# nianticlabs/implicit-depth

Measured on AMD Instinct MI355X. Metric: frames/sec (BDModel.forward hot path, 512x384, 64 planes, 8-frame tuple = 1 current + 7 source views; third-party backbones excluded), higher is better.
Workload: dtype f32

## Files before the change

implicit-depth_amd/_lib.py:

```python
from __future__ import annotations

import ctypes as C
import os

import torch

_HERE = os.path.dirname(os.path.abspath(__file__))
LIB_PATH = os.environ.get("IDH_LIB") or os.path.join(_HERE, "lib", "libidh.so")

_lib = None
MIN_ABI_VERSION = 111

f32p = C.c_void_p


class IdhError(RuntimeError):
    pass


class VolumeOpts(C.Structure):

    _fields_ = [("cur_batch_stride", C.c_int64), ("src_batch_stride", C.c_int64), ("planes", C.c_void_p),
                ("planes_batch_stride", C.c_int64), ("planes_plane_stride", C.c_int64), ("planes_pixel_stride", C.c_int32),
                ("kernel", C.c_int32), ("scratch", C.c_void_p), ("scratch_floats", C.c_int64), ("struct_size", C.c_int64)]

    def __init__(self, *a, **k):
        super().__init__(*a, **k)
        self.struct_size = C.sizeof(VolumeOpts)


CV_KERNEL_LANE, CV_KERNEL_QUAD, CV_KERNEL_WINDOW = 1, 2, 3


class EvalArgs(C.Structure):

    _fields_ = [("struct_size", C.c_int64), ("prediction", C.c_void_p), ("pred_kind", C.c_int32), ("sampling", C.c_int32),
                ("sigmoid_multiplier", C.c_float), ("surface_threshold", C.c_float), ("rendered_bphw", C.c_void_p), ("depth_b1hw", C.c_void_p),
                ("gt_b1HW", C.c_void_p), ("thresholds", C.c_void_p), ("bins", C.c_void_p), ("T", C.c_int32), ("n_bins", C.c_int32),
                ("tag_mask", C.c_int32), ("B", C.c_int32), ("P", C.c_int32), ("h", C.c_int32), ("w", C.c_int32), ("H", C.c_int32), ("W", C.c_int32)]

    def __init__(self, *a, **k):
        super().__init__(*a, **k)
        self.struct_size = C.sizeof(EvalArgs)


EVAL_PRED_LOGITS, EVAL_PRED_DEPTH = 0, 1
EVAL_BILINEAR, EVAL_NEAREST = 0, 1
EVAL_TAG_ALL, EVAL_TAG_SURFACE, EVAL_TAG_BOUNDARY = 1, 2, 4


class CompositeArgs(C.Structure):

    _fields_ = [("struct_size", C.c_int64), ("image_bHW3", C.c_void_p), ("virtual_rgba_bHW4", C.c_void_p), ("map_b1hw", C.c_void_p),
                ("virtual_depth_bHW", C.c_void_p), ("fade_b", C.c_void_p), ("out_bHW3", C.c_void_p), ("matte_out_bHW", C.c_void_p),
                ("plane_distance", C.c_double), ("colour", C.c_double * 3), ("sigmoid_multiplier", C.c_float), ("mode", C.c_int32),
                ("has_colour", C.c_int32), ("has_plane", C.c_int32), ("bgr", C.c_int32), ("B", C.c_int32), ("h", C.c_int32), ("w", C.c_int32),
                ("H", C.c_int32), ("W", C.c_int32)]

    def __init__(self, *a, **k):
        super().__init__(*a, **k)
        self.struct_size = C.sizeof(CompositeArgs)


COMPOSITE_MASK_LOGITS, COMPOSITE_MASK_PROB, COMPOSITE_DEPTH_SOFT, COMPOSITE_DEPTH_HARD = 0, 1, 2, 3


class IngestColorArgs(C.Structure):

    _fields_ = [("struct_size", C.c_int64), ("frames_bHW3", C.c_void_p), ("x_bounds", C.c_void_p), ("x_taps", C.c_void_p), ("y_bounds", C.c_void_p),
                ("y_taps", C.c_void_p), ("image_b3hw", C.c_void_p), ("resized_bhw3", C.c_void_p), ("filter", C.c_int32), ("normalize", C.c_int32),
                ("B", C.c_int32), ("Hs", C.c_int32), ("Ws", C.c_int32), ("h", C.c_int32), ("w", C.c_int32)]

    def __init__(self, *a, **k):
        super().__init__(*a, **k)
        self.struct_size = C.sizeof(IngestColorArgs)


class IngestDepthArgs(C.Structure):

    _fields_ = [("struct_size", C.c_int64), ("depth_bHW", C.c_void_p), ("depth_b1hw", C.c_void_p), ("mask_b1hw", C.c_void_p),
                ("mask_b_b1hw", C.c_void_p), ("full_depth_b1HW", C.c_void_p), ("full_mask_b1HW", C.c_void_p), ("full_mask_b_b1HW", C.c_void_p),
                ("value_scale", C.c_float), ("min_valid", C.c_float), ("max_valid", C.c_float), ("B", C.c_int32), ("Hs", C.c_int32),
                ("Ws", C.c_int32), ("h", C.c_int32), ("w", C.c_int32)]

    def __init__(self, *a, **k):
        super().__init__(*a, **k)
        self.struct_size = C.sizeof(IngestDepthArgs)


class Bank(C.Structure):

    _fields_ = [("struct_size", C.c_int64), ("feats", C.c_void_p), ("mats", C.c_void_p), ("N", C.c_int32), ("H", C.c_int32), ("W", C.c_int32),
                ("C", C.c_int32)]

    def __init__(self, *a, **k):
        super().__init__(*a, **k)
        self.struct_size = C.sizeof(Bank)


BANK_MAX_SLOTS, BANK_MAX_VIEWS = 64, 1024

RESIZE_BILINEAR, RESIZE_BICUBIC = 0, 1
INGEST_MAX_RATIO = 8


class ConvDescSrc(C.Structure):
    _fields_ = [(n, C.c_int32) for n in ("H", "W", "cs", "Cin", "ks", "stride", "is_cat", "_r")]


class ConvDesc(C.Structure):

    _fields_ = ([(n, C.c_int32) for n in ("N", "Ho", "Wo", "Cout", "pad_mode", "act")] + [("slope", C.c_float)] +
                [(n, C.c_int32) for n in ("out_cs", "res_cs", "has_res", "has_norm", "any_size", "math", "n_src")] + [("src", ConvDescSrc * 2)])


class ConvTuning(C.Structure):

    _fields_ = ([(n, C.c_int32) for n in ("winograd", "winograd4", "winograd4_proj", "s2_first", "wino_min_tiles", "wino4_min_tiles", "split_min_blocks",
                                          "narrow_tile_below", "narrowest_tile_below", "split_min_chunks", "split_max", "s2_first_min_blocks",
                                          "fused_up_rows", "target_waves", "min_waves", "_r")] +
                [(n, C.c_double) for n in ("wino_min_fill", "wino4_min_fill", "proj_chunk_weight")])


class ConvChoice(C.Structure):

    _fields_ = [(n, C.c_int32) for n in ("tile_m", "tile_n", "split_k", "w_layout", "families", "lds_tile_m", "lds_split_k", "lds_subtiles", "split_rows",
                                         "direct_tile_m", "direct_tile_n", "direct_split_k")]


_SIGS = {
    "idh_version": (C.c_int, []),
    "idh_sizeof_volume_opts": (C.c_size_t, []),
    "idh_cost_volume_dot_scratch_floats": (C.c_longlong, [C.c_int, C.c_int, C.c_int, C.c_int, C.c_int, C.c_int]),
    "idh_error_string": (C.c_char_p, [C.c_int]),
    "idh_nchw_to_nhwc_f32": (C.c_int, [f32p, f32p, C.c_int, C.c_int, C.c_int, C.c_void_p]),
    "idh_nhwc_to_nchw_f32": (C.c_int, [f32p, f32p, C.c_int, C.c_int, C.c_int, C.c_void_p]),
    "idh_packed_weight_floats": (C.c_size_t, [C.c_int, C.c_int, C.c_int]),
    "idh_pack_conv_weight": (C.c_int, [f32p, f32p, C.c_int, C.c_int, C.c_int, C.c_void_p]),
    "idh_packed_split_weight_bytes": (C.c_size_t, [C.c_int, C.c_int, C.c_int, C.c_int]),
    "idh_pack_conv_weight_split": (C.c_int, [f32p, f32p, C.c_void_p, C.c_int, C.c_int, C.c_int, C.c_int, C.c_void_p]),
    "idh_packed_wino_weight_floats": (C.c_size_t, [C.c_int, C.c_int]),
    "idh_pack_conv_weight_wino": (C.c_int, [f32p, f32p, C.c_int, C.c_int, C.c_void_p]),
    "idh_packed_wino4_weight_floats": (C.c_size_t, [C.c_int, C.c_int]),
    "idh_pack_conv_weight_wino4": (C.c_int, [f32p, f32p, C.c_int, C.c_int, C.c_void_p]),
    "idh_stem_weight_floats": (C.c_size_t, []),
    "idh_pack_stem_weight": (C.c_int, [f32p] * 5 + [C.c_float, f32p, C.c_void_p]),
    "idh_fold_conv_bn": (C.c_int, [f32p, C.c_int, C.c_int] + [f32p] * 4 + [C.c_float, f32p, f32p, C.c_void_p]),
    "idh_sizeof_op": (C.c_size_t, []),
    "idh_run_ops": (C.c_int, [C.c_void_p, C.c_int, C.c_void_p]),
    "idh_count_launches": (C.c_int, [C.c_void_p, C.c_int]),
    "idh_conv_variant": (C.c_int, [C.c_void_p, C.POINTER(C.c_int32)]),
    "idh_conv_tuning_defaults": (None, [C.POINTER(ConvTuning)]),
    "idh_conv_select": (C.c_int, [C.POINTER(ConvDesc), C.POINTER(ConvTuning), C.POINTER(ConvChoice)]),
    "idh_sizeof_conv_select": (None, [C.POINTER(C.c_size_t)]),
    "idh_schedule_ops": (C.c_int, [C.c_void_p, C.c_int, C.c_int, C.c_void_p, C.c_void_p, C.c_int, C.c_void_p, C.c_void_p]),
    "idh_packed_mlp_weight_floats": (C.c_size_t, [C.c_int]),
    "idh_pack_mlp_weight": (C.c_int, [f32p, f32p, C.c_int, C.c_int, C.c_int, C.c_void_p]),
    "idh_binary_mlp_fwd": (C.c_int, [f32p, C.c_int, C.c_int, f32p, f32p, C.c_int, C.c_float, f32p, f32p, f32p, C.c_int, C.c_int, C.c_int, f32p, C.c_void_p]),
    "idh_binary_mlp_strided_fwd": (C.c_int, [f32p, C.c_longlong, C.c_int, C.c_int, C.c_int, f32p, f32p, C.c_int, C.c_float, f32p, f32p, f32p, C.c_int, C.c_int, C.c_int, f32p, C.c_void_p]),
    "idh_binary_mlp_f16x3_fwd": (C.c_int, [f32p, C.c_int, C.c_int, f32p, f32p, C.c_int, C.c_float, f32p, f32p, f32p, C.c_int, C.c_int, C.c_int, f32p, C.c_void_p]),
    "idh_feature_volume_workspace_bytes": (C.c_size_t, [C.c_int]),
    "idh_feature_volume_plane_groups": (C.c_int, [C.c_int] * 4 + [C.POINTER(C.c_int)] * 2),
    "idh_feature_volume_fwd": (
        C.c_int,
        [f32p] * 6 + [C.c_float, C.c_float] + [C.c_int] * 6 + [f32p] * 6 + [f32p, C.c_int, f32p, C.c_void_p, f32p, C.c_void_p, C.c_size_t, C.c_void_p],
    ),
    "idh_feature_volume_f16x3_fwd": (
        C.c_int,
        [f32p] * 6 + [C.c_float, C.c_float] + [C.c_int] * 6 + [f32p] * 6 + [f32p, C.c_int, f32p, C.c_void_p, f32p, C.c_void_p, C.c_size_t, C.c_void_p],
    ),
    "idh_feature_volume_ex_fwd": (
        C.c_int,
        [f32p] * 6 + [C.c_float, C.c_float] + [C.c_int] * 6 + [f32p] * 6 + [f32p, C.c_int, f32p, C.c_void_p, f32p, C.c_void_p, C.c_size_t,
                                                                  C.c_int, C.POINTER(VolumeOpts), C.c_void_p],
    ),
    "idh_cost_volume_dot_ex_fwd": (
        C.c_int,
        [f32p, f32p, f32p, f32p, f32p, C.c_float, C.c_float] + [C.c_int] * 6 + [f32p, C.c_int, f32p, f32p, C.POINTER(VolumeOpts), C.c_void_p],
    ),
    "idh_cost_volume_dot_kernel_name": (C.c_char_p, [C.c_int] * 5),
    "idh_packed_mlp_weight_f16_bytes": (C.c_size_t, [C.c_int]),
    "idh_pack_mlp_weight_f16": (C.c_int, [f32p, C.c_void_p, C.c_int, C.c_int, C.c_int, C.c_void_p]),
    "idh_binary_mlp_search_fwd": (C.c_int, [f32p, C.c_int, C.c_int, f32p, C.c_int, C.c_float, f32p, f32p, f32p, C.c_int, C.c_int, C.c_int,
                                            C.c_float, C.c_float, C.c_float, f32p, f32p, C.c_void_p]),
    "idh_binary_mlp_search_thr_fwd": (C.c_int, [f32p, C.c_int, C.c_int, f32p, C.c_int, C.c_float, f32p, f32p, f32p, C.c_int, C.c_int, C.c_int,
                                                C.c_float, C.c_float, f32p, f32p, C.c_int, f32p, f32p, C.c_void_p]),
    "idh_binary_mlp_search_f16x3_fwd": (C.c_int, [f32p, C.c_int, C.c_int, f32p, C.c_int, C.c_float, f32p, C.c_void_p, f32p, C.c_int, C.c_int, C.c_int,
                                                  C.c_float, C.c_float, C.c_float, f32p, f32p, C.c_int, f32p, f32p, C.c_void_p]),
    "idh_metrics_workspace_bytes": (C.c_size_t, [C.c_int, C.c_int, C.c_int, C.c_int]),
    "idh_plane_iou_fwd": (C.c_int, [f32p, f32p, f32p, f32p, C.c_int, f32p, C.c_int, C.c_int, C.c_int, C.c_int, f32p, C.c_void_p, C.c_size_t, C.c_void_p]),
    "idh_depth_metrics_fwd": (C.c_int, [f32p, f32p, C.c_void_p, C.c_int, C.c_int, C.c_int, f32p, C.c_void_p, C.c_size_t, C.c_void_p]),
    "idh_sizeof_eval_args": (C.c_size_t, []),
    "idh_eval_frame_workspace_bytes": (C.c_size_t, [C.c_int] * 7),
    "idh_eval_masks_fwd": (C.c_int, [f32p, f32p, C.c_int, C.c_int, C.c_int, C.c_int, C.c_float, f32p, f32p, C.c_void_p, C.c_void_p]),
    "idh_eval_plane_scores_fwd": (C.c_int, [C.POINTER(EvalArgs), f32p, C.c_void_p, C.c_void_p, C.c_size_t, C.c_void_p]),
    "idh_eval_depth_metrics_fwd": (C.c_int, [f32p, f32p] + [C.c_int] * 6 + [C.c_float, C.c_int, f32p, C.c_void_p, C.c_size_t, C.c_void_p]),
    "idh_raster_workspace_bytes": (C.c_size_t, [C.c_int] * 3),
    "idh_raster_depth_fwd": (C.c_int, [f32p, C.c_int, C.c_void_p, C.c_int, f32p, f32p, C.c_int, C.c_int, C.c_int, f32p, C.c_void_p, C.c_size_t, C.c_void_p]),
    "idh_vertex_predictions_fwd": (C.c_int, [f32p, C.c_int, f32p, f32p, f32p, f32p, C.c_int, C.c_int, C.c_float, f32p, C.c_void_p]),
    "idh_vertex_occlusion_changes_fwd": (C.c_int, [f32p, C.c_int, C.c_int, C.c_void_p, C.c_void_p]),
    "idh_sizeof_composite_args": (C.c_size_t, []),
    "idh_prep_rendered_depth_fwd": (C.c_int, [f32p, C.c_int, C.c_int, C.c_int, C.c_int, C.c_int, f32p, C.c_void_p]),
    "idh_composite_fwd": (C.c_int, [C.POINTER(CompositeArgs), C.c_void_p]),
    "idh_resize_coeffs_sizes": (C.c_int, [C.c_int, C.c_int, C.c_int, C.POINTER(C.c_int64), C.POINTER(C.c_int64)]),
    "idh_resize_coeffs_pack": (C.c_int, [C.c_int, C.c_int, C.c_int, C.c_void_p, C.c_void_p]),
    "idh_sizeof_ingest_color_args": (C.c_size_t, []),
    "idh_sizeof_ingest_depth_args": (C.c_size_t, []),
    "idh_ingest_color_fwd": (C.c_int, [C.POINTER(IngestColorArgs), C.c_void_p]),
    "idh_ingest_depth_fwd": (C.c_int, [C.POINTER(IngestDepthArgs), C.c_void_p]),
    "idh_sizeof_bank": (C.c_size_t, []),
    "idh_bank_commit_fwd": (C.c_int, [C.POINTER(Bank), C.c_int, f32p, f32p, f32p, f32p, C.c_void_p]),
    "idh_bank_gather_fwd": (C.c_int, [C.POINTER(Bank), C.POINTER(C.c_int32), f32p, f32p, f32p, f32p, f32p, f32p, C.c_int, C.c_int, C.c_void_p]),
    "idh_sample_prior_fwd": (C.c_int, [f32p, f32p, C.c_int, f32p, f32p, f32p, f32p, C.c_int, C.c_int, C.c_int, C.c_int, f32p, C.c_void_p]),
    "idh_binary_mlp_rays_fwd": (C.c_int, [f32p, C.c_int, C.c_int, C.c_int, C.c_int, C.c_int, f32p, f32p, f32p, C.c_int, C.c_float, C.c_int, C.c_int,
                                          C.c_int, C.c_int, C.c_int, f32p, f32p, f32p, f32p, C.c_void_p]),
    "idh_project_points_fwd": (C.c_int, [f32p, f32p, f32p, C.c_int, C.c_int, C.c_int, C.c_int, f32p, f32p, C.c_void_p, f32p, f32p, f32p, f32p, C.c_void_p]),
    "idh_cost_volume_dot_fwd": (
        C.c_int,
        [f32p, f32p, f32p, f32p, f32p, C.c_float, C.c_float] + [C.c_int] * 6 + [f32p, C.c_int, f32p, f32p, C.c_void_p],
    ),
}


def _all_sigs():
    from . import model_abi, net_abi

    return {**_SIGS, **net_abi.SIGS, **model_abi.SIGS}


def declared_symbols():
    return sorted(_all_sigs())


def lib():
    global _lib
    if _lib is None:
        if not os.path.exists(LIB_PATH):
            raise IdhError(
                f"{LIB_PATH} not found — the gfx950 HIP extension is not built. Run "
                "`python -c 'import __graft_entry__ as g; g.build()'` (there is no CPU fallback)."
            )
        h = C.CDLL(LIB_PATH)
        for name, (res, args) in _all_sigs().items():
            try:
                fn = getattr(h, name)
            except AttributeError:
                raise IdhError(f"{LIB_PATH} does not export {name}: it was built from an older tree; rebuild with `python implicit-depth_amd/build.py --force`") from None
            fn.restype = res
            fn.argtypes = args
        ver = h.idh_version()
        if ver < MIN_ABI_VERSION and not os.environ.get("IDH_LIB_ANY_ABI"):
            raise IdhError(f"{LIB_PATH} reports ABI version {ver}, this binding needs >= {MIN_ABI_VERSION}: rebuild with `python implicit-depth_amd/build.py --force`")
        if h.idh_sizeof_eval_args() != C.sizeof(EvalArgs):
            raise IdhError(f"{LIB_PATH}: sizeof(idh_eval_args) = {h.idh_sizeof_eval_args()} in the library, {C.sizeof(EvalArgs)} in this binding")
        if h.idh_sizeof_composite_args() != C.sizeof(CompositeArgs):
            raise IdhError(f"{LIB_PATH}: sizeof(idh_composite_args) = {h.idh_sizeof_composite_args()} in the library, {C.sizeof(CompositeArgs)} in this binding")
        for what, got, mirror in (("idh_ingest_color_args", h.idh_sizeof_ingest_color_args(), IngestColorArgs),
                                  ("idh_ingest_depth_args", h.idh_sizeof_ingest_depth_args(), IngestDepthArgs),
                                  ("idh_bank", h.idh_sizeof_bank(), Bank)):
            if got != C.sizeof(mirror):
                raise IdhError(f"{LIB_PATH}: sizeof({what}) = {got} in the library, {C.sizeof(mirror)} in this binding")
        sizes = (C.c_size_t * 3)()
        h.idh_sizeof_conv_select(sizes)
        if list(sizes) != [C.sizeof(ConvDesc), C.sizeof(ConvTuning), C.sizeof(ConvChoice)]:
            raise IdhError(f"{LIB_PATH}: sizeof(idh_conv_desc / _tuning / _choice) = {list(sizes)} in the library, another in this binding")
        if h.idh_sizeof_volume_opts() != C.sizeof(VolumeOpts):
            raise IdhError(f"{LIB_PATH}: sizeof(idh_volume_opts) = {h.idh_sizeof_volume_opts()} in the library, {C.sizeof(VolumeOpts)} in this binding")
        _lib = h
    return _lib


def check(code: int, what: str) -> None:
    if code != 0:
        msg = lib().idh_error_string(code).decode()
        raise IdhError(f"{what} failed: {msg} ({code})")


def ptr(t: "torch.Tensor | None"):
    if t is None:
        return None
    return t.data_ptr()


def stream_ptr():
    return torch.cuda.current_stream().cuda_stream


_weights_epoch = 0


def invalidate_weight_caches() -> None:
    global _weights_epoch
    _weights_epoch += 1


def _sd_post_hook(module, incompatible_keys) -> None:
    invalidate_weight_caches()


def watch_state_dict_loads(module) -> None:
    for m in module.modules():
        if not m.__dict__.get("_idh_sd_hook"):
            m.register_load_state_dict_post_hook(_sd_post_hook)
            m.__dict__["_idh_sd_hook"] = True


def param_version(t):
    try:
        return t._version
    except RuntimeError:
        return ("inference", _weights_epoch)


def require_cuda_f32(*tensors):
    for t in tensors:
        if t is None:
            continue
        if not t.is_cuda:
            raise IdhError("implicit_depth_amd kernels need tensors on the MI355X (got a CPU tensor); there is no CPU fallback")
        if t.dtype != torch.float32:
            raise IdhError(f"implicit_depth_amd kernels are fp32 (got {t.dtype})")
```

implicit-depth_amd/csrc/conv.hip:

```cpp
#include <algorithm>
#include "conv_args.h"
#include "../../include/idh_ops.h"

using namespace idh_conv;

int idh_stem_op(const idh_op &op, hipStream_t st, bool launch);

namespace {

__device__ float g_zero_page[kZeroFloats];

thread_local bool t_dry_run = false;
thread_local int t_launches = 0;
#undef IDH_CHECK_LAUNCH
#define IDH_CHECK_LAUNCH()                                              \
    do {                                                                \
        if (!t_dry_run && hipGetLastError() != hipSuccess) return IDH_ELAUNCH; \
    } while (0)
#define IDH_LAUNCH(...)                         \
    do {                                        \
        if (t_dry_run) ++t_launches;            \
        else hipLaunchKernelGGL(__VA_ARGS__);   \
    } while (0)

// ... 896 lines not shown
            float *o = a.out + ((size_t)n * a.HW + p) * a.out_cs + 4 * h;
#pragma unroll
            for (int j = 0; j < NT; ++j) {
                f32x4 v = acc[j];
                if (a.bias) v += *reinterpret_cast<const f32x4 *>(a.bias + 16 * j + 4 * h);
                *reinterpret_cast<f32x4 *>(o + 16 * j) = v;
            }
        }
    };
    f32x4 xa[C16], xb[C16];
    long long t = blockIdx.x;
    if (t >= a.tiles) return;
    load(t, xa);
    for (;;) {
        const long long t1 = t + gridDim.x;
        if (t1 < a.tiles) load(t1, xb);
        compute(t, xa);
        if (t1 >= a.tiles) break;
        const long long t2 = t1 + gridDim.x;
        if (t2 < a.tiles) load(t2, xa);
        compute(t1, xb);
        if (t2 >= a.tiles) break;
        t = t2;
    }
}

struct PwUpArgs {
    const float *in, *w, *bias, *low;
    float *out;
    int H, W, in_cs, low_cs, out_cs, tiles_per_img;
    long long tiles;
};

template <int C16, int NT>
__global__ __launch_bounds__(256) void pointwise_up_k(const PwUpArgs a) {
    constexpr int kCout = 16 * NT;
    extern __shared__ f32x4 sWu[];
    {
        const f32x4 *g = reinterpret_cast<const f32x4 *>(a.w);
        for (int i = threadIdx.x; i < 4 * C16 * kCout; i += 256) sWu[i] = g[i];
    }
    __syncthreads();
    const int lane = threadIdx.x & 63;
    const int wave = __builtin_amdgcn_readfirstlane(threadIdx.x >> 6);
    const int ln = lane & 15, h = lane >> 4;
    const int HW = a.H * a.W, Hl = a.H >> 1, Wl = a.W >> 1;
    for (long long tile = blockIdx.x; tile < a.tiles; tile += gridDim.x) {
        const int n = (int)(tile / a.tiles_per_img);
        const int p = (int)(tile - (long long)n * a.tiles_per_img) * kPwTile + 16 * wave + ln;
        const bool ok = p < HW;
        const int pc = ok ? p : 0;
        const float *ip = a.in + ((size_t)n * HW + pc) * a.in_cs + 4 * h;
        f32x4 x[C16];
#pragma unroll
        for (int c = 0; c < C16; ++c) x[c] = *reinterpret_cast<const f32x4 *>(ip + 16 * c);
        const int y = pc / a.W, xq = pc - y * a.W;
        const int iy = y >> 1, ix = xq >> 1;
        int y0, y1, x0, x1;
        float hy0, hy1, wx0, wx1;
        if (y & 1) { y0 = iy; y1 = min(iy + 1, Hl - 1); hy0 = 0.75f; hy1 = 0.25f; }
        else { y0 = max(iy - 1, 0); y1 = iy; hy0 = 0.25f; hy1 = 0.75f; }
        if (xq & 1) { x0 = ix; x1 = min(ix + 1, Wl - 1); wx0 = 0.75f; wx1 = 0.25f; }
        else { x0 = max(ix - 1, 0); x1 = ix; wx0 = 0.25f; wx1 = 0.75f; }
        const float *lb = a.low + (size_t)n * Hl * Wl * a.low_cs + 4 * h;
        const float *t00 = lb + ((size_t)y0 * Wl + x0) * a.low_cs, *t01 = lb + ((size_t)y0 * Wl + x1) * a.low_cs;
        const float *t10 = lb + ((size_t)y1 * Wl + x0) * a.low_cs, *t11 = lb + ((size_t)y1 * Wl + x1) * a.low_cs;
        f32x4 acc[NT];
#pragma unroll
        for (int j = 0; j < NT; ++j) acc[j] = a.bias ? *reinterpret_cast<const f32x4 *>(a.bias + 16 * j + 4 * h) : (f32x4){0.f, 0.f, 0.f, 0.f};
        int opaque = 0;
        asm volatile("" : "+s"(opaque));
        const f32x4 *sWt = sWu + opaque;
#pragma unroll
        for (int c = 0; c < C16; ++c)
#pragma unroll
            for (int j = 0; j < NT; ++j) {
                const f32x4 A = sWt[(4 * c + h) * kCout + 16 * j + ln];
#pragma unroll
                for (int kk = 0; kk < 4; ++kk) acc[j] = __builtin_amdgcn_mfma_f32_16x16x4f32(A[kk], x[c][kk], acc[j], 0, 0, 0);
            }
        if (ok) {
            float *o = a.out + ((size_t)n * HW + p) * a.out_cs + 4 * h;
#pragma unroll
            for (int j = 0; j < NT; ++j) {
                const f32x4 p00 = *reinterpret_cast<const f32x4 *>(t00 + 16 * j), p01 = *reinterpret_cast<const f32x4 *>(t01 + 16 * j);
                const f32x4 p10 = *reinterpret_cast<const f32x4 *>(t10 + 16 * j), p11 = *reinterpret_cast<const f32x4 *>(t11 + 16 * j);
                f32x4 v;
#pragma unroll
                for (int e = 0; e < 4; ++e) v[e] = acc[j][e] + (hy0 * (wx0 * p00[e] + wx1 * p01[e]) + hy1 * (wx0 * p10[e] + wx1 * p11[e]));
                *reinterpret_cast<f32x4 *>(o + 16 * j) = v;
            }
        }
    }
}

__global__ __launch_bounds__(256) void pointwise_head_k(const float *__restrict__ in, const float *__restrict__ w,
                                                        const float *__restrict__ bias, float *__restrict__ out,
                                                        float *__restrict__ out_exp, long long M, int C, int in_cs) {
    for (long long m = blockIdx.x * 256ll + threadIdx.x; m < M; m += gridDim.x * 256ll) {
        const float4 *p = reinterpret_cast<const float4 *>(in + m * in_cs);
        const float4 *wv = reinterpret_cast<const float4 *>(w);
        float s = 0.f;
        for (int q = 0; q < (C >> 2); ++q) {
            const float4 a = p[q], b = wv[q];
            s = fmaf(a.x, b.x, s); s = fmaf(a.y, b.y, s); s = fmaf(a.z, b.z, s); s = fmaf(a.w, b.w, s);
        }
        const float v = s + (bias ? bias[0] : 0.f);
        out[m] = v;
        if (out_exp) out_exp[m] = expf(v);
    }
}

constexpr int kInChunk = 1024;

template <int SUB>
__global__ __launch_bounds__(1024) void instnorm_stats_k(const float *__restrict__ in, int cs, int C, int HW, int nchunks,
                                                         float *__restrict__ part) {
    extern __shared__ float red[];
    const int n = blockIdx.y, chunk = blockIdx.x;
    const int cq = C >> 2;
    const int q = threadIdx.x % cq;
    const int prow = threadIdx.x / cq, pstep = (int)blockDim.x / cq;
    const int rows = SUB * pstep;
    const int p0 = chunk * kInChunk, p1 = min(HW, p0 + kInChunk);
    const float4 pv = *reinterpret_cast<const float4 *>(in + (size_t)n * HW * cs + 4 * q);
    float s[SUB][4], ss[SUB][4];
#pragma unroll
    for (int u = 0; u < SUB; ++u)
#pragma unroll
        for (int e = 0; e < 4; ++e) s[u][e] = ss[u][e] = 0.f;
    for (int p = p0 + prow; p < p1; p += rows) {
#pragma unroll
        for (int u = 0; u < SUB; ++u) {
            const int pp = p + u * pstep;
            if (pp < p1) {
                const float4 v = *reinterpret_cast<const float4 *>(in + ((size_t)n * HW + pp) * cs + 4 * q);
                const float d0 = v.x - pv.x, d1 = v.y - pv.y, d2 = v.z - pv.z, d3 = v.w - pv.w;
                s[u][0] += d0; s[u][1] += d1; s[u][2] += d2; s[u][3] += d3;
                ss[u][0] = fmaf(d0, d0, ss[u][0]); ss[u][1] = fmaf(d1, d1, ss[u][1]); ss[u][2] = fmaf(d2, d2, ss[u][2]); ss[u][3] = fmaf(d3, d3, ss[u][3]);
            }
        }
    }
#pragma unroll
    for (int u = 0; u < SUB; ++u) {
        float *mine = red + ((size_t)(prow + u * pstep) * cq + q) * 8;
#pragma unroll
        for (int e = 0; e < 4; ++e) { mine[e] = s[u][e]; mine[4 + e] = ss[u][e]; }
    }
    __syncthreads();
    for (int t = threadIdx.x; t < 8 * cq; t += blockDim.x) {
        const int qq = t >> 3, e = t & 7;
        float a = 0.f;
        for (int r = 0; r < rows; ++r) a += red[(r * cq + qq) * 8 + e];
        part[((size_t)(n * nchunks + chunk) * 2 + (e >> 2)) * C + 4 * qq + (e & 3)] = a;
    }
}

__global__ __launch_bounds__(256) void instnorm_finalize_k(const float *__restrict__ part, const float *__restrict__ in, int cs, int C, int HW,
                                                           int nchunks, float *__restrict__ stats) {
    const int n = blockIdx.x;
    for (int c = threadIdx.x; c < C; c += 256) {
        float s = 0.f, ss = 0.f;
        for (int k = 0; k < nchunks; ++k) {
            const float *o = part + ((size_t)(n * nchunks + k) * 2) * C + c;
            s += o[0];
            ss += o[C];
        }
        const float ms = s / (float)HW;
        const float var = fmaxf(ss / (float)HW - ms * ms, 0.f);
        stats[(size_t)n * 2 * C + c] = in[(size_t)n * HW * cs + c] + ms;
        stats[(size_t)n * 2 * C + C + c] = 1.0f / sqrtf(var + 1e-5f);
    }
}

__global__ __launch_bounds__(256) void instnorm_apply_k(const float *__restrict__ in, int cs, float *__restrict__ out, int out_cs,
                                                        int C, int HW, long long total, const float *__restrict__ stats, int act,
                                                        float slope) {
    const int cq = C >> 2;
    for (long long t = blockIdx.x * 256ll + threadIdx.x; t < total; t += gridDim.x * 256ll) {
        const int q = (int)(t % cq);
        const long long np = t / cq;
        const int n = (int)(np / HW);
        const float4 mean = *reinterpret_cast<const float4 *>(stats + (size_t)n * 2 * C + 4 * q);
        const float4 rstd = *reinterpret_cast<const float4 *>(stats + (size_t)n * 2 * C + C + 4 * q);
        const float4 v = *reinterpret_cast<const float4 *>(in + (size_t)np * cs + 4 * q);
        float r[4] = {(v.x - mean.x) * rstd.x, (v.y - mean.y) * rstd.y, (v.z - mean.z) * rstd.z, (v.w - mean.w) * rstd.w};
        for (int e = 0; e < 4; ++e) r[e] = act_apply(r[e], act, slope);
        *reinterpret_cast<float4 *>(out + (size_t)np * out_cs + 4 * q) = make_float4(r[0], r[1], r[2], r[3]);
    }
}

enum { LV_LDS4 = 0, LV_LDS2 = 1, LV_MFMA14 = 2, LV_UP2 = 3 };
struct LevelArgs {
    int n;
    unsigned start[kMaxGroup + 1];
    int kind[kMaxGroup];
    LdsConvArgs op[kMaxGroup];
};

template <bool WIDE>
__global__ __launch_bounds__(256) void level_k(const LevelArgs g) {
    __shared__ f32x4 sA[lds_a_slots(1)];
    __shared__ f32x4 sB[lds_b_slots(WIDE ? 4 : 2)];
    int idx = 0;
    for (int i = 1; i < g.n; ++i)
        if (blockIdx.x >= g.start[i]) idx = i;
    const unsigned blk = blockIdx.x - g.start[idx], nblk = g.start[idx + 1] - g.start[idx];
    const LdsConvArgs &la = g.op[idx];
    switch (g.kind[idx]) {
        case LV_LDS4:
            if constexpr (WIDE) conv3x3_lds_body<1, false, 4>(la, blk, nblk, sA, sB);
            break;
        case LV_LDS2: conv3x3_lds_body<1, false, 2>(la, blk, nblk, sA, sB); break;
        case LV_MFMA14: conv_mfma_body<1, 4>(la.c, blk, nblk); break;
        default: upsample2_body(la.c.s[0].in, la.c.out, la.c.M, la.c.s[0].H, la.c.s[0].W, la.c.s[0].Cin, la.c.s[0].cs, la.c.out_cs, blk, nblk); break;
    }
}

inline int ceil16(int v) { return (v + 15) & ~15; }

struct PreparedConv {
    ConvArgs a;
    LdsConvArgs la;
    int lds_rows, tm, tn;
    int n_img;
    unsigned blocks;
    bool up;
    bool norm;
    bool s2;
    int nj;
    ReduceDesc red;
};

int prep_conv(const idh_op &op, PreparedConv &pc) {
    ConvArgs &a = pc.a;
    a = ConvArgs{};
    pc.up = false;
    pc.norm = op.src[0].norm != nullptr;
    pc.s2 = false;
    pc.nj = 4;
    int steps = 0;
    for (int i = 0; i < 2; ++i) {
        const idh_conv_src &s = op.src[i];
        ConvSrc &d = a.s[i];
        d.in = s.in;
        if (!s.in) continue;
        if (!s.w || s.Cin <= 0 || s.cs < (s.up_in[0] ? s.up_c0 : ceil16(s.Cin)) || (s.cs & 3) || (s.ks != 1 && s.ks != 3) ||
            (s.stride != 1 && s.stride != 2) || s.H <= 0 || s.W <= 0)
            return IDH_EINVAL;
        if (ceil16(s.Cin) > kZeroFloats) return IDH_EUNSUPPORTED;
        const int pad = s.ks / 2;
        if ((s.H + 2 * pad - s.ks) / s.stride + 1 != op.Ho || (s.W + 2 * pad - s.ks) / s.stride + 1 != op.Wo)
            return IDH_EINVAL;
        d.w = s.w; d.cs = s.cs; d.H = s.H; d.W = s.W; d.Cin = s.Cin; d.ks = s.ks; d.stride = s.stride;
        d.pad_mode = s.pad_mode; d.cblocks = ceil16(s.Cin) / 16;
        d.up_in[0] = s.up_in[0]; d.up_in[1] = s.up_in[1]; d.up_cs[0] = s.up_cs[0]; d.up_cs[1] = s.up_cs[1];
        d.up_c0 = s.up_c0; d.up_C = s.up_C;
        d.norm = s.norm; d.norm_slope = s.norm_slope; d.norm_act = s.norm_act;
        if (s.norm && (i != 0 || s.up_in[0] || ((uintptr_t)s.norm & 15) || (s.Cin & 15))) return IDH_EUNSUPPORTED;
        if (s.up_in[0]) {
            const int nseg = s.up_in[1] ? 2 : 1;
            if (s.up_c0 < 0 || (s.up_c0 & 15) || s.up_C <= 0 || (s.up_C & 15) || s.up_c0 + nseg * s.up_C != s.Cin || (s.H & 1) || (s.W & 1) ||
                s.stride != 1 || (s.up_c0 > 0 && s.cs < s.up_c0) || s.up_cs[0] < s.up_C || (s.up_cs[0] & 3) ||
                (nseg == 2 && (s.up_cs[1] < s.up_C || (s.up_cs[1] & 3))))
                return IDH_EINVAL;
            pc.up = true;
        }
        steps += s.ks * s.ks * d.cblocks;
    }
    if (!a.s[0].in || !op.out || op.Cout <= 0 || op.N <= 0) return IDH_EINVAL;
    if ((op.Cout & 3) || (op.out_cs & 3) || ((uintptr_t)op.out & 15) || (op.bias && ((uintptr_t)op.bias & 15)) ||
        (op.res && ((op.res_cs & 3) || ((uintptr_t)op.res & 15))))
        return IDH_EINVAL;
    a.bias = op.bias; a.res = op.res; a.out = op.out; a.ws = op.ws;
    a.res_cs = op.res_cs; a.out_cs = op.out_cs; a.Ho = op.Ho; a.Wo = op.Wo; a.Cout = op.Cout;
    a.Cout_pad = ceil16(op.Cout);
    const long long M = (long long)op.N * op.Ho * op.Wo;
    if (M >= (1ll << 31)) return IDH_EUNSUPPORTED;
    a.M = (int)M; a.steps_total = steps; a.act = op.act; a.slope = op.slope;
    a.S = op.split_k > 1 ? op.split_k : 1;
    if (a.S > steps) a.S = steps;
    if (a.s[0].ks == 3 && a.s[0].stride == 2 && !a.s[1].in && (op.tile_m == 8 || op.tile_m == 9) && a.s[0].pad_mode == IDH_PAD_ZEROS &&
        !a.s[0].up_in[0] && !a.s[0].norm && op.Wo >= kLT_W && (op.Cout % 32) == 0 && (op.tile_n == 0 ? (op.Cout % 64) == 0 : op.tile_n == 2)) {
        a.s[1] = a.s[0];
        ConvSrc e{};
        e.in = a.s[1].in; e.w = a.s[1].w; e.ks = 3; e.stride = 1; e.pad_mode = IDH_PAD_ZEROS;
        a.s[0] = e;
    }
    const int nj = (op.tile_m == 8 || op.tile_m == 9 || op.tile_m == 0) ? (op.tile_n == 0 ? 4 : op.tile_n) : 4;
    const bool lds_ok = a.s[0].ks == 3 && a.s[0].stride == 1 && (nj == 4 || nj == 2 || nj == 1) && (op.Cout % (16 * nj)) == 0 &&
                        (a.s[0].pad_mode == IDH_PAD_ZEROS || (a.s[0].pad_mode == IDH_PAD_REPLICATE && !a.s[1].in)) &&
                        (!a.s[1].in || (a.s[1].ks == 1 && a.s[1].stride == 1) ||
                         (a.s[1].ks == 3 && a.s[1].stride == 2 && a.s[1].pad_mode == IDH_PAD_ZEROS && !a.s[1].up_in[0] && !a.s[0].up_in[0] &&
                          !op.src[0].norm && (nj == 4 || nj == 2))) &&
                        op.Wo >= kLT_W;
    pc.lds_rows = 0;
    const bool lds_fits = (long long)a.s[0].H * a.s[0].W * a.s[0].cs * 4 < (1ll << 31) && 9ll * a.s[0].cblocks * 4 * a.Cout_pad * 16 < (1ll << 31) &&
                          (!a.s[1].in || ((long long)a.s[1].H * a.s[1].W * a.s[1].cs * 4 < (1ll << 31) && 9ll * a.s[1].cblocks * 4 * a.Cout_pad * 16 < (1ll << 31))) &&
                          (long long)op.Ho * op.Wo * op.out_cs * 4 < (1ll << 31) && (!op.res || (long long)op.Ho * op.Wo * op.res_cs * 4 < (1ll << 31));
    if (op.tile_m == IDH_TILE_WINO) {
        if (!wino_supported(a)) return IDH_EUNSUPPORTED;
        pc.lds_rows = 32;
        pc.tm = op.tile_m;
        pc.tn = 0;
        pc.n_img = op.N;
        pc.blocks = 0;
    } else if (op.tile_m == IDH_TILE_WINO4) {
        if (!wino4_supported(a)) return IDH_EUNSUPPORTED;
        pc.lds_rows = 36;
        pc.tm = op.tile_m;
        pc.tn = 0;
        pc.n_img = op.N;
        pc.blocks = 0;
    } else if (op.tile_m == IDH_SPLIT_F16X3) {
        if (!lds_ok || a.s[0].pad_mode != IDH_PAD_ZEROS || (op.Cout % 64) || a.S != 1 || op.Wo < kSplitTile || op.Ho < 1 || (op.tile_n != 0 && op.tile_n != 8 && op.tile_n != 16))
            return IDH_EUNSUPPORTED;
        if (a.s[1].in && (a.s[1].ks != 1 || a.s[1].stride != 1 || a.s[1].H != op.Ho || a.s[1].W != op.Wo || a.s[1].up_in[0] || a.s[1].norm))
            return IDH_EUNSUPPORTED;
        a.NT = op.Cout / 64;
        pc.lds_rows = 16;
        pc.tm = op.tile_m;
        pc.tn = op.tile_n == 8 ? 8 : 16;
        pc.n_img = op.N;
        pc.blocks = 0;
    } else if (lds_ok && lds_fits && (op.tile_m == 8 || op.tile_m == 0 || op.tile_m == 9)) {
        const int rows = op.tile_m == 9 ? 4 : 8;
        const int chunks = a.s[0].cblocks + (a.s[1].in ? a.s[1].cblocks : 0);
        if (a.S > chunks) a.S = chunks;
        {
            const int w1 = (a.s[1].in && a.s[1].ks == 3) ? 9 : 1;
            const int T = 9 * a.s[0].cblocks + (a.s[1].in ? w1 * a.s[1].cblocks : 0);
            const int smax = T / 9 > 1 ? T / 9 : 1;
            if (a.S > smax) a.S = smax;
        }
        a.NT = op.Cout / (16 * nj);
        pc.nj = nj;
        pc.la = LdsConvArgs{a, (op.Wo + kLT_W - 1) / kLT_W, (op.Ho + rows - 1) / rows};
        const long long blocks = (long long)a.S * op.N * pc.la.tiles_x * pc.la.tiles_y * a.NT;
        if (blocks >= (1ll << 31)) return IDH_EUNSUPPORTED;
        pc.blocks = (unsigned)blocks;
        pc.lds_rows = rows;
        pc.s2 = a.s[1].in && a.s[1].ks == 3;
    } else {
        int tm = op.tile_m, tn = op.tile_n;
        if (tm == 8 || tm == 9) tm = 0;
        const int nsub = a.Cout_pad / 16;
        if (tn == 0) tn = (nsub % 4 == 0) ? 4 : (nsub % 2 == 0 ? 2 : 1);
        if (tm == 0) tm = 4;
        if ((tm != 1 && tm != 2 && tm != 4) || (tn != 1 && tn != 2 && tn != 4) || nsub % tn) return IDH_EINVAL;
        a.MT = (int)((M + 16 * tm - 1) / (16 * tm));
        a.NT = nsub / tn;
        pc.tm = tm; pc.tn = tn;
        const long long waves = (long long)a.MT * a.NT * a.S;
        if ((waves + 3) / 4 >= (1ll << 31)) return IDH_EUNSUPPORTED;
        pc.blocks = (unsigned)((waves + 3) / 4);
    }
    if (pc.up && ((pc.lds_rows != 8 && pc.lds_rows != 4) || pc.nj != 4)) return IDH_EUNSUPPORTED;
    if (pc.norm && ((pc.lds_rows != 8 && pc.lds_rows != 4) || pc.nj != 1)) return IDH_EUNSUPPORTED;
    if (a.S > 1) {
        if (!op.ws) return IDH_EWORKSPACE;
        pc.red = ReduceDesc{op.ws, op.bias, op.res, op.out, a.M, op.Cout, a.Cout_pad, a.S, op.res_cs, op.out_cs, op.act, op.slope};
    }
    return IDH_OK;
}

int launch_conv(const PreparedConv &pc, hipStream_t st) {
    if (pc.lds_rows == 16) {
        if (t_dry_run) { ++t_launches; return IDH_OK; }
        return launch_conv_split(pc.a, pc.n_img, pc.tm, pc.tn, st);
    }
    if (pc.lds_rows == 32) {
        if (t_dry_run) { ++t_launches; return IDH_OK; }
        return launch_conv_wino(pc.a, pc.n_img, pc.tn, st);
    }
    if (pc.lds_rows == 36) {
        if (t_dry_run) { ++t_launches; return IDH_OK; }
        return launch_conv_wino4(pc.a, pc.n_img, st);
    }
    if (pc.lds_rows == 8 && pc.up) IDH_LAUNCH(conv3x3_lds_up_k<2>, dim3(pc.blocks), dim3(256), 0, st, pc.la);
    else if (pc.lds_rows == 8 && pc.s2 && pc.nj == 4) IDH_LAUNCH((conv3x3_lds_k<2, false, 4, false, true>), dim3(pc.blocks), dim3(256), 0, st, pc.la);
    else if (pc.lds_rows == 8 && pc.s2) IDH_LAUNCH((conv3x3_lds_k<2, false, 2, false, true>), dim3(pc.blocks), dim3(256), 0, st, pc.la);
    else if (pc.lds_rows == 4 && pc.s2 && pc.nj == 4) IDH_LAUNCH((conv3x3_lds_k<1, false, 4, false, true>), dim3(pc.blocks), dim3(256), 0, st, pc.la);
    else if (pc.lds_rows == 4 && pc.s2) IDH_LAUNCH((conv3x3_lds_k<1, false, 2, false, true>), dim3(pc.blocks), dim3(256), 0, st, pc.la);
    else if (pc.lds_rows == 8 && pc.norm) IDH_LAUNCH((conv3x3_lds_k<2, false, 1, true>), dim3(pc.blocks), dim3(256), 0, st, pc.la);
    else if (pc.lds_rows == 4 && pc.norm) IDH_LAUNCH((conv3x3_lds_k<1, false, 1, true>), dim3(pc.blocks), dim3(256), 0, st, pc.la);
    else if (pc.lds_rows == 8 && pc.nj == 2) IDH_LAUNCH((conv3x3_lds_k<2, false, 2>), dim3(pc.blocks), dim3(256), 0, st, pc.la);
    else if (pc.lds_rows == 8 && pc.nj == 1) IDH_LAUNCH((conv3x3_lds_k<2, false, 1>), dim3(pc.blocks), dim3(256), 0, st, pc.la);
    else if (pc.lds_rows == 4 && pc.nj == 2) IDH_LAUNCH((conv3x3_lds_k<1, false, 2>), dim3(pc.blocks), dim3(256), 0, st, pc.la);
    else if (pc.lds_rows == 4 && pc.nj == 1) IDH_LAUNCH((conv3x3_lds_k<1, false, 1>), dim3(pc.blocks), dim3(256), 0, st, pc.la);
    else if (pc.lds_rows == 8) IDH_LAUNCH((conv3x3_lds_k<2, false>), dim3(pc.blocks), dim3(256), 0, st, pc.la);
    else if (pc.lds_rows == 4 && pc.up) IDH_LAUNCH(conv3x3_lds_up_k<1>, dim3(pc.blocks), dim3(256), 0, st, pc.la);
    else if (pc.lds_rows == 4) IDH_LAUNCH((conv3x3_lds_k<1, false>), dim3(pc.blocks), dim3(256), 0, st, pc.la);
    else {
#define IDH_CASE(TM_, TN_) \
    if (pc.tm == TM_ && pc.tn == TN_) IDH_LAUNCH((conv_mfma_k<TM_, TN_>), dim3(pc.blocks), dim3(256), 0, st, pc.a);
        IDH_CASE(4, 4) IDH_CASE(2, 4) IDH_CASE(1, 4) IDH_CASE(4, 2) IDH_CASE(2, 2) IDH_CASE(1, 2) IDH_CASE(4, 1)
        IDH_CASE(2, 1) IDH_CASE(1, 1)
#undef IDH_CASE
    }
    IDH_CHECK_LAUNCH();
    return IDH_OK;
}

int launch_reduces(const PreparedConv *pcs, int n, hipStream_t st) {
    ReduceGroupArgs g{};
    unsigned cursor = 0;
    for (int i = 0; i < n; ++i) {
        if (pcs[i].a.S <= 1) continue;
        g.start[g.n] = cursor;
        g.d[g.n] = pcs[i].red;
        cursor += (unsigned)idh_cdiv((long long)pcs[i].red.M * pcs[i].red.Cout, 256);
        ++g.n;
    }
    if (g.n == 0) return IDH_OK;
    g.start[g.n] = cursor;
    IDH_LAUNCH(splitk_reduce_group_k, dim3(cursor), dim3(256), 0, st, g);
    IDH_CHECK_LAUNCH();
    return IDH_OK;
}

int launch_group(const PreparedConv *pcs, int n, hipStream_t st) {
    LdsGroupArgs g{};
    unsigned cursor = 0;
    g.n = n;
    for (int i = 0; i < n; ++i) {
        g.start[i] = cursor;
        g.op[i] = pcs[i].la;
        cursor += pcs[i].blocks;
    }
    g.start[n] = cursor;
    bool any_up = false;
    for (int i = 0; i < n; ++i) any_up = any_up || pcs[i].up;
    if (any_up) IDH_LAUNCH((conv3x3_lds_group_k<1, true>), dim3(cursor), dim3(256), 0, st, g);
    else if (pcs[0].nj == 2) IDH_LAUNCH((conv3x3_lds_group_k<1, false, 2>), dim3(cursor), dim3(256), 0, st, g);
    else if (pcs[0].nj == 1) IDH_LAUNCH((conv3x3_lds_group_k<1, false, 1>), dim3(cursor), dim3(256), 0, st, g);
    else IDH_LAUNCH((conv3x3_lds_group_k<1, false>), dim3(cursor), dim3(256), 0, st, g);
    IDH_CHECK_LAUNCH();
    return launch_reduces(pcs, n, st);
}

int launch_level(const PreparedConv *pcs, const int *kinds, int n, hipStream_t st) {
    LevelArgs g{};
    unsigned cursor = 0;
    g.n = n;
    for (int i = 0; i < n; ++i) {
        g.start[i] = cursor;
        g.kind[i] = kinds[i];
        g.op[i] = pcs[i].la;
        if (kinds[i] == LV_MFMA14) g.op[i].c = pcs[i].a;
        cursor += pcs[i].blocks;
    }
    g.start[n] = cursor;
    bool wide = false;
    for (int i = 0; i < n; ++i) wide = wide || kinds[i] == LV_LDS4;
    if (wide) IDH_LAUNCH(level_k<true>, dim3(cursor), dim3(256), 0, st, g);
    else IDH_LAUNCH(level_k<false>, dim3(cursor), dim3(256), 0, st, g);
    IDH_CHECK_LAUNCH();
    return launch_reduces(pcs, n, st);
}

int level_kind(const PreparedConv &pc) {
    if (pc.up || pc.norm || pc.s2) return -1;
    if (pc.lds_rows == 4 && pc.nj == 4) return LV_LDS4;
    if (pc.lds_rows == 4 && pc.nj == 2) return LV_LDS2;
    if (pc.lds_rows == 0 && pc.tm == 1 && pc.tn == 4) return LV_MFMA14;
    return -1;
}

int check_upsample(const idh_op &op) {
    const idh_conv_src &s = op.src[0];
    if (!s.in || !op.out || (s.Cin & 3) || (s.cs & 3) || (op.out_cs & 3) || op.N <= 0 || s.H <= 0 || s.W <= 0 || s.Cin <= 0) return IDH_EINVAL;
    if ((long long)op.N * s.H * s.W * (s.Cin >> 2) >= (1ll << 31)) return IDH_EUNSUPPORTED;
    return IDH_OK;
}

constexpr unsigned kLevelMaxBlocks = 512;
constexpr unsigned kLevelUpsampleBlocks = 512;
constexpr long long kLevelUpsampleNatural = 4096;

}

extern "C" size_t idh_sizeof_op(void) { return sizeof(idh_op); }

extern "C" size_t idh_packed_weight_floats(int Cout, int Cin, int ks) {
    if (Cout <= 0 || Cin <= 0 || ks <= 0) return 0;
    return (size_t)ks * ks * ceil16(Cin) * ceil16(Cout);
}

extern "C" int idh_pack_conv_weight(const float *w, float *dst, int Cout, int Cin, int ks, void *stream) {
    if (!w || !dst || Cout <= 0 || Cin <= 0 || (ks != 1 && ks != 3)) return IDH_EINVAL;
    const long long total = (long long)idh_packed_weight_floats(Cout, Cin, ks);
    int grid = idh_cdiv(total, 256);
    if (grid > 4096) grid = 4096;
    hipLaunchKernelGGL(pack_weight_k, dim3(grid), dim3(256), 0, idh_stream(stream), w, dst, Cout, Cin, ks, ceil16(Cin),
                       ceil16(Cout));
    IDH_CHECK_LAUNCH();
    return IDH_OK;
}

extern "C" int idh_run_ops(const idh_op *ops, int n, void *stream) {
    if (n < 0 || (n > 0 && !ops)) return IDH_EINVAL;
    hipStream_t st = idh_stream(stream);
    for (int i = 0; i < n; ++i) {
        const idh_op &op = ops[i];
        const idh_conv_src &s = op.src[0];
        switch (op.kind) {
            case IDH_OP_CONV:
            case IDH_OP_UPSAMPLE2: {
                PreparedConv pcs[kMaxGroup];
                int kinds[kMaxGroup];
                int run = 0;
                for (int j = i; j < n && run < kMaxGroup; ++j) {
                    const idh_op &o = ops[j];
                    if (j > i && (op.group == 0 || o.group != op.group)) break;
                    PreparedConv &pc = pcs[run];
                    if (o.kind == IDH_OP_CONV) {
                        const int rc = prep_conv(o, pc);
                        if (rc != IDH_OK) return rc;
                        kinds[run] = level_kind(pc);
                    } else if (o.kind == IDH_OP_UPSAMPLE2) {
                        const int rc = check_upsample(o);
                        if (rc != IDH_OK) return rc;
                        const idh_conv_src &us = o.src[0];
                        pc = PreparedConv{};
                        ConvArgs &c = pc.la.c;
                        c.s[0].in = us.in; c.s[0].H = us.H; c.s[0].W = us.W; c.s[0].Cin = us.Cin; c.s[0].cs = us.cs;
                        c.out = o.out; c.out_cs = o.out_cs; c.M = o.N; c.S = 1;
                        pc.a = c;
                        const long long tot = (long long)o.N * 4 * us.H * us.W * (us.Cin >> 2);
                        const long long natural = idh_cdiv(tot, 256);
                        pc.blocks = (unsigned)std::min<long long>(idh_cdiv(tot / 4, 256), kLevelUpsampleBlocks);
                        kinds[run] = natural <= kLevelUpsampleNatural ? LV_UP2 : -1;
                    } else {
                        break;
                    }
                    ++run;
                }
                int cnt = 0;
                if (op.kind == IDH_OP_CONV && pcs[0].lds_rows == 4 && !pcs[0].norm && !pcs[0].s2) {
                    cnt = 1;
                    while (cnt < run && ops[i + cnt].kind == IDH_OP_CONV && pcs[cnt].lds_rows == 4 && pcs[cnt].nj == pcs[0].nj &&
                           (!pcs[cnt].up || pcs[0].nj == 4) && !pcs[cnt].norm && !pcs[cnt].s2)
                        ++cnt;
                }
                int mix = 0;
                while (mix < run && kinds[mix] >= 0 && pcs[mix].blocks <= kLevelMaxBlocks) ++mix;
                int wg = 0;
                if (op.kind == IDH_OP_CONV && pcs[0].lds_rows == 32) {
                    wg = 1;
                    while (wg < run && wg < wino_max_group() && ops[i + wg].kind == IDH_OP_CONV && pcs[wg].lds_rows == 32 &&
                           (pcs[wg].a.s[1].in != nullptr) == (pcs[0].a.s[1].in != nullptr))
                        ++wg;
                }
                int rc, used;
                if (wg > 1) {
                    if (t_dry_run) {
                        ++t_launches;
                        rc = IDH_OK;
                    } else {
                        const ConvArgs *as[kMaxGroup];
                        int ns[kMaxGroup];
                        for (int j = 0; j < wg; ++j) { as[j] = &pcs[j].a; ns[j] = pcs[j].n_img; }
                        rc = launch_conv_wino_group(as, ns, wg, st);
                        if (rc == IDH_EUNSUPPORTED) {
                            rc = IDH_OK;
                            for (int j = 0; j < wg && rc == IDH_OK; ++j) rc = launch_conv(pcs[j], st);
                        }
                    }
                    used = wg;
                } else if (mix > cnt && mix > 1) {
                    rc = launch_level(pcs, kinds, mix, st);
                    used = mix;
                } else if (cnt > 1) {
                    rc = launch_group(pcs, cnt, st);
                    used = cnt;
                } else if (op.kind == IDH_OP_CONV) {
                    rc = launch_conv(pcs[0], st);
                    if (rc == IDH_OK) rc = launch_reduces(pcs, 1, st);
                    used = 1;
                } else {
                    const long long quads = (long long)op.N * s.H * s.W * (s.Cin >> 2);
                    int grid = idh_cdiv(quads, 256);
                    if (grid > 32768) grid = 32768;
                    IDH_LAUNCH(upsample2_k, dim3(grid), dim3(256), 0, st, s.in, op.out, op.N, s.H, s.W, s.Cin, s.cs, op.out_cs);
                    IDH_CHECK_LAUNCH();
                    rc = IDH_OK;
                    used = 1;
                }
                if (rc != IDH_OK) return rc;
                i += used - 1;
                break;
            }
            case IDH_OP_UPSAMPLE2_NEAREST: {
                if (!s.in || !op.out || (s.Cin & 3) || (s.cs & 3) || (op.out_cs & 3) || op.N <= 0) return IDH_EINVAL;
                const long long tot = (long long)op.N * 4 * s.H * s.W * (s.Cin >> 2);
                int grid = idh_cdiv(tot, 256);
                if (grid > 8192) grid = 8192;
                IDH_LAUNCH(upsample2_nearest_k, dim3(grid), dim3(256), 0, st, s.in, op.out, op.N, s.H, s.W, s.Cin, s.cs, op.out_cs);
                IDH_CHECK_LAUNCH();
                break;
            }
            case IDH_OP_NCHW_TO_NHWC: {
                ImportGroupArgs g{};
                unsigned cursor = 0;
                int run = 0;
                for (int j = i; j < n && run < kMaxImport; ++j) {
                    const idh_op &o = ops[j];
                    if (o.kind != IDH_OP_NCHW_TO_NHWC || (j > i && (op.group == 0 || o.group != op.group))) break;
                    const idh_conv_src &os = o.src[0];
                    if (!os.in || !o.out || o.N <= 0 || o.N > 65535 || os.H <= 0 || os.W <= 0 || os.Cin <= 0) return IDH_EINVAL;
                    const int HWj = os.H * os.W;
                    const long long blocks = (long long)idh_cdiv(HWj, 64) * idh_cdiv(os.Cin, 32) * o.N;
                    if (blocks > kLevelMaxBlocks * 8ll || cursor + blocks >= (1ll << 31)) break;
                    g.d[run].src = os.in; g.d[run].dst = o.out; g.d[run].C = os.Cin; g.d[run].HW = HWj; g.d[run].out_cs = o.out_cs;
                    g.d[run].nbx = idh_cdiv(HWj, 64); g.d[run].nby = idh_cdiv(os.Cin, 32);
                    g.start[run] = cursor;
                    cursor += (unsigned)blocks;
                    ++run;
                }
                if (run > 1) {
                    g.n = run;
                    g.start[run] = cursor;
                    IDH_LAUNCH(import_nchw_group_k, dim3(cursor), dim3(256), 0, st, g);
                    IDH_CHECK_LAUNCH();
                    i += run - 1;
                    break;
                }
                if (!s.in || !op.out || op.N <= 0 || op.N > 65535) return IDH_EINVAL;
                const int HW = s.H * s.W;
                IDH_LAUNCH(import_nchw_k, dim3(idh_cdiv(HW, 64), idh_cdiv(s.Cin, 32), op.N), dim3(256), 0, st, s.in,
                                   op.out, s.Cin, HW, op.out_cs);
                IDH_CHECK_LAUNCH();
                break;
            }
            case IDH_OP_NHWC_TO_NCHW: {
                if (!s.in || !op.out || op.N <= 0 || op.N > 65535) return IDH_EINVAL;
                const int HW = s.H * s.W;
                IDH_LAUNCH(export_nchw_k, dim3(idh_cdiv(HW, 64), idh_cdiv(s.Cin, 32), op.N), dim3(256), 0, st, s.in,
                                   op.out, s.Cin, HW, s.cs);
                IDH_CHECK_LAUNCH();
                break;
            }
            case IDH_OP_POINTWISE_HEAD: {
                if (!s.in || !s.w || !op.out || (s.Cin & 3) || (s.cs & 3)) return IDH_EINVAL;
                const long long M = (long long)op.N * s.H * s.W;
                int grid = idh_cdiv(M, 256);
                if (grid > 8192) grid = 8192;
                IDH_LAUNCH(pointwise_head_k, dim3(grid), dim3(256), 0, st, s.in, s.w, op.bias, op.out, op.ws, M, s.Cin,
                                   s.cs);
                IDH_CHECK_LAUNCH();
                break;
            }
            case IDH_OP_POINTWISE_NCHW: {
                if (!s.in || !s.w || !op.out || op.N <= 0 || s.H <= 0 || s.W <= 0 || (op.out_cs & 3) || ((uintptr_t)op.out & 15) ||
                    (op.bias && ((uintptr_t)op.bias & 15)))
                    return IDH_EINVAL;
                if (s.Cin != kPwCin || op.Cout != kPwCout || op.out_cs < kPwCout || (long long)s.H * s.W * kPwCin * 4 >= (1ll << 31))
                    return IDH_EUNSUPPORTED;
                PwNchwArgs pa{};
                pa.in = s.in; pa.w = s.w; pa.bias = op.bias; pa.out = op.out;
                pa.HW = s.H * s.W; pa.out_cs = op.out_cs;
                pa.tiles_per_img = idh_cdiv(pa.HW, kPwTile);
                pa.tiles = (long long)op.N * pa.tiles_per_img;
                const int grid = (int)std::min<long long>(pa.tiles, 256 * 4 * 4);
                IDH_LAUNCH(pointwise_nchw_k, dim3(grid), dim3(256), 0, st, pa);
                IDH_CHECK_LAUNCH();
                break;
            }
            case IDH_OP_POINTWISE_UP: {
                const idh_conv_src &lo = op.src[1];
                if (!s.in || !s.w || !lo.in || !op.out || op.N <= 0 || s.H <= 0 || s.W <= 0 || (s.H & 1) || (s.W & 1) || (s.cs & 3) || (lo.cs & 3) || (op.out_cs & 3) ||
                    s.cs < s.Cin || lo.cs < op.Cout || op.out_cs < op.Cout || ((uintptr_t)s.in & 15) || ((uintptr_t)lo.in & 15) || ((uintptr_t)op.out & 15) ||
                    ((uintptr_t)s.w & 15) || (op.bias && ((uintptr_t)op.bias & 15)) || lo.H != s.H / 2 || lo.W != s.W / 2)
                    return IDH_EINVAL;
                if (s.Cin != op.Cout || (s.Cin != 64 && s.Cin != 128) || (long long)s.H * s.W >= (1ll << 31)) return IDH_EUNSUPPORTED;
                PwUpArgs pa{};
                pa.in = s.in; pa.w = s.w; pa.bias = op.bias; pa.low = lo.in; pa.out = op.out;
                pa.H = s.H; pa.W = s.W; pa.in_cs = s.cs; pa.low_cs = lo.cs; pa.out_cs = op.out_cs;
                pa.tiles_per_img = idh_cdiv(s.H * s.W, kPwTile);
                pa.tiles = (long long)op.N * pa.tiles_per_img;
                const int grid = (int)std::min<long long>(pa.tiles, 256 * 8);
                if (s.Cin == 64) IDH_LAUNCH((pointwise_up_k<4, 4>), dim3(grid), dim3(256), 16 * 64 * sizeof(f32x4), st, pa);
                else IDH_LAUNCH((pointwise_up_k<8, 8>), dim3(grid), dim3(256), 32 * 128 * sizeof(f32x4), st, pa);
                IDH_CHECK_LAUNCH();
                break;
            }
            case IDH_OP_STEM: {
                const int rc = idh_stem_op(op, st, !t_dry_run);
                if (rc != IDH_OK) return rc;
                if (t_dry_run) ++t_launches;
                break;
            }
            case IDH_OP_COPY: {
                if (!s.in || !op.out || (s.Cin & 3) || (s.cs & 3) || (op.out_cs & 3) || op.N <= 0) return IDH_EINVAL;
                const long long npix = (long long)op.N * s.H * s.W;
                int grid = idh_cdiv(npix * (s.Cin >> 2), 256);
                if (grid > 8192) grid = 8192;
                IDH_LAUNCH(copy_nhwc_k, dim3(grid), dim3(256), 0, st, s.in, op.out, npix, s.Cin, s.cs, op.out_cs);
                IDH_CHECK_LAUNCH();
                break;
            }
            case IDH_OP_INSTNORM: {
                const int C = s.Cin, HW = s.H * s.W;
                if (!s.in || !op.ws || C <= 0 || (C & 3) || 256 % (C >> 2) || (s.cs & 3) || (op.out && (op.out_cs & 3)) ||
                    op.N <= 0 || op.N > 65535)
                    return IDH_EINVAL;
                const int nchunks = idh_cdiv(HW, kInChunk);
                const int sthreads = ((long long)nchunks * op.N < 512 && C >= 64) ? 1024 : 256;
                if (C >= 64 && sthreads == 256)
                    IDH_LAUNCH(instnorm_stats_k<4>, dim3(nchunks, op.N), dim3(256), 1024 * 8 * sizeof(float), st, s.in, s.cs, C, HW, nchunks, op.ws);
                else
                    IDH_LAUNCH(instnorm_stats_k<1>, dim3(nchunks, op.N), dim3(sthreads), sthreads * 8 * sizeof(float), st, s.in, s.cs, C, HW,
                                       nchunks, op.ws);
                IDH_CHECK_LAUNCH();
                float *stats = op.ws + (size_t)op.N * nchunks * 2 * C;
                IDH_LAUNCH(instnorm_finalize_k, dim3(op.N), dim3(256), 0, st, op.ws, s.in, s.cs, C, HW, nchunks, stats);
                IDH_CHECK_LAUNCH();
                if (!op.out) break;
                const long long total = (long long)op.N * HW * (C >> 2);
                int gx = idh_cdiv(total, 256 * 4);
                if (gx > 16384) gx = 16384;
                IDH_LAUNCH(instnorm_apply_k, dim3(gx), dim3(256), 0, st, s.in, s.cs, op.out, op.out_cs, C, HW, total, stats, op.act,
                                   op.slope);
                IDH_CHECK_LAUNCH();
                break;
            }
            default:
                return IDH_EINVAL;
        }
    }
    return IDH_OK;
}

extern "C" int idh_conv_variant(const idh_op *op, int32_t out[8]) {
    if (!op || !out || op->kind != IDH_OP_CONV) return IDH_EINVAL;
    PreparedConv pc{};
    const int rc = prep_conv(*op, pc);
    if (rc != IDH_OK) return rc;
    const bool lds = pc.lds_rows == 8 || pc.lds_rows == 4;
    out[0] = pc.lds_rows;
    out[1] = lds ? pc.nj : 0;
    out[2] = lds ? 0 : pc.tm;
    out[3] = lds ? 0 : pc.tn;
    out[4] = pc.a.S;
    out[5] = pc.up;
    out[6] = pc.norm;
    out[7] = pc.s2;
    return IDH_OK;
}

extern "C" int idh_count_launches(const idh_op *ops, int n) {
    t_dry_run = true;
    t_launches = 0;
    const int rc = idh_run_ops(ops, n, nullptr);
    t_dry_run = false;
    return rc == IDH_OK ? t_launches : rc;
}
```

implicit-depth_amd/csrc/conv_args.h:

```cpp
#pragma once
#include "idh_common.h"

namespace idh_conv {

typedef float f32x4 __attribute__((ext_vector_type(4)));

struct ConvSrc {
    const float *in;
    const float *w;
    int cs, H, W, Cin;
    int ks, stride, pad_mode, cblocks;
    const float *up_in[2];
    int up_cs[2];
    int up_c0, up_C;
    const float *norm;
    float norm_slope;
    int norm_act;
};

struct ConvArgs {
    ConvSrc s[2];
    const float *bias;
    const float *res;
    float *out;
    float *ws;
    int res_cs, out_cs;
    int Ho, Wo, Cout, Cout_pad;
    int M;
    int MT, NT, S;
    int steps_total;
    int act;
    float slope;
};

__device__ __forceinline__ float act_apply(float v, int act, float slope) {
    if (act == IDH_ACT_LRELU) return (slope >= 0.f && slope <= 1.f) ? fmaxf(v, v * slope) : (v < 0.f ? v * slope : v);
    if (act == IDH_ACT_ELU) return v > 0.f ? v : expm1f(v);
    return v;
}

template <typename Body>
__device__ __forceinline__ void act_dispatch(int act, float slope, Body &&body) {
    if (act == IDH_ACT_LRELU) {
        if (slope >= 0.f && slope <= 1.f) body([slope](float v) { return fmaxf(v, v * slope); });
        else body([slope](float v) { return v < 0.f ? v * slope : v; });
    } else if (act == IDH_ACT_ELU) {
        body([](float v) { return v > 0.f ? v : expm1f(v); });
    } else {
        body([](float v) { return v; });
    }
}

constexpr int kZeroFloats = 4096;

constexpr int kSplitTile = 16;
int launch_conv_split(const ConvArgs &a, int N, int mode, int rows, hipStream_t st);

bool wino_supported(const ConvArgs &a);
int launch_conv_wino(const ConvArgs &a, int N, int rows, hipStream_t st);
int wino_max_group();
int launch_conv_wino_group(const ConvArgs *const *as, const int *Ns, int n, hipStream_t st);

bool wino4_supported(const ConvArgs &a);
int launch_conv_wino4(const ConvArgs &a, int N, hipStream_t st);
bool wino4_split_enabled();

}
```

implicit-depth_amd/csrc/conv_wino.hip:

```cpp
#include <type_traits>

#include "conv_args.h"
#include "../../include/idh_ops.h"

using namespace idh_conv;

namespace {

typedef unsigned u32x4_t __attribute__((ext_vector_type(4)));
typedef __attribute__((address_space(3))) void lds_void;

constexpr int kWinoCH = 8;
constexpr int kWinoTileW = 32;
constexpr int kWinoHalf = 17;
constexpr int kOob = 0x7fffffff;

constexpr int wino_plane(int WAVES) { return (2 * WAVES + 2) * 2 * kWinoHalf; }
constexpr int wino_qs(int WAVES) { return (wino_plane(WAVES) + 63) / 64 * 64; }
constexpr int wino_stage(int WAVES, int NCO) { return 4 * wino_qs(WAVES) + NCO * 1024; }

__global__ __launch_bounds__(256) void pack_wino_weight_k(const float *__restrict__ w, float *__restrict__ dst, int Cout, int Cin, int nS, int nCB, int KS) {
    const long long total = (long long)nS * nCB * 16 * 64 * KS;
    for (long long t = blockIdx.x * 256ll + threadIdx.x; t < total; t += gridDim.x * 256ll) {
        const int e = (int)(t % KS);
        long long r = t / KS;
        const int m = (int)(r & 15), h = (int)((r >> 4) & 3), pos = (int)((r >> 6) & 15);
        r >>= 10;
        const int cb = (int)(r % nCB), c = (int)(r / nCB);
        const int co = 16 * cb + m, ci = 4 * KS * c + KS * h + e;
        double u = 0.0;
        if (co < Cout && ci < Cin) {
            const float *g = w + ((size_t)co * Cin + ci) * 9;
            const int xi = pos >> 2, nu = pos & 3;
            const double G[4][3] = {{1.0, 0.0, 0.0}, {0.5, 0.5, 0.5}, {0.5, -0.5, 0.5}, {0.0, 0.0, 1.0}};
            for (int a = 0; a < 3; ++a)
                for (int b = 0; b < 3; ++b) u += G[xi][a] * (double)g[a * 3 + b] * G[nu][b];
        }
        dst[t] = (float)u;
    }
}

__device__ __forceinline__ void dma16(__amdgpu_buffer_rsrc_t rs, f32x4 *dst, int voff, int soff) {
    __builtin_amdgcn_raw_ptr_buffer_load_lds(rs, (lds_void *)dst, 16, voff, soff, 0, 0);
}
struct BufRef {
    const float *p;
    int bytes;
};
__device__ __forceinline__ void dma16(BufRef b, f32x4 *dst, int voff, int soff) {
    dma16(__builtin_amdgcn_make_buffer_rsrc(const_cast<float *>(b.p), 0, b.bytes, 0x00020000), dst, voff, soff);
}

#ifdef IDH_ABL_WINO_TRACE
#define WINO_TRACE(idx) do { if (lane == 0) trace[(idx)] = __builtin_readcyclecounter(); } while (0)
#else
#define WINO_TRACE(idx) do { } while (0)
#endif

struct WinoArgs {
    ConvArgs c;
    int tiles_x, tiles_y;
    int tiles;
};

template <int WAVES, int NCO, int CH, bool SRC2>
constexpr int wino_stage_slots() {
    constexpr int halo = ((CH / 4) * wino_plane(WAVES) + 63) / 64 * 64;
    constexpr int s3 = halo + 64 * NCO * 4 * (CH / 4), sp = 8 * 32 * 2 * WAVES + 64 * 2 * NCO;
    return SRC2 && sp > s3 ? sp : s3;
}

template <int WAVES, int NCO, int CH, bool SRC2>
__device__ __forceinline__ void wino_tiles(const WinoArgs &wa, f32x4 *lds, const unsigned vblock, const unsigned vgrid) {
    constexpr int KS = CH / 4;
    constexpr int NP = CH / 4;
    typedef float vec __attribute__((ext_vector_type(KS)));
    constexpr int kRows = 2 * WAVES;
    constexpr int kPlane = wino_plane(WAVES);
    static_assert(NP == 2, "halo swizzle written for 8-channel K steps");
    constexpr int kHaloPieces = (NP * kPlane + 63) / 64;
    constexpr int kHP = (kHaloPieces + WAVES - 1) / WAVES;
    constexpr int kPanelPieces = NCO * 4 * KS;
    static_assert(kPanelPieces % WAVES == 0, "panel pieces must split evenly over the waves");
    constexpr int kPanel = kPanelPieces / WAVES;
    constexpr int kTPW = kHP + kPanel;
    static_assert(CH == 8, "K steps of 8 channels: every tile has >= 2 steps (the first stores the previous tile's outputs, the last loads the residual)");
    static_assert(kTPW <= 8 && 4 * NCO <= 8, "one DMA piece per even position group, one output store per odd group");
    constexpr int kHalo = 64 * kHaloPieces;
    constexpr int kTight = 32 * kRows;
    constexpr int kStage3 = kHalo + 64 * kPanelPieces;
    constexpr int kStageP = 8 * kTight + 64 * 2 * NCO;
    constexpr int kStage = SRC2 && kStageP > kStage3 ? kStageP : kStage3;
    static_assert(kStage == wino_stage_slots<WAVES, NCO, CH, SRC2>(), "stage size used by the kernels' LDS declaration");

    const ConvArgs &a = wa.c;
    const ConvSrc &s = a.s[0];
    const int lane = threadIdx.x & 63;
    const int wave = __builtin_amdgcn_readfirstlane(threadIdx.x >> 6);
    const int n = lane & 15, h = lane >> 4;
#ifdef IDH_ABL_WINO_TRACE
    unsigned long long *trace = reinterpret_cast<unsigned long long *>(a.ws) + ((size_t)blockIdx.x * WAVES + wave) * 64;
    int tr_i = 1;
    WINO_TRACE(0);
    if (lane == 0) trace[63] = __builtin_amdgcn_s_getreg((4 << 0) | (0 << 6) | (31 << 11));
#endif
    const int nS = s.cblocks * (16 / CH);
    const int nCB = a.Cout_pad / 16;
    const BufRef rsW{s.w, s.cblocks * nCB * 16384};

    const int T = wa.tiles;
    int t_cur, t_end, t_stride;
    if ((vgrid & 7) == 0) {
        const int xcd = vblock & 7;
        t_stride = vgrid >> 3;
        t_cur = (int)((long long)T * xcd / 8) + (int)(vblock >> 3);
        t_end = (int)((long long)T * (xcd + 1) / 8);
    } else {
        t_cur = vblock; t_end = T; t_stride = vgrid;
    }
    if (t_cur >= t_end) return;

    int y0, x0, cb0, img;
    auto decode = [&](int t) {
        unsigned blk = (unsigned)t;
        const int nt = blk % a.NT; blk /= a.NT;
        const int tx = blk % wa.tiles_x; blk /= wa.tiles_x;
        const int ty = blk % wa.tiles_y;
        img = blk / wa.tiles_y;
        y0 = ty * kRows; x0 = tx * kWinoTileW; cb0 = nt * NCO;
    };
    BufRef rsA;
    int voffH[kHP], panel_so;
    const int voffP = 16 * lane;
    auto halo_piece = [&](int k) { return wave + WAVES * k < kHaloPieces ? wave + WAVES * k : wave; };
    auto halo_voff = [&](int j, int lane) {
        const int pt = 32 * j + (lane >> 1);
        const int row = pt / kWinoHalf, hxh = pt - row * kWinoHalf;
        const int q = (lane & 1) ^ ((hxh >> 3) & 1);
        const int iy = y0 - 1 + (row >> 1), ix = x0 - 1 + 2 * hxh + (row & 1);
        const bool ok = (pt < kPlane) & ((unsigned)iy < (unsigned)s.H) & ((unsigned)ix < (unsigned)s.W);
        return ok ? (iy * s.W + ix) * s.cs * 4 + 16 * q : kOob;
    };
    auto set_fetch_tile = [&]() {
        rsA = BufRef{s.in + (size_t)img * s.H * s.W * s.cs, s.H * s.W * s.cs * 4};
        int lane_o = lane;
        asm volatile("" : "+v"(lane_o));
#pragma unroll
        for (int k = 0; k < kHP; ++k) voffH[k] = halo_voff(halo_piece(k), lane_o);
        panel_so = (cb0 * (4 * KS) + wave * kPanel) * 1024;
    };
    static_assert(!SRC2 || (kTight == 64 * WAVES && 2 * NCO == WAVES), "P-step pieces: eight of the pixels and one of the panel per wave");
    constexpr int kTPW2 = SRC2 ? 9 : 0;
    const ConvSrc &s1 = a.s[1];
    const int nS2 = SRC2 ? (s1.cblocks + 1) / 2 : 0;
    BufRef rsA2 = rsW, rsW2 = rsW;
    int voffT = 0, voffP2 = 0;
    if constexpr (SRC2) {
        rsW2 = BufRef{s1.w, s1.cblocks * 4 * a.Cout_pad * 16};
        voffP2 = ((lane >> 4) * a.Cout_pad + (lane & 15)) * 16;
    }
    int tile2_so = 0;
    auto set_fetch_tile2 = [&]() {
        if constexpr (SRC2) {
            rsA2 = BufRef{s1.in + (size_t)img * s1.H * s1.W * s1.cs, s1.H * s1.W * s1.cs * 4};
            tile2_so = (y0 * s1.W + x0) * s1.cs * 4;
        }
    };
    if constexpr (SRC2) voffT = 2 * (lane >> 3) * s1.cs * 4;
    auto issue_next = [&](int k, bool p, int c, int stage, int cbf) {
        int so, lo, vo;
        bool halo = true;
        const int k0 = k < kTPW ? k : kTPW - 1;
        if (k0 < kHP) {
            vo = voffH[k0]; so = 4 * CH * c; lo = 64 * halo_piece(k0);
        } else {
            const int i = k0 - kHP;
            halo = false;
            vo = voffP; so = panel_so + (c * nCB * (4 * KS) + i) * 1024; lo = kHalo + 64 * (wave * kPanel + i);
        }
#ifdef IDH_ABL_WINO_NOHALO
        if (halo && c + stage > 0) return;
#endif
#ifdef IDH_ABL_WINO_NOPANEL
        if (!halo && c + stage > 0) return;
#endif
        BufRef rs = halo ? rsA : rsW;
        if constexpr (SRC2) {
            int so1, lo1, vo1;
            bool halo1 = true;
            if (k < 8) {
                const int t = 8 * wave + k;
                const int plane = (lane & 7) ^ ((4 * (t & 1) + (lane >> 4)) & 7);
                vo1 = (plane >= 4 && 2 * c + 1 >= s1.cblocks) ? kOob : voffT + 16 * plane;
                so1 = tile2_so + (((t >> 2) * s1.W + 16 * (t & 1) + ((t >> 1) & 1)) * s1.cs + 32 * c) * 4;
                lo1 = 64 * t;
            } else {
                const int hh = wave / NCO, cbw = wave % NCO;
                halo1 = false;
                vo1 = voffP2; so1 = (4 * (2 * c + hh) * a.Cout_pad + 16 * (cbf + cbw)) * 16; lo1 = 8 * kTight + 64 * wave;
            }
            const int m = -(int)p;
            const unsigned long long m64 = (unsigned long long)(long long)m;
            vo ^= (vo ^ vo1) & m; so ^= (so ^ so1) & m; lo ^= (lo ^ lo1) & m;
            const BufRef rs1 = halo1 ? rsA2 : rsW2;
            const unsigned long long p0 = (unsigned long long)rs.p, p1 = (unsigned long long)rs1.p;
            rs.p = reinterpret_cast<const float *>(p0 ^ ((p0 ^ p1) & m64));
            rs.bytes ^= (rs.bytes ^ rs1.bytes) & m;
        }
        dma16(rs, lds + __builtin_amdgcn_readfirstlane(stage * kStage + lo), vo, __builtin_amdgcn_readfirstlane(so));
    };

    f32x4 acc[16][NCO];
    f32x4 ost[2][2][NCO];
    int voffS[2][2];
    __amdgpu_buffer_rsrc_t rsS;
    bool pending = false;

    const int pq = (KS * h) >> 2, pb8 = ((KS * h) & 3) * 4;
    const int patch0 = (NP * ((4 * wave) * kWinoHalf + n) + (pq ^ ((n >> 3) & 1))) * 16 + pb8;
    const int frag0 = kHalo * 16 + (h * 16 + n) * (4 * KS);

    constexpr int kAhead = CH == 16 ? 2 : 3;
    auto compute = [&](int stage, bool pnext, int cnext, int snext, int cbf, bool flush) {
        typedef const __attribute__((address_space(3))) volatile char lds_cchar;
        typedef const __attribute__((address_space(3))) volatile vec lds_cvec;
        int n_o = n;
        asm volatile("" : "+v"(n_o));
        const int patch1 = patch0 + (NP + ((pq ^ (((n_o + 1) >> 3) & 1)) - (pq ^ ((n_o >> 3) & 1)))) * 16;
        lds_cchar *sH0 = (lds_cchar *)(lds + stage * kStage) + patch0, *sH1 = (lds_cchar *)(lds + stage * kStage) + patch1;
        lds_cchar *sW = (lds_cchar *)(lds + stage * kStage) + frag0;
        vec d[4][4], A[kAhead + 1][NCO], r[4];
        auto rd_frag = [&](int g) {
            const int p = ((g >> 2) == 0 ? 4 : (g >> 2) == 1 ? 8 : (g >> 2) == 2 ? 0 : 12) + (g & 3);
#pragma unroll
            for (int j = 0; j < NCO; ++j) A[g % (kAhead + 1)][j] = *(lds_cvec *)(sW + (j * 16 + p) * 64 * (4 * KS));
        };
        auto rd_row = [&](int y) {
#pragma unroll
            for (int x = 0; x < 4; ++x) d[y][x] = *(lds_cvec *)(((x >> 1) ? sH1 : sH0) + NP * (2 * y + (x & 1)) * kWinoHalf * 16);
        };
        rd_frag(0);
        rd_row(1);
        rd_row(2);
#pragma unroll
        for (int g = 1; g < kAhead; ++g) rd_frag(g);
#pragma unroll
        for (int g = 0; g < 16; ++g) {
            const int xi = (g >> 2) == 0 ? 1 : (g >> 2) == 1 ? 2 : (g >> 2) == 2 ? 0 : 3, nu = g & 3;
            const int p = 4 * xi + nu;
            if (g + kAhead < 16) rd_frag(g + kAhead);
            if (g == 5) rd_row(0);
            if (g == 9) rd_row(3);
#ifndef IDH_ABL_WINO_NODMA
            if ((g & 1) == 0 && (g >> 1) < kTPW) issue_next(g >> 1, pnext, cnext, snext, cbf);
            if (SRC2 && (g == 1 || g == 3) && kTPW + (g >> 1) < kTPW2) {
                if (pnext) issue_next(kTPW + (g >> 1), true, cnext, snext, cbf);
            }
#endif
#ifndef IDH_ABL_WINO_NOSTORE
            if ((g & 1) == 1 && (g >> 1) < 4 * NCO && flush) {
                const int k = g >> 1;
                __builtin_amdgcn_raw_buffer_store_b128(__builtin_bit_cast(u32x4_t, ost[k >> 1 & 1][k & 1][k >> 2]), rsS, voffS[k >> 1 & 1][k & 1] + 64 * (k >> 2), 0, 0);
            }
#endif
            __builtin_amdgcn_sched_barrier(0);
#ifdef IDH_ABL_WINO_SCALARXF
            auto vadd = [](vec a, vec b) { vec o; for (int e = 0; e < KS; ++e) { float t = a[e] + b[e]; asm("" : "+v"(t)); o[e] = t; } return o; };
            auto vsub = [](vec a, vec b) { vec o; for (int e = 0; e < KS; ++e) { float t = a[e] - b[e]; asm("" : "+v"(t)); o[e] = t; } return o; };
#else
            auto vadd = [](vec a, vec b) { return a + b; };
            auto vsub = [](vec a, vec b) { return a - b; };
#endif
#ifndef IDH_ABL_WINO_NOXFORM
            if (nu == 0) {
#pragma unroll
                for (int x = 0; x < 4; ++x)
                    r[x] = xi == 0 ? vsub(d[0][x], d[2][x]) : xi == 1 ? vadd(d[1][x], d[2][x]) : xi == 2 ? vsub(d[2][x], d[1][x]) : vsub(d[1][x], d[3][x]);
            }
#endif
#ifdef IDH_ABL_WINO_NOXFORM
            const vec v = d[xi][nu];
#else
            const vec v = nu == 0 ? vsub(r[0], r[2]) : nu == 1 ? vadd(r[1], r[2]) : nu == 2 ? vsub(r[2], r[1]) : vsub(r[1], r[3]);
#endif
#pragma unroll
            for (int k = 0; k < KS; ++k)
#pragma unroll
                for (int j = 0; j < NCO; ++j)
                    acc[p][j] = __builtin_amdgcn_mfma_f32_16x16x4f32(A[g % (kAhead + 1)][j][k], v[k], acc[p][j], 0, 0, 0);
            __builtin_amdgcn_sched_barrier(0);
        }
    };

    auto compute_p = [&](int stage, bool pnext, int cnext, int snext, int cbf) {
        int ln_o = lane;
        asm volatile("" : "+v"(ln_o));
        const int n_o = ln_o & 15, h_o = ln_o >> 4;
        const f32x4 *sH = lds + stage * kStage + 8 * ((4 * wave) * 16 + n_o);
        const int x0s = h_o ^ ((n_o >> 1) & 7);
        const f32x4 *sW = lds + stage * kStage + 8 * kTight + ln_o;
        f32x4 d2[2][2][2], A1[2][NCO];
#pragma unroll
        for (int hh = 0; hh < 2; ++hh)
#pragma unroll
            for (int j = 0; j < NCO; ++j) A1[hh][j] = sW[64 * (hh * NCO + j)];
#pragma unroll
        for (int i = 0; i < 2; ++i)
#pragma unroll
            for (int j = 0; j < 2; ++j)
#pragma unroll
                for (int hh = 0; hh < 2; ++hh) d2[i][j][hh] = sH[8 * 16 * (2 * i + j) + (x0s ^ (4 * hh))];
#pragma unroll
        for (int g = 0; g < 8; ++g) {
            if (pnext) {
                if (g < 4) { issue_next(2 * g, true, cnext, snext, cbf); issue_next(2 * g + 1, true, cnext, snext, cbf); }
                if (g == 4) issue_next(8, true, cnext, snext, cbf);
            } else {
                if (g < 3) { issue_next(2 * g, false, cnext, snext, cbf); issue_next(2 * g + 1, false, cnext, snext, cbf); }
                if (g == 3 && kTPW > 6) issue_next(6, false, cnext, snext, cbf);
            }
            __builtin_amdgcn_sched_barrier(0);
            const int px = g >> 1, hh = g & 1;
            const int pos = 12 * (px >> 1) + 3 * (px & 1);
            f32x4 bop = d2[px >> 1][px & 1][hh];
            if ((px >> 1) != (px & 1)) bop = -bop;
#pragma unroll
            for (int k = 0; k < 4; ++k)
#pragma unroll
                for (int j = 0; j < NCO; ++j)
                    acc[pos][j] = __builtin_amdgcn_mfma_f32_16x16x4f32(A1[hh][j][k], bop[k], acc[pos][j], 0, 0, 0);
            __builtin_amdgcn_sched_barrier(0);
        }
    };

    decode(t_cur);
    set_fetch_tile();
#pragma unroll
    for (int k = 0; k < kTPW; ++k) issue_next(k, false, 0, 0, 0);
    WINO_TRACE(tr_i++);
    asm volatile("s_waitcnt vmcnt(0)" ::: "memory");
    __syncthreads();
    WINO_TRACE(tr_i++);

    int it = 0;
#pragma unroll 1
    for (;;) {
        const int t_next = t_cur + t_stride;
        const bool has_next = t_next < t_end;
#pragma unroll
        for (int p = 0; p < 16; ++p)
#pragma unroll
            for (int j = 0; j < NCO; ++j) acc[p][j] = (f32x4){0.f, 0.f, 0.f, 0.f};

        const int n0 = 16 * cb0;
        const __amdgpu_buffer_rsrc_t rsO = __builtin_amdgcn_make_buffer_rsrc(a.out + (size_t)img * a.Ho * a.Wo * a.out_cs, 0, a.Ho * a.Wo * a.out_cs * 4, 0x00020000);
        const __amdgpu_buffer_rsrc_t rsR = __builtin_amdgcn_make_buffer_rsrc(const_cast<float *>(a.res ? a.res + (size_t)img * a.Ho * a.Wo * a.res_cs : a.out), 0,
                                                                              a.res ? a.Ho * a.Wo * a.res_cs * 4 : 0, 0x00020000);
        const __amdgpu_buffer_rsrc_t rsB = __builtin_amdgcn_make_buffer_rsrc(const_cast<float *>(a.bias ? a.bias : a.out), 0, a.bias ? a.Cout * 4 : 0, 0x00020000);
        f32x4 b4[NCO];
        const int ey0 = y0, ex0 = x0;

        set_fetch_tile2();
        const int cb_cur = cb0;
        const int nT = nS + nS2;
#pragma unroll 1
        for (int c = 0; c < nT; ++c) {
            const bool last = c + 1 == nT;
            if (last) {
#pragma unroll
                for (int i = 0; i < 2; ++i)
#pragma unroll
                    for (int j = 0; j < 2; ++j) {
                        const int oy = y0 + 2 * wave + i, ox = x0 + 2 * n + j;
                        const bool ok = (oy < a.Ho) & (ox < a.Wo);
                        const int voffR = ok ? ((oy * a.Wo + ox) * a.res_cs + n0 + 4 * h) * 4 : kOob;
#pragma unroll
                        for (int cb = 0; cb < NCO; ++cb) ost[i][j][cb] = __builtin_bit_cast(f32x4, __builtin_amdgcn_raw_buffer_load_b128(rsR, voffR + 64 * cb, 0, 0));
                    }
#pragma unroll
                for (int cb = 0; cb < NCO; ++cb) b4[cb] = __builtin_bit_cast(f32x4, __builtin_amdgcn_raw_buffer_load_b128(rsB, (n0 + 16 * cb + 4 * h) * 4, 0, 0));
                if (has_next) {
                    decode(t_next);
                    set_fetch_tile();
                }
            }
            const bool pnext = SRC2 && !last && c + 1 >= nS;
            const int cnext = last ? 0 : pnext ? c + 1 - nS : c + 1, sn = (it + 1) & 1;
            if (!SRC2 || c < nS) {
                compute(it & 1, pnext, cnext, sn, cb_cur, pending);
                pending = false;
            } else {
                compute_p(it & 1, pnext, cnext, sn, cb_cur);
            }
            ++it;
            WINO_TRACE(tr_i < 61 ? tr_i++ : 61);
            asm volatile("s_waitcnt vmcnt(0)" ::: "memory");
            __syncthreads();
            WINO_TRACE(tr_i < 61 ? tr_i++ : 61);
        }

        act_dispatch(a.act, a.slope, [&](auto fn) {
#pragma unroll
            for (int cb = 0; cb < NCO; ++cb) {
                f32x4 t[2][4];
#pragma unroll
                for (int nu = 0; nu < 4; ++nu) {
                    t[0][nu] = acc[0 + nu][cb] + acc[4 + nu][cb] + acc[8 + nu][cb];
                    t[1][nu] = acc[4 + nu][cb] - acc[8 + nu][cb] - acc[12 + nu][cb];
                }
#pragma unroll
                for (int i = 0; i < 2; ++i) {
                    f32x4 y[2];
                    y[0] = t[i][0] + t[i][1] + t[i][2];
                    y[1] = t[i][1] - t[i][2] - t[i][3];
#pragma unroll
                    for (int j = 0; j < 2; ++j) {
                        f32x4 o = y[j] + b4[cb] + ost[i][j][cb];
#pragma unroll
                        for (int r = 0; r < 4; ++r) o[r] = fn(o[r]);
#ifdef IDH_ABL_WINO_NOSTORE
                        asm volatile("" ::"v"(o));
#endif
                        ost[i][j][cb] = o;
                    }
                }
            }
        });
#pragma unroll
        for (int i = 0; i < 2; ++i)
#pragma unroll
            for (int j = 0; j < 2; ++j) {
                const int oy = ey0 + 2 * wave + i, ox = ex0 + 2 * n + j;
                voffS[i][j] = ((oy < a.Ho) & (ox < a.Wo)) ? ((oy * a.Wo + ox) * a.out_cs + n0 + 4 * h) * 4 : kOob;
            }
        rsS = rsO;
        pending = true;
        WINO_TRACE(tr_i < 61 ? tr_i++ : 61);
        if (!has_next) break;
        t_cur = t_next;
    }
#ifndef IDH_ABL_WINO_NOSTORE
#pragma unroll
    for (int k = 0; k < 4 * NCO; ++k)
        __builtin_amdgcn_raw_buffer_store_b128(__builtin_bit_cast(u32x4_t, ost[k >> 1 & 1][k & 1][k >> 2]), rsS, voffS[k >> 1 & 1][k & 1] + 64 * (k >> 2), 0, 0);
#endif
    WINO_TRACE(62);
}

template <int WAVES, int NCO, int CH, bool SRC2>
__global__ __launch_bounds__(64 * WAVES, 2) void conv3x3_wino_k(const WinoArgs wa) {
    __shared__ f32x4 lds[2 * wino_stage_slots<WAVES, NCO, CH, SRC2>()];
    wino_tiles<WAVES, NCO, CH, SRC2>(wa, lds, blockIdx.x, gridDim.x);
}

constexpr int kWinoMaxGroup = 6;
struct WinoGroupArgs {
    WinoArgs op[kWinoMaxGroup];
    int rot[kWinoMaxGroup];
    int n;
};
template <int WAVES, int NCO, int CH, bool SRC2>
__global__ __launch_bounds__(64 * WAVES, 2) void conv3x3_wino_group_k(const WinoGroupArgs g) {
    __shared__ f32x4 lds[2 * wino_stage_slots<WAVES, NCO, CH, SRC2>()];
    const unsigned per = gridDim.x >> 3;
    for (int i = 0; i < g.n; ++i) {
        const unsigned vblock = (((blockIdx.x >> 3) + per - (unsigned)g.rot[i] % per) % per) << 3 | (blockIdx.x & 7);
        wino_tiles<WAVES, NCO, CH, SRC2>(g.op[i], lds, vblock, gridDim.x);
        asm volatile("s_waitcnt vmcnt(0)" ::: "memory");
        __syncthreads();
    }
}

template <int WAVES, int NCO>
int wino_args(const ConvArgs &a, int N, WinoArgs &wa) {
    wa = WinoArgs{a, (a.Wo + kWinoTileW - 1) / kWinoTileW, (a.Ho + 2 * WAVES - 1) / (2 * WAVES), 0};
    wa.c.NT = a.Cout / (16 * NCO);
    const long long tiles = (long long)N * wa.tiles_x * wa.tiles_y * wa.c.NT;
    if (tiles >= (1ll << 31)) return IDH_EUNSUPPORTED;
    wa.tiles = (int)tiles;
    return IDH_OK;
}

template <int WAVES, int NCO, int CH, bool SRC2>
long long wino_resident() {
    static int resident = 0;
    if (resident == 0) {
        int dev = 0, cus = 256;
        if (hipGetDevice(&dev) == hipSuccess) (void)hipDeviceGetAttribute(&cus, hipDeviceAttributeMultiprocessorCount, dev);
        resident = cus > 0 ? cus : 256;
    }
    constexpr int kLdsBytes = 2 * wino_stage_slots<WAVES, NCO, CH, SRC2>() * 16;
    return (long long)resident * (kLdsBytes * 2 <= 160 * 1024 ? 2 : 1);
}

template <int WAVES, int NCO, int CH, bool SRC2>
int launch_wino(const ConvArgs &a, int N, hipStream_t st) {
    WinoArgs wa;
    if (int rc = wino_args<WAVES, NCO>(a, N, wa)) return rc;
    long long grid = wino_resident<WAVES, NCO, CH, SRC2>();
    if (grid > wa.tiles) grid = wa.tiles >= 8 ? wa.tiles / 8 * 8 : wa.tiles;
    hipLaunchKernelGGL((conv3x3_wino_k<WAVES, NCO, CH, SRC2>), dim3((unsigned)grid), dim3(64 * WAVES), 0, st, wa);
    IDH_CHECK_LAUNCH();
    return IDH_OK;
}

template <int WAVES, int NCO, int CH, bool SRC2>
int launch_wino_group(const ConvArgs *const *as, const int *Ns, int n, hipStream_t st) {
    WinoGroupArgs g{};
    long long total = 0;
    int rot = 0;
    const long long res = wino_resident<WAVES, NCO, CH, SRC2>();
    for (int i = 0; i < n; ++i) {
        if (int rc = wino_args<WAVES, NCO>(*as[i], Ns[i], g.op[i])) return rc;
        g.rot[i] = rot;
        rot = (int)((rot + (g.op[i].tiles + 7) / 8) % (res / 8));
        total += g.op[i].tiles;
    }
    g.n = n;
    long long grid = res;
    if (grid > total) grid = total >= 8 ? total / 8 * 8 : 8;
    if ((grid & 7) || (res & 7)) return IDH_EUNSUPPORTED;
    hipLaunchKernelGGL((conv3x3_wino_group_k<WAVES, NCO, CH, SRC2>), dim3((unsigned)grid), dim3(64 * WAVES), 0, st, g);
    IDH_CHECK_LAUNCH();
    return IDH_OK;
}

}

namespace idh_conv {

bool wino_supported(const ConvArgs &a) {
    const ConvSrc &s = a.s[0];
    const ConvSrc &s1 = a.s[1];
    const bool src2_ok = !s1.in || (s1.ks == 1 && s1.stride == 1 && !s1.up_in[0] && !s1.norm && s1.H == s.H && s1.W == s.W &&
                                    (long long)s1.H * s1.W * s1.cs * 4 < (1ll << 31) && (long long)s1.cblocks * a.Cout_pad * 64 < (1ll << 31));
    return s.ks == 3 && s.stride == 1 && s.pad_mode == IDH_PAD_ZEROS && !s.up_in[0] && !s.norm && src2_ok && a.S == 1 && (a.Cout % 32) == 0 &&
           (long long)s.H * s.W * s.cs * 4 < (1ll << 31) && (long long)a.Ho * a.Wo * a.out_cs * 4 < (1ll << 31) &&
           (!a.res || (long long)a.Ho * a.Wo * a.res_cs * 4 < (1ll << 31)) && (long long)s.cblocks * a.Cout_pad * 1024 < (1ll << 31);
}

int wino_max_group() { return kWinoMaxGroup; }

int launch_conv_wino_group(const ConvArgs *const *as, const int *Ns, int n, hipStream_t st) {
    if (n < 1 || n > kWinoMaxGroup) return IDH_EINVAL;
    const bool src2 = as[0]->s[1].in != nullptr;
    for (int i = 0; i < n; ++i)
        if (!wino_supported(*as[i]) || (as[i]->s[1].in != nullptr) != src2) return IDH_EUNSUPPORTED;
    return src2 ? launch_wino_group<4, 2, kWinoCH, true>(as, Ns, n, st) : launch_wino_group<4, 2, kWinoCH, false>(as, Ns, n, st);
}

int launch_conv_wino(const ConvArgs &a, int N, int rows, hipStream_t st) {
    if (!wino_supported(a)) return IDH_EUNSUPPORTED;
    (void)rows;
    return a.s[1].in ? launch_wino<4, 2, kWinoCH, true>(a, N, st) : launch_wino<4, 2, kWinoCH, false>(a, N, st);
}

}

extern "C" size_t idh_packed_wino_weight_floats(int Cout, int Cin) {
    if (Cout <= 0 || Cin <= 0) return 0;
    return (size_t)((Cin + 15) & ~15) * ((Cout + 15) & ~15) * 16;
}

extern "C" int idh_pack_conv_weight_wino(const float *w, float *dst, int Cout, int Cin, void *stream) {
    constexpr int ch = kWinoCH;
    if (!w || !dst || Cout <= 0 || Cin <= 0) return IDH_EINVAL;
    const int nC = (Cin + 15) / 16, nCB = (Cout + 15) / 16;
    const long long total = (long long)nC * nCB * 4096;
    int grid = idh_cdiv(total, 256);
    if (grid > 4096) grid = 4096;
    hipLaunchKernelGGL(pack_wino_weight_k, dim3(grid), dim3(256), 0, idh_stream(stream), w, dst, Cout, Cin, nC * (16 / ch), nCB, ch / 4);
    IDH_CHECK_LAUNCH();
    return IDH_OK;
}
```

implicit-depth_amd/csrc/networks.hip:

```cpp
#include <algorithm>
#include <cstring>
#include <map>
#include <tuple>
#include <vector>

#include "idh_common.h"
#include "net_plan.h"
#include "../../include/idh_net.h"
#include "../../include/idh_ops.h"

namespace {

constexpr long long kReuseMinBytes = 64ll << 20;
constexpr bool kFuseHeadNorm = true;
constexpr bool kFuseHeadImport = true;

inline int ceil16(int v) { return (v + 15) & ~15; }
inline int cdiv(int a, int b) { return (a + b - 1) / b; }
inline size_t align64(size_t v) { return (v + 63) & ~(size_t)63; }

__global__ __launch_bounds__(256) void bias_sum_k(const float *__restrict__ a, const float *__restrict__ b, float *__restrict__ out, int n) {
    const int i = blockIdx.x * 256 + threadIdx.x;
    if (i < n) out[i] = (a ? a[i] : 0.f) + (b ? b[i] : 0.f);
}

enum Mode { MODE_SIZES, MODE_PACK, MODE_RUN };

struct Buf {
    float *base;
    int N, H, W, cs;
    bool internal;
    bool zero_fill;
    size_t floats;
};

struct View {
    int buf = -1, c0 = 0, C = 0;
};

struct Region {
    uint64_t buf, c0, c1;
};

struct Meta {
    std::vector<Region> reads, writes;
};

struct Src {
    View v;
    const idh_conv_params *cv;
};

struct Norm {
    const float *stats = nullptr;
    int buf = -1;
    int act = IDH_ACT_NONE;
    float slope = 0.2f;
};

class Plan {
  public:
    Plan(Mode mode, float *ws, size_t ws_cap, float *blob, hipStream_t st) : mode_(mode), ws_(ws), ws_cap_(ws_cap), blob_(blob), st_(st) {
        if (mode_ != MODE_RUN) ws_ = reinterpret_cast<float *>(uintptr_t(1) << 32);
        if (mode_ == MODE_SIZES) blob_ = reinterpret_cast<float *>(uintptr_t(1) << 40);
    }

    int err = IDH_OK;
    std::vector<idh_op> ops;
    std::vector<Meta> meta;
    std::vector<Buf> bufs;
    size_t ws_off = 0, blob_off = 0;
    int n_wino4 = 0, n_wino2 = 0, recycled = 0;

    int N(const View &v) const { return bufs[v.buf].N; }
    int H(const View &v) const { return bufs[v.buf].H; }
    int W(const View &v) const { return bufs[v.buf].W; }
    int cs(const View &v) const { return bufs[v.buf].cs; }
    float *ptr(const View &v) const { return bufs[v.buf].base + v.c0; }
    static View slice(const View &v, int c0, int C) { return View{v.buf, v.c0 + c0, C}; }

    float *ws_alloc(size_t floats) {
        float *p = ws_ + ws_off;
        ws_off = align64(ws_off + floats);
        if (mode_ == MODE_RUN && ws_off > ws_cap_) err = IDH_EWORKSPACE;
        return p;
    }
    float *blob_alloc(size_t floats) {
        float *p = blob_ + blob_off;
        blob_off = align64(blob_off + floats);
        return p;
    }

    View buffer(int n, int h, int w, int c) {
        const int cs_ = ceil16(c);
        if (dry_) return phantom(n, h, w, c, cs_);
        if (cs_ == c) {
            auto it = free_.find(std::make_tuple(n, h, w, cs_));
            if (it != free_.end() && !it->second.empty()) {
                const int b = it->second.back();
                it->second.pop_back();
                ++recycled;
                return View{b, 0, c};
            }
        }
        Buf b{};
        b.N = n; b.H = h; b.W = w; b.cs = cs_; b.internal = true; b.zero_fill = cs_ != c;
        b.floats = (size_t)n * h * w * cs_;
        b.base = ws_alloc(b.floats);
        bufs.push_back(b);
        return View{(int)bufs.size() - 1, 0, c};
    }
    View phantom(int n, int h, int w, int c, int cs_) {
        Buf b{};
        b.N = n; b.H = h; b.W = w; b.cs = cs_; b.internal = false; b.zero_fill = false;
        b.base = reinterpret_cast<float *>((uintptr_t(7) << 32) + ((uintptr_t)bufs.size() << 24));
        bufs.push_back(b);
        return View{(int)bufs.size() - 1, 0, c};
    }
    View external(const idh_tensor &t, int n) {
        Buf b{};
        b.N = n; b.H = t.H; b.W = t.W; b.cs = t.cs; b.internal = false; b.zero_fill = false;
        b.base = mode_ == MODE_RUN ? t.ptr : reinterpret_cast<float *>((uintptr_t(2) << 32) + ((uintptr_t)bufs.size() << 24));
        bufs.push_back(b);
        return View{(int)bufs.size() - 1, 0, t.C};
    }
    void release(const View &v) {
        const Buf &b = bufs[v.buf];
        if (!b.internal || v.c0 != 0 || v.C != b.cs || (long long)b.floats * 4 < kReuseMinBytes) return;
        auto &pool = free_[std::make_tuple(b.N, b.H, b.W, b.cs)];
        if (std::find(pool.begin(), pool.end(), v.buf) != pool.end()) { err = IDH_EINVAL; return; }
        pool.push_back(v.buf);
    }

    static Region region(const View &v, bool pad16 = false) { return Region{(uint64_t)v.buf, (uint64_t)v.c0, (uint64_t)(v.c0 + (pad16 ? ceil16(v.C) : v.C))}; }

    int select(const std::vector<Src> &srcs, const View &out, int act, float slope, const View *res, int pad_mode, bool norm, bool any_size,
               idh_conv_choice *c) const {
        idh_conv_desc d{};
        d.N = N(out); d.Ho = H(out); d.Wo = W(out); d.Cout = srcs[0].cv->cout; d.pad_mode = pad_mode; d.act = act; d.slope = slope;
        d.out_cs = cs(out); d.has_res = res != nullptr; d.res_cs = res ? cs(*res) : 0; d.has_norm = norm; d.any_size = any_size;
        d.n_src = (int)srcs.size();
        for (size_t i = 0; i < srcs.size(); ++i) {
            const View &v = srcs[i].v;
            d.src[i] = idh_conv_desc_src{H(v), W(v), cs(v), srcs[i].cv->cin, srcs[i].cv->ks, srcs[i].cv->stride, 0, 0};
        }
        return idh_conv_select(&d, nullptr, c);
    }

    const float *packed(const idh_conv_params &cv, int lay) {
        size_t n = 0;
        if (lay == IDH_W_WINO4) n = idh_packed_wino4_weight_floats(cv.cout, cv.cin);
        else if (lay == IDH_W_WINO) n = idh_packed_wino_weight_floats(cv.cout, cv.cin);
        else n = idh_packed_weight_floats(cv.cout, cv.cin, cv.ks);
        float *dst = blob_alloc(n);
        if (mode_ == MODE_PACK) {
            if (!cv.weight) { err = IDH_EINVAL; return dst; }
            int rc;
            if (lay == IDH_W_WINO4) rc = idh_pack_conv_weight_wino4(cv.weight, dst, cv.cout, cv.cin, st_);
            else if (lay == IDH_W_WINO) rc = idh_pack_conv_weight_wino(cv.weight, dst, cv.cout, cv.cin, st_);
            else rc = idh_pack_conv_weight(cv.weight, dst, cv.cout, cv.cin, cv.ks, st_);
            if (rc != IDH_OK) err = rc;
        }
        return dst;
    }
    const float *bias_of(const idh_conv_params &a, const idh_conv_params *b) {
        float *dst = blob_alloc(a.cout);
        if (mode_ == MODE_PACK) {
            hipLaunchKernelGGL(bias_sum_k, dim3(cdiv(a.cout, 256)), dim3(256), 0, st_, a.bias, b ? b->bias : nullptr, dst, a.cout);
            if (hipGetLastError() != hipSuccess) err = IDH_ELAUNCH;
        }
        return dst;
    }

    View conv(const View &x, const idh_conv_params &cv, const View &out, int act, float slope, const View *res, const View *x2, const idh_conv_params *cv2,
              int pad_mode = IDH_PAD_ZEROS, const Norm *norm = nullptr, bool wino4_any_size = false) {
        if (err) return out;
        idh_op op;
        std::memset(&op, 0, sizeof op);
        op.kind = IDH_OP_CONV;
        op.N = N(x);
        std::vector<Src> srcs{{x, &cv}};
        if (x2) srcs.push_back({*x2, cv2});
        const int n = N(out), Ho = H(out), Wo = W(out), cout = cv.cout;
        if (out.C != cout) { err = IDH_EINVAL; return out; }
        idh_conv_choice ch;
        if ((err = select(srcs, out, act, slope, res, pad_mode, norm != nullptr, wino4_any_size, &ch)) != IDH_OK) return out;
        for (size_t i = 0; i < srcs.size(); ++i) {
            const View &v = srcs[i].v;
            const idh_conv_params &c = *srcs[i].cv;
            if (v.C != c.cin || (c.ks != 1 && c.ks != 3) || c.cout != cout) { err = IDH_EINVAL; return out; }
            if (v.C % 16 && (v.c0 != 0 || cs(v) != ceil16(v.C))) { err = IDH_EINVAL; return out; }
            idh_conv_src &s = op.src[i];
            s.in = ptr(v); s.w = packed(c, i == 0 ? ch.w_layout : IDH_W_DIRECT); s.cs = cs(v); s.H = H(v); s.W = W(v); s.Cin = v.C;
            s.ks = c.ks; s.stride = c.stride; s.pad_mode = pad_mode;
        }
        op.bias = bias_of(cv, cv2);
        if (res) { op.res = ptr(*res); op.res_cs = cs(*res); }
        op.out = ptr(out); op.out_cs = cs(out);
        op.Ho = Ho; op.Wo = Wo; op.Cout = cout;
        op.act = act; op.slope = slope;
        const long long M = (long long)n * Ho * Wo;
        const int tm = ch.tile_m, tn = ch.tile_n, split = ch.split_k;
        n_wino4 += tm == IDH_TILE_WINO4 && !dry_;
        n_wino2 += tm == IDH_TILE_WINO && !dry_;
        op.tile_m = tm; op.tile_n = tn; op.split_k = split;
        if (norm) {
            if ((tm != 8 && tm != 9) || tn != 1 || x2) { err = IDH_EINVAL; return out; }
            op.src[0].norm = norm->stats; op.src[0].norm_act = norm->act; op.src[0].norm_slope = norm->slope;
        }
        if (dry_) return out;
        if (split > 1) op.ws = ws_alloc((size_t)split * M * ceil16(cout));
        ops.push_back(op);
        Meta m;
        if (res) m.reads.push_back(region(*res));
        if (norm) m.reads.push_back(Region{(uint64_t)norm->buf, 0, 1});
        for (const Src &s : srcs) m.reads.push_back(region(s.v, true));
        m.writes.push_back(region(out));
        meta.push_back(m);
        return out;
    }
    void upsample2(const View &x, const View &out) {
        if (err) return;
        idh_op op;
        std::memset(&op, 0, sizeof op);
        op.kind = IDH_OP_UPSAMPLE2; op.N = N(x);
        idh_conv_src &s = op.src[0];
        s.in = ptr(x); s.cs = cs(x); s.H = H(x); s.W = W(x); s.Cin = x.C;
        op.out = ptr(out); op.out_cs = cs(out);
        ops.push_back(op);
        meta.push_back(Meta{{region(x)}, {region(out)}});
    }
    void import_nchw(const float *src, int n, int C, int H_, int W_, const View &out) {
        if (err) return;
        if (n != N(out) || H_ != H(out) || W_ != W(out) || C != out.C) { err = IDH_EINVAL; return; }
        idh_op op;
        std::memset(&op, 0, sizeof op);
        op.kind = IDH_OP_NCHW_TO_NHWC; op.N = n;
        op.src[0].in = mode_ == MODE_RUN ? src : reinterpret_cast<const float *>(uintptr_t(3) << 32);
        op.src[0].H = H_; op.src[0].W = W_; op.src[0].Cin = C;
        op.out = ptr(out); op.out_cs = cs(out);
        ops.push_back(op);
        meta.push_back(Meta{{}, {region(out)}});
    }
    void export_nchw(const View &x, float *dst) {
        if (err) return;
        idh_op op;
        std::memset(&op, 0, sizeof op);
        op.kind = IDH_OP_NHWC_TO_NCHW; op.N = N(x);
        idh_conv_src &s = op.src[0];
        s.in = ptr(x); s.cs = cs(x); s.H = H(x); s.W = W(x); s.Cin = x.C;
        op.out = mode_ == MODE_RUN ? dst : reinterpret_cast<float *>(uintptr_t(4) << 32);
        ops.push_back(op);
        meta.push_back(Meta{{region(x)}, {}});
    }
    void head(const View &x, const idh_conv_params &cv, float *out, float *out_exp) {
        if (err) return;
        if (cv.cout != 1 || cv.ks != 1 || cv.cin != x.C) { err = IDH_EINVAL; return; }
        float *w = blob_alloc(cv.cin), *b = blob_alloc(1);
        if (mode_ == MODE_PACK) {
            if (!cv.weight || !cv.bias) { err = IDH_EINVAL; return; }
            if (hipMemcpyAsync(w, cv.weight, sizeof(float) * cv.cin, hipMemcpyDeviceToDevice, st_) != hipSuccess ||
                hipMemcpyAsync(b, cv.bias, sizeof(float), hipMemcpyDeviceToDevice, st_) != hipSuccess) err = IDH_ELAUNCH;
        }
        idh_op op;
        std::memset(&op, 0, sizeof op);
        op.kind = IDH_OP_POINTWISE_HEAD; op.N = N(x);
        idh_conv_src &s = op.src[0];
        s.in = ptr(x); s.w = w; s.cs = cs(x); s.H = H(x); s.W = W(x); s.Cin = x.C;
        op.bias = b;
        op.out = mode_ == MODE_RUN ? out : reinterpret_cast<float *>(uintptr_t(5) << 32);
        op.ws = mode_ == MODE_RUN ? out_exp : nullptr;
        ops.push_back(op);
        meta.push_back(Meta{{region(x)}, {}});
    }

    Norm instance_norm(const View &x, const View *out, int act, float slope) {
        Norm nm;
        if (err) return nm;
        if (x.C % 4 || 256 % (x.C / 4)) { err = IDH_EINVAL; return nm; }
        const int nchunks = cdiv(H(x) * W(x), 1024);
        float *w = ws_alloc((size_t)N(x) * (nchunks + 1) * 2 * x.C);
        idh_op op;
        std::memset(&op, 0, sizeof op);
        op.kind = IDH_OP_INSTNORM; op.N = N(x);
        idh_conv_src &s = op.src[0];
        s.in = ptr(x); s.cs = cs(x); s.H = H(x); s.W = W(x); s.Cin = x.C;
        op.act = act; op.slope = slope;
        if (out) { op.out = ptr(*out); op.out_cs = cs(*out); }
        op.ws = w;
        ops.push_back(op);
        Meta m{{region(x)}, {}};
        if (out) {
            m.writes.push_back(region(*out));
        } else {
            Buf b{};
            b.base = w + (size_t)N(x) * nchunks * 2 * x.C; b.N = N(x); b.H = 1; b.W = 1; b.cs = 1; b.internal = false;
            bufs.push_back(b);
            nm.stats = b.base; nm.buf = (int)bufs.size() - 1;
            m.writes.push_back(Region{(uint64_t)nm.buf, 0, 1});
        }
        meta.push_back(m);
        return nm;
    }
    static bool pointwise_nchw_eligible(const idh_conv_params &c) { return c.ks == 1 && c.stride == 1 && c.cin == 64 && c.cout == 128; }
    void pointwise_nchw(const float *src, int n, int C, int H_, int W_, const idh_conv_params &cv, const View &out) {
        if (err) return;
        if (n != N(out) || H_ != H(out) || W_ != W(out) || C != cv.cin || out.C != cv.cout || !pointwise_nchw_eligible(cv)) { err = IDH_EINVAL; return; }
        idh_op op;
        std::memset(&op, 0, sizeof op);
        op.kind = IDH_OP_POINTWISE_NCHW; op.N = n;
        idh_conv_src &s = op.src[0];
        s.in = mode_ == MODE_RUN ? src : reinterpret_cast<const float *>(uintptr_t(6) << 32);
        s.w = packed(cv, IDH_W_DIRECT); s.H = H_; s.W = W_; s.Cin = C; s.ks = 1; s.stride = 1;
        op.bias = bias_of(cv, nullptr);
        op.out = ptr(out); op.out_cs = cs(out); op.Ho = H_; op.Wo = W_; op.Cout = cv.cout;
        ops.push_back(op);
        meta.push_back(Meta{{}, {region(out)}});
    }

    void stem(const float *images, int n, int h, int w, const float *blob, const View &out) {
        if (err) return;
        idh_op op;
        std::memset(&op, 0, sizeof op);
        op.kind = IDH_OP_STEM; op.N = n;
        idh_conv_src &s = op.src[0];
        s.in = mode_ == MODE_RUN ? images : reinterpret_cast<const float *>(uintptr_t(3) << 32);
        s.w = blob; s.H = h; s.W = w; s.Cin = 3;
        s.up_C = n; s.up_cs[0] = 3 * h * w; s.up_cs[1] = n * 3 * h * w;
        op.out = ptr(out); op.out_cs = cs(out); op.Ho = H(out); op.Wo = W(out); op.Cout = 64;
        ops.push_back(op);
        meta.push_back(Meta{{}, {region(out)}});
    }

    View basic_block(const View &x, const idh_block_params &blk, const View *out_opt = nullptr) {
        const int st = blk.conv1.stride;
        if (st != 1 && st != 2) { err = IDH_EINVAL; return x; }
        const int Ho = (H(x) + 2 - 3) / st + 1, Wo = (W(x) + 2 - 3) / st + 1;
        const int planes = blk.conv1.cout;
        const View h = buffer(N(x), Ho, Wo, planes);
        conv(x, blk.conv1, h, IDH_ACT_LRELU, 0.2f, nullptr, nullptr, nullptr);
        const View out = out_opt ? *out_opt : buffer(N(x), Ho, Wo, planes);
        if (H(out) != Ho || W(out) != Wo) { err = IDH_EINVAL; return out; }
        if (blk.downsample.ks == 0) {
            if (x.C != planes || st != 1) { err = IDH_EINVAL; return out; }
            conv(h, blk.conv2, out, IDH_ACT_LRELU, 0.2f, &x, nullptr, nullptr);
        } else {
            conv(h, blk.conv2, out, IDH_ACT_LRELU, 0.2f, nullptr, &x, &blk.downsample);
        }
        release(h);
        return out;
    }

    void reserve_block(const View &x, const idh_block_params &blk, int out_cs) {
        dry_ = true;
        if (out_cs) {
            const int st = blk.conv1.stride == 2 ? 2 : 1;
            const View o = phantom(N(x), (H(x) + 2 - 3) / st + 1, (W(x) + 2 - 3) / st + 1, blk.conv1.cout, out_cs);
            basic_block(x, blk, &o);
        } else {
            basic_block(x, blk);
        }
        dry_ = false;
    }

    int schedule(int n_first = 0) {
        std::vector<Region> flat;
        std::vector<int32_t> offs{0};
        for (const Meta &m : meta)
            for (const std::vector<Region> *rs : {&m.reads, &m.writes}) {
                flat.insert(flat.end(), rs->begin(), rs->end());
                offs.push_back((int32_t)flat.size());
            }
        flat.push_back(Region{});
        return idh_schedule_ops(ops.data(), (int)ops.size(), n_first, &flat[0].buf, offs.data(), IDH_SCHED_MERGE_LEVELS | IDH_SCHED_WINO_GROUP, nullptr, nullptr);
    }

    int finish(idh_net_sizes *sizes, int n_first = 0) {
        if (err || (err = schedule(n_first)) != IDH_OK) return err;
        if (sizes) {
            sizes->workspace_floats = ws_off;
            sizes->weight_floats = blob_off;
            sizes->ops = (int)ops.size();
            sizes->launches = idh_count_launches(ops.data(), (int)ops.size());
            sizes->wino4 = n_wino4; sizes->wino2 = n_wino2; sizes->recycled = recycled;
            if (sizes->launches < 0) return sizes->launches;
        }
        if (mode_ == MODE_RUN) {
            if (ws_off > ws_cap_) return IDH_EWORKSPACE;
            for (const Buf &b : bufs)
                if (b.internal && b.zero_fill && hipMemsetAsync(b.base, 0, b.floats * sizeof(float), st_) != hipSuccess) return IDH_ELAUNCH;
            int rc = n_first ? idh_run_ops(ops.data(), n_first, st_) : IDH_OK;
            if (rc == IDH_OK && before_run) rc = before_run(before_ctx);
            return rc != IDH_OK ? rc : idh_run_ops(ops.data() + n_first, (int)ops.size() - n_first, st_);
        }
        return IDH_OK;
    }

    Mode mode() const { return mode_; }
    hipStream_t stream() const { return st_; }
    int (*before_run)(void *) = nullptr;
    void *before_ctx = nullptr;

  private:
    Mode mode_;
    float *ws_;
    size_t ws_cap_;
    float *blob_;
    hipStream_t st_;
    bool dry_ = false;
    std::map<std::tuple<int, int, int, int>, std::vector<int>> free_;
};

bool tensor_ok(const idh_tensor *t, bool need_ptr, bool read = true) {
    if (!t || t->C <= 0 || t->H <= 0 || t->W <= 0) return false;
    if (t->layout != IDH_LAYOUT_NHWC && t->layout != IDH_LAYOUT_NCHW) return false;
    if (t->layout == IDH_LAYOUT_NHWC && (t->cs < t->C || (t->cs & 3) || (read && (t->C & 15) && t->cs != ceil16(t->C)))) return false;
    if (need_ptr && (!t->ptr || ((uintptr_t)t->ptr & 15))) return false;
    return true;
}

View input_view(Plan &p, const idh_tensor &t, int N) {
    if (t.layout == IDH_LAYOUT_NHWC) return p.external(t, N);
    const View v = p.buffer(N, t.H, t.W, t.C);
    p.import_nchw(t.ptr, N, t.C, t.H, t.W, v);
    return v;
}
View output_view(Plan &p, const idh_tensor &t, int N) {
    if (t.layout == IDH_LAYOUT_NHWC) return p.external(t, N);
    return p.buffer(N, t.H, t.W, t.C);
}
void output_done(Plan &p, const idh_tensor &t, const View &v) {
    if (t.layout == IDH_LAYOUT_NCHW) p.export_nchw(v, t.ptr);
}

int build_basic_block(Plan &p, const idh_block_params *blk, int N, const idh_tensor *x, const idh_tensor *out) {
    const bool run = p.mode() == MODE_RUN;
    if (!blk || N <= 0 || !tensor_ok(x, run) || !tensor_ok(out, run, false) || x->C != blk->conv1.cin || out->C != blk->conv1.cout) return IDH_EINVAL;
    const View xin = input_view(p, *x, N);
    const View o = output_view(p, *out, N);
    p.basic_block(xin, *blk, &o);
    output_done(p, *out, o);
    return p.err;
}

int build_matching_stem(Plan &p, const idh_stem_params *sp, int N, const idh_tensor *img, const idh_tensor *out) {
    const bool run = p.mode() == MODE_RUN;
    if (!sp || N <= 0 || !img || img->layout != IDH_LAYOUT_NCHW || img->C != 3 || img->H < 8 || img->W < 8 || (run && !img->ptr)) return IDH_EINVAL;
// ... 367 lines not shown
```

implicit-depth_amd/csrc/plan_select.hip:

```cpp
#include <algorithm>
#include <array>
#include <vector>

#include "../../include/idh.h"
#include "../../include/idh_ops.h"

namespace {

typedef long long i64;
inline int ceil16(int v) { return (v + 15) & ~15; }
inline i64 cdiv(i64 a, i64 b) { return (a + b - 1) / b; }
inline int lds_subtiles(int cout) { return cout % 64 == 0 ? 4 : (cout % 32 == 0 ? 2 : 1); }

struct Shape {
    const idh_conv_desc &d;
    const idh_conv_tuning &t;
    const idh_conv_desc_src &s0, &s1;
    bool two;

    bool plain3(int cout_mult, bool cat_ok) const {
        if (s0.ks != 3 || s0.stride != 1 || d.pad_mode != IDH_PAD_ZEROS || d.Cout % cout_mult || (!cat_ok && s0.is_cat)) return false;
        return !two || (s1.ks == 1 && s1.stride == 1 && (cat_ok || !s1.is_cat));
    }
    bool wino_grid(int ch, double min_fill, int min_tiles) const {
        const i64 ty = cdiv(d.Ho, 8), tx = cdiv(d.Wo, 32);
        if ((double)((i64)d.Ho * d.Wo) < min_fill * (ty * 8) * (tx * 32)) return false;
        return d.N * ty * tx * (d.Cout / ch) >= min_tiles;
    }
    bool wino() const { return plain3(32, false) && wino_grid(32, t.wino_min_fill, t.wino_min_tiles); }
    bool wino4() const {
        if (!plain3(64, false) || (two && !t.winograd4_proj)) return false;
        if ((d.act != IDH_ACT_NONE && d.act != IDH_ACT_LRELU && d.act != IDH_ACT_ELU) || (d.act == IDH_ACT_LRELU && !(d.slope >= 0.f && d.slope <= 1.f))) return false;
        if (s0.Cin <= 16) return false;
        if ((i64)s0.H * s0.W * s0.cs * 4 >= (1ll << 30)) return false;
        if ((i64)d.Ho * d.Wo * d.out_cs * 4 >= (1ll << 31) || (d.has_res && (i64)d.Ho * d.Wo * d.res_cs * 4 >= (1ll << 31))) return false;
        if (two && ((i64)s1.H * s1.W * s1.cs * 4 >= (1ll << 31) || (i64)((s1.Cin + 15) / 16) * 4 * ceil16(d.Cout) * 64 >= (1ll << 31))) return false;
        if ((i64)((s0.Cin + 15) / 16) * 4 * ceil16(d.Cout) * 36 * 16 * 4 >= (1ll << 31)) return false;
        return d.any_size || wino_grid(64, t.wino4_min_fill, t.wino4_min_tiles);
    }
    bool split() const {
        if (!plain3(64, true) || d.Wo < 16 || d.Ho < 8) return false;
        return d.N * cdiv(d.Ho, 8) * cdiv(d.Wo, 16) * (d.Cout / 64) >= t.split_min_blocks;
    }
    bool lds() const {
        if (s0.ks != 3 || s0.stride != 1 || d.Cout % 16 || d.Wo < 16) return false;
        if (d.pad_mode != IDH_PAD_ZEROS && (d.pad_mode != IDH_PAD_REPLICATE || two)) return false;
        if (!two || (s1.ks == 1 && s1.stride == 1)) return true;
        return s1.ks == 3 && s1.stride == 2 && d.pad_mode == IDH_PAD_ZEROS && d.Cout % 32 == 0 && !s1.is_cat;
    }
    bool s2_first() const {
        if (!t.s2_first || two || s0.ks != 3 || s0.stride != 2 || d.pad_mode != IDH_PAD_ZEROS || d.Cout % 32 || d.Wo < 16 || s0.is_cat) return false;
        return d.N * cdiv(d.Wo, 16) * cdiv(d.Ho, 4) * (d.Cout / (16 * lds_subtiles(d.Cout))) >= t.s2_first_min_blocks;
    }

    int split_rows() const {
        auto eff = [&](int rows, double bonus) {
            const i64 ty = cdiv(d.Ho, rows), blocks = d.N * ty * cdiv(d.Wo, 16) * (d.Cout / 64);
            return bonus * ((double)d.Ho / (double)(ty * rows)) * std::min(1.0, blocks / 768.0);
        };
        return d.Ho >= 16 && eff(16, 1.0) >= eff(8, 0.93) ? 16 : 8;
    }
    void lds_tile(int &code, int &split) const {
        double chunks = 0;
        for (int i = 0; i <= (int)two; ++i) chunks += (ceil16(d.src[i].Cin) / 16) * (d.src[i].ks == 3 ? 1.0 : t.proj_chunk_weight);
        const i64 per_row = d.N * cdiv(d.Wo, 16) * (d.Cout / (16 * lds_subtiles(d.Cout)));
        const bool rows4 = per_row * cdiv(d.Ho, 8) < 768;
        code = rows4 ? 9 : 8;
        const i64 blocks = per_row * cdiv(d.Ho, rows4 ? 4 : 8);
        split = (int)std::max<i64>(1, std::min<i64>({cdiv(768, blocks), (int)chunks / t.split_min_chunks, t.split_max}));
    }
    void direct_tile(int &tm, int &tn, int &split) const {
        int steps = 0;
        for (int i = 0; i <= (int)two; ++i) steps += d.src[i].ks * d.src[i].ks * (ceil16(d.src[i].Cin) / 16);
        const i64 M = (i64)d.N * d.Ho * d.Wo;
        const int nsub = ceil16(d.Cout) / 16;
        tn = nsub % 4 == 0 ? 4 : (nsub % 2 == 0 ? 2 : 1);
        i64 waves = 0;
        for (int cand : {4, 2, 1}) {
            waves = cdiv(M, 16 * cand) * (nsub / tn);
            tm = cand;
            if (waves >= t.target_waves) break;
        }
        split = waves < t.min_waves ? (int)std::max<i64>(1, std::min<i64>({cdiv(t.min_waves, waves), steps / 4, 32})) : 1;
    }
};

void launch_rank(const idh_op &op, int flags, i64 r[3]) {
    const bool conv = op.kind == IDH_OP_CONV, merge = flags & IDH_SCHED_MERGE_LEVELS;
    r[0] = 3; r[1] = 0; r[2] = 0;
    if ((flags & IDH_SCHED_WINO_GROUP) && conv && op.tile_m == IDH_TILE_WINO) { r[0] = -1; r[1] = op.src[1].in ? 1 : 0; r[2] = -(i64)op.N * op.Ho * op.Wo * op.Cout; }
    else if (conv && op.tile_m == 9) { r[0] = 0; r[1] = op.tile_n; }
    else if (merge && conv && op.tile_m == 1 && op.tile_n == 4) { r[0] = 1; }
    else if (merge && op.kind == IDH_OP_UPSAMPLE2) { r[0] = 2; }
    else if (merge && op.kind == IDH_OP_NCHW_TO_NHWC) { r[0] = 2; r[1] = 1; }
}

}

extern "C" void idh_conv_tuning_defaults(idh_conv_tuning *t) {
    if (t) *t = idh_conv_tuning{1, 1, 1, 1, 128, 768, 256, 400, 0, 6, 16, 512, 4, 2048, 1024, 0, 0.74, 0.85, 0.5};
}

extern "C" void idh_sizeof_conv_select(size_t out[3]) {
    if (out) { out[0] = sizeof(idh_conv_desc); out[1] = sizeof(idh_conv_tuning); out[2] = sizeof(idh_conv_choice); }
}

extern "C" int idh_conv_select(const idh_conv_desc *desc, const idh_conv_tuning *tuning, idh_conv_choice *out) {
    idh_conv_tuning def;
    idh_conv_tuning_defaults(&def);
    const idh_conv_tuning &t = tuning ? *tuning : def;
    if (!desc || !out || desc->n_src < 1 || desc->n_src > 2 || desc->N <= 0 || desc->Ho <= 0 || desc->Wo <= 0 || desc->Cout <= 0) return IDH_EINVAL;
    if ((desc->math != 0 && desc->math != IDH_SPLIT_F16X3) || desc->out_cs < 0 || desc->res_cs < 0 || t.split_min_chunks < 1) return IDH_EINVAL;
    for (int i = 0; i < desc->n_src; ++i) {
        const idh_conv_desc_src &s = desc->src[i];
        if ((s.ks != 1 && s.ks != 3) || s.stride < 1 || s.Cin < 0 || s.H < 0 || s.W < 0 || s.cs < 0) return IDH_EINVAL;
    }
    const idh_conv_desc &d = *desc;
    const Shape s{d, t, d.src[0], d.src[1], d.n_src == 2};
    const bool fp32 = d.math == 0, cat = d.src[0].is_cat || (s.two && d.src[1].is_cat);
    idh_conv_choice c{};
    c.families = (s.wino() ? IDH_FAMILY_WINO : 0) | (s.wino4() ? IDH_FAMILY_WINO4 : 0) | (s.split() ? IDH_FAMILY_SPLIT : 0) | (s.lds() ? IDH_FAMILY_LDS : 0) |
                 (s.s2_first() ? IDH_FAMILY_S2_FIRST : 0);
    c.lds_subtiles = lds_subtiles(d.Cout);
    if (d.Cout % 16 == 0) s.lds_tile(c.lds_tile_m, c.lds_split_k);
    c.split_rows = s.split_rows();
    s.direct_tile(c.direct_tile_m, c.direct_tile_n, c.direct_split_k);
    const bool plain = fp32 && !d.has_norm;
    c.split_k = 1;
    if (!fp32 && (c.families & IDH_FAMILY_SPLIT)) {
        c.w_layout = IDH_W_SPLIT; c.tile_m = d.math; c.tile_n = c.split_rows;
    } else if (plain && t.winograd4 && (!s.two || !d.has_res) && (c.families & IDH_FAMILY_WINO4)) {
        c.w_layout = IDH_W_WINO4; c.tile_m = IDH_TILE_WINO4;
    } else if (plain && t.winograd && (c.families & IDH_FAMILY_WINO)) {
        c.w_layout = IDH_W_WINO; c.tile_m = IDH_TILE_WINO;
    } else if (c.families & IDH_FAMILY_LDS) {
        c.tile_m = c.lds_tile_m == 8 && t.fused_up_rows == 4 && cat ? 9 : c.lds_tile_m;
        c.tile_n = c.lds_subtiles;
        c.split_k = c.lds_split_k;
        if (c.tile_n == 4 && c.tile_m == 9 && t.narrow_tile_below && !cat) {
            const i64 blocks64 = d.N * cdiv(d.Ho, 4) * cdiv(d.Wo, 16) * (d.Cout / 64) * c.split_k;
            if (blocks64 < t.narrow_tile_below) c.tile_n = blocks64 < t.narrowest_tile_below ? 1 : 2;
        }
        c.tile_n = c.tile_n == 4 ? 0 : c.tile_n;
    } else if (plain && (c.families & IDH_FAMILY_S2_FIRST)) {
        c.tile_m = c.lds_tile_m; c.split_k = c.lds_split_k;
        c.tile_n = c.lds_subtiles == 4 ? 0 : c.lds_subtiles;
    } else {
        c.tile_m = c.direct_tile_m; c.tile_n = c.direct_tile_n; c.split_k = c.direct_split_k;
    }
    *out = c;
    return IDH_OK;
}

extern "C" int idh_schedule_ops(idh_op *ops, int n, int n_first, const uint64_t *regions, const int32_t *offsets, int flags, int32_t *order, int32_t *levels) {
    if (n < 0 || (n > 0 && (!ops || !regions || !offsets))) return IDH_EINVAL;
    for (int k = 0; k < 2 * n; ++k)
        if (offsets[k] < 0 || offsets[k + 1] < offsets[k]) return IDH_EINVAL;
    n_first = std::max(0, std::min(n_first, n));
    auto overlap = [&](int a0, int a1, int b0, int b1) {
        for (int a = a0; a < a1; ++a)
            for (int b = b0; b < b1; ++b) {
                const uint64_t *x = regions + 3 * (size_t)a, *y = regions + 3 * (size_t)b;
                if (x[0] == y[0] && x[1] < y[2] && y[1] < x[2]) return true;
            }
        return false;
    };
    std::vector<int> level(n, 0), perm(n);
    std::vector<std::array<i64, 6>> key(n);
    for (int j = 0; j < n; ++j) {
        const int32_t *oj = offsets + 2 * j;
        for (int i = j < n_first ? 0 : n_first; i < j; ++i) {
            const int32_t *oi = offsets + 2 * i;
            if (overlap(oi[1], oi[2], oj[0], oj[1]) || overlap(oi[1], oi[2], oj[1], oj[2]) || overlap(oi[0], oi[1], oj[1], oj[2])) level[j] = std::max(level[j], level[i] + 1);
        }
        i64 r[3];
        launch_rank(ops[j], flags, r);
        key[j] = {j < n_first ? 0 : 1, level[j], r[0], r[1], r[2], j};
        ops[j].group = r[0] < 3 ? level[j] + 1 : 0;
        perm[j] = j;
    }
    std::sort(perm.begin(), perm.end(), [&](int a, int b) { return key[a] < key[b]; });
    const std::vector<idh_op> built(ops, ops + n);
    for (int k = 0; k < n; ++k) {
        ops[k] = built[perm[k]];
        if (order) order[k] = perm[k];
        if (levels) levels[k] = level[perm[k]];
    }
    return IDH_OK;
}
```

implicit-depth_amd/nhwc.py:

```python
from __future__ import annotations

import ctypes as C
from dataclasses import dataclass
from typing import Dict, List, Optional, Sequence

import torch
from torch import nn

from . import _lib

OP_CONV, OP_UPSAMPLE2, OP_IMPORT, OP_EXPORT, OP_SPLITK, OP_HEAD, OP_INSTNORM, OP_UPSAMPLE2_NEAREST, OP_COPY, OP_POINTWISE_NCHW, OP_POINTWISE_UP = 1, 2, 3, 4, 5, 6, 7, 8, 9, 10, 11
OP_STEM = 12
ACT_NONE, ACT_LRELU, ACT_ELU = 0, 1, 2
PAD_ZEROS, PAD_REPLICATE = 0, 1


class ConvSrc(C.Structure):
    _fields_ = [("in_", C.c_void_p), ("w", C.c_void_p), ("cs", C.c_int32), ("H", C.c_int32), ("W", C.c_int32),
                ("Cin", C.c_int32), ("ks", C.c_int32), ("stride", C.c_int32), ("pad_mode", C.c_int32), ("_r", C.c_int32),
                ("up_in", C.c_void_p * 2), ("up_cs", C.c_int32 * 2), ("up_c0", C.c_int32), ("up_C", C.c_int32),
                ("norm", C.c_void_p), ("norm_slope", C.c_float), ("norm_act", C.c_int32)]


class Op(C.Structure):
    _fields_ = [("kind", C.c_int32), ("N", C.c_int32), ("src", ConvSrc * 2), ("bias", C.c_void_p), ("res", C.c_void_p),
                ("out", C.c_void_p), ("ws", C.c_void_p), ("res_cs", C.c_int32), ("out_cs", C.c_int32), ("Ho", C.c_int32),
                ("Wo", C.c_int32), ("Cout", C.c_int32), ("act", C.c_int32), ("slope", C.c_float), ("split_k", C.c_int32),
                ("tile_m", C.c_int32), ("tile_n", C.c_int32), ("group", C.c_int32)]


def _bind():
    return _lib.lib()


@dataclass
class View:

    buf: torch.Tensor
    c0: int
    C: int

    @property
    def N(self):
        return self.buf.shape[0]

    @property
    def H(self):
        return self.buf.shape[1]

    @property
    def W(self):
        return self.buf.shape[2]

    @property
    def cs(self):
        return self.buf.shape[3]

    @property
    def ptr(self):
        return self.buf.data_ptr() + 4 * self.c0

    def slice(self, c0, C):
        return View(self.buf, self.c0 + c0, C)

    def dense(self) -> torch.Tensor:
        return self.buf[..., self.c0 : self.c0 + self.C]


@dataclass
class CatView:

    direct: View
    ups: List[View]

    @property
    def N(self):
        return self.direct.N

    @property
    def H(self):
        return self.direct.H

    @property
    def W(self):
        return self.direct.W

    @property
    def C(self):
        return self.direct.C + sum(u.C for u in self.ups)


def ceil16(v: int) -> int:
    return (v + 15) & ~15


def _region(v: "View", pad16: bool = False):
    return (v.buf.data_ptr(), v.c0, v.c0 + (ceil16(v.C) if pad16 else v.C))


def packed_weight(conv: nn.Conv2d) -> torch.Tensor:
    w = conv.weight
    key = (w.data_ptr(), _lib.param_version(w), str(w.device))
    cached = getattr(conv, "_idh_packed", None)
    if cached is not None and cached[0] == key:
        return cached[1]
    _lib.require_cuda_f32(w)
    L = _bind()
    co, ci, kh, kw = w.shape
    if kh != kw or kh not in (1, 3):
        raise _lib.IdhError(f"conv kernel {kh}x{kw} not covered by the gfx950 conv kernel (1x1 / 3x3 only)")
    n = L.idh_packed_weight_floats(co, ci, kh)
    dst = torch.empty(n, device=w.device, dtype=torch.float32)
    wc = w.detach().contiguous()
    _lib.check(L.idh_pack_conv_weight(wc.data_ptr(), dst.data_ptr(), co, ci, kh, _lib.stream_ptr()), "idh_pack_conv_weight")
    conv._idh_packed = (key, dst)
    return dst


def packed_wino_weight(conv: nn.Conv2d) -> torch.Tensor:
    w = conv.weight
    key = (w.data_ptr(), _lib.param_version(w), str(w.device))
    cached = getattr(conv, "_idh_packed_wino", None)
    if cached is not None and cached[0] == key:
        return cached[1]
    _lib.require_cuda_f32(w)
    L = _bind()
    co, ci, kh, kw = w.shape
    if (kh, kw) != (3, 3):
        raise _lib.IdhError("the Winograd F(2x2,3x3) kernel covers 3x3 convolutions only")
    dst = torch.empty(L.idh_packed_wino_weight_floats(co, ci), device=w.device, dtype=torch.float32)
    wc = w.detach().contiguous()
    _lib.check(L.idh_pack_conv_weight_wino(wc.data_ptr(), dst.data_ptr(), co, ci, _lib.stream_ptr()), "idh_pack_conv_weight_wino")
    conv._idh_packed_wino = (key, dst)
    return dst


def packed_wino4_weight(conv: nn.Conv2d) -> torch.Tensor:
    w = conv.weight
    key = (w.data_ptr(), _lib.param_version(w), str(w.device))
    cached = getattr(conv, "_idh_packed_wino4", None)
    if cached is not None and cached[0] == key:
        return cached[1]
    _lib.require_cuda_f32(w)
    L = _bind()
    co, ci, kh, kw = w.shape
    if (kh, kw) != (3, 3):
        raise _lib.IdhError("the Winograd F(4x4,3x3) kernel covers 3x3 convolutions only")
    dst = torch.empty(L.idh_packed_wino4_weight_floats(co, ci), device=w.device, dtype=torch.float32)
    wc = w.detach().contiguous()
    _lib.check(L.idh_pack_conv_weight_wino4(wc.data_ptr(), dst.data_ptr(), co, ci, _lib.stream_ptr()), "idh_pack_conv_weight_wino4")
    conv._idh_packed_wino4 = (key, dst)
    return dst


TILE_WINO = 12
TILE_WINO4 = 13
WINOGRAD = True
WINO_MIN_TILES = 128
WINO_MIN_FILL = 0.74
WINO_GROUP = True


def wino_eligible(srcs, cout: int, N: int, Ho: int, Wo: int, pad_mode: int) -> bool:
    return bool(select(srcs, cout, N, Ho, Wo, pad_mode).families & FAMILY_WINO)


BUFFER_REUSE = True
REUSE_MIN_BYTES = 64 << 20
WINOGRAD4 = True
WINOGRAD4_PROJ = True
WINO4_MIN_TILES = 768
WINO4_MIN_FILL = 0.85


def wino4_eligible(srcs, cout: int, N: int, Ho: int, Wo: int, pad_mode: int, act: int, out=None, res=None, slope: float = 0.2, any_size: bool = False) -> bool:
    return bool(select(srcs, cout, N, Ho, Wo, pad_mode, act, slope, out, res, any_size=any_size).families & FAMILY_WINO4)


SPLIT_CODE = {"f16x3": 11}


def split_packed_weight(conv: nn.Conv2d, math: str, proj: Optional[nn.Conv2d] = None) -> torch.Tensor:
    w = conv.weight
    w1 = proj.weight if proj is not None else None
    key = (w.data_ptr(), _lib.param_version(w), str(w.device), math) + ((w1.data_ptr(), _lib.param_version(w1)) if w1 is not None else ())
    cached = getattr(conv, "_idh_packed_split", None)
    if cached is not None and cached[0] == key:
        return cached[1]
    _lib.require_cuda_f32(w)
    L = _bind()
    co, ci, kh, kw = w.shape
    ci1 = 0
    w1c = None
    if w1 is not None:
        _lib.require_cuda_f32(w1)
        if tuple(w1.shape[2:]) != (1, 1) or w1.shape[0] != co:
            raise _lib.IdhError("the fused second source of a split-precision conv must be a 1x1 conv with the same Cout")
        ci1 = w1.shape[1]
        w1c = w1.detach().reshape(co, ci1).contiguous()
    n = L.idh_packed_split_weight_bytes(co, ci, ci1, SPLIT_CODE[math])
    if kh != 3 or kw != 3 or n == 0:
        raise _lib.IdhError("split-precision conv covers 3x3 kernels with Cout % 64 == 0")
    dst = torch.empty(n // 4, device=w.device, dtype=torch.int32)
    wc = w.detach().contiguous()
    _lib.check(L.idh_pack_conv_weight_split(wc.data_ptr(), _lib.ptr(w1c), dst.data_ptr(), co, ci, ci1, SPLIT_CODE[math], _lib.stream_ptr()),
               "idh_pack_conv_weight_split")
    conv._idh_packed_split = (key, dst)
    return dst


MATH_MODES = ("fp32", "f16x3")
DEFAULT_MATH = "fp32"
SPLIT_MIN_BLOCKS = 256


def split_eligible(srcs, cout: int, N: int, Ho: int, Wo: int, pad_mode: int) -> bool:
    return bool(select(srcs, cout, N, Ho, Wo, pad_mode).families & FAMILY_SPLIT)


def choose_split_rows(N: int, Ho: int, Wo: int, cout: int) -> int:
    return select([(None, _conv_shape(16, 3))], cout, N, Ho, Wo).split_rows


FUSE_UPSAMPLE = False
FUSED_UP_ROWS = 4

MERGE_LEVELS = True
FUSE_HEAD_NORM = True
FUSE_HEAD_IMPORT = True

TARGET_WAVES = 2048
MIN_WAVES = 1024


def lds_eligible(srcs, cout: int, Wo: int, pad_mode: int) -> bool:
    return bool(select(srcs, cout, 1, 1, Wo, pad_mode).families & FAMILY_LDS)


S2_FIRST = True
S2_FIRST_MIN_BLOCKS = 512


def s2_first_eligible(srcs, cout: int, N: int, Ho: int, Wo: int, pad_mode: int) -> bool:
    return bool(select(srcs, cout, N, Ho, Wo, pad_mode).families & FAMILY_S2_FIRST)


def lds_subtiles(cout: int) -> int:
    return select([(None, _conv_shape(16, 3))], cout, 1, 1, 1).lds_subtiles


NARROW_TILE_BELOW = 400
NARROWEST_TILE_BELOW = 0


SPLIT_MIN_CHUNKS = 6
SPLIT_MAX = 16
PROJ_LOWRES = False
PROJ_LOWRES_MIN_TILES = 1536
PROJ_CHUNK_WEIGHT = 0.5


def choose_lds_tile(N: int, Ho: int, Wo: int, cout: int, chunks: int):
    ch = select([(None, _conv_shape(16 * chunks, 3))], cout, N, Ho, Wo)
    return ch.lds_tile_m, ch.lds_split_k


def choose_tiles(M: int, cout: int, steps: int):
    ch = select([(None, _conv_shape(16 * steps, 1))], cout, 1, 1, M)
    return ch.direct_tile_m, ch.direct_tile_n, ch.direct_split_k


W_DIRECT, W_WINO, W_WINO4, W_SPLIT = 0, 1, 2, 3
FAMILY_WINO, FAMILY_WINO4, FAMILY_SPLIT, FAMILY_LDS, FAMILY_S2_FIRST = 1, 2, 4, 8, 16
SCHED_MERGE_LEVELS, SCHED_WINO_GROUP = 1, 2


def _conv_shape(cin: int, ks: int, stride: int = 1):
    import types

    return types.SimpleNamespace(in_channels=cin, kernel_size=(ks, ks), stride=(stride, stride))


def conv_tuning() -> "_lib.ConvTuning":
    return _lib.ConvTuning(WINOGRAD, WINOGRAD4, WINOGRAD4_PROJ, S2_FIRST, WINO_MIN_TILES, WINO4_MIN_TILES, SPLIT_MIN_BLOCKS, NARROW_TILE_BELOW,
                           NARROWEST_TILE_BELOW, SPLIT_MIN_CHUNKS, SPLIT_MAX, S2_FIRST_MIN_BLOCKS, FUSED_UP_ROWS, TARGET_WAVES, MIN_WAVES, 0,
                           WINO_MIN_FILL, WINO4_MIN_FILL, PROJ_CHUNK_WEIGHT)


def select(srcs, cout: int, N: int, Ho: int, Wo: int, pad_mode: int = PAD_ZEROS, act: int = ACT_NONE, slope: float = 0.2, out=None, res=None,
           norm: bool = False, any_size: bool = False, math: str = "fp32") -> "_lib.ConvChoice":
    d = _lib.ConvDesc(N, Ho, Wo, cout, pad_mode, act, slope, getattr(out, "cs", 0), getattr(res, "cs", 0), res is not None, norm, any_size,
                      SPLIT_CODE.get(math, 0), len(srcs))
    for s, (v, cv) in zip(d.src, srcs):
        s.H, s.W, s.cs, s.is_cat = getattr(v, "H", 0), getattr(v, "W", 0), getattr(v, "cs", 0), isinstance(v, CatView)
        s.Cin, s.ks, s.stride = getattr(cv, "in_channels", 0), cv.kernel_size[0], cv.stride[0]
    ch = _lib.ConvChoice()
    _lib.check(_bind().idh_conv_select(C.byref(d), C.byref(conv_tuning()), C.byref(ch)), "idh_conv_select")
    return ch


class Plan:

    def __init__(self, device, math: Optional[str] = None):
        self.device = device
        self.math = DEFAULT_MATH if math is None else math
        if self.math not in MATH_MODES:
            raise _lib.IdhError(f"unknown conv math mode {self.math!r} (expected one of {MATH_MODES})")
        self.ops: List[Op] = []
        self.meta: List[dict] = []
        self.keep: List[torch.Tensor] = []
        self._free: Dict[tuple, List[torch.Tensor]] = {}
        self.recycled_candidates = 0
        self.recycled = 0
        self._arr = None
        self._pos: Optional[List[int]] = None
        self.flops = 0

    def buffer(self, N, H, W, Cch) -> View:
        cs = ceil16(Cch)
        pool = self._free.get((N, H, W, cs)) if cs == Cch else None
        if pool:
            self.recycled += 1
            return View(pool.pop(), 0, Cch)
        alloc = torch.zeros if cs != Cch else torch.empty
        t = alloc(N, H, W, cs, device=self.device, dtype=torch.float32)
        self.keep.append(t)
        return View(t, 0, Cch)

    def release(self, v: View):
        t = v.buf
        if (BUFFER_REUSE and v.c0 == 0 and v.C == t.shape[-1] and t.dim() == 4 and t.numel() * 4 >= REUSE_MIN_BYTES
                and any(t is k for k in self.keep)):
            pool = self._free.setdefault(tuple(t.shape), [])
            if any(t is f for f in pool):
                raise _lib.IdhError("Plan.release: buffer released twice")
            pool.append(t)
            self.recycled_candidates += 1

    def conv(self, x: View, conv: nn.Conv2d, out: View, act=ACT_NONE, slope=0.2, res: Optional[View] = None,
             x2: Optional[View] = None, conv2: Optional[nn.Conv2d] = None, pad_mode=PAD_ZEROS, norm=None, wino4_any_size: bool = False):
        op = Op()
        op.kind = OP_CONV
        op.N = x.N
        srcs = [(x, conv)] + ([(x2, conv2)] if x2 is not None else [])
        for v, cv in srcs:
            if v.C != cv.in_channels:
                raise _lib.IdhError(f"conv expects {cv.in_channels} input channels, view has {v.C}")
        ch = select(srcs, conv.out_channels, out.N, out.H, out.W, pad_mode, act, slope, out, res, norm is not None, wino4_any_size, self.math)
        pack = (packed_weight, packed_wino_weight, packed_wino4_weight)
        for i, (v, cv) in enumerate(srcs):
            ks, st = cv.kernel_size[0], cv.stride[0]
            cat = v if isinstance(v, CatView) else None
            if cat is not None:
                if ch.w_layout == W_SPLIT or not ch.families & FAMILY_LDS or st != 1:
                    raise _lib.IdhError("a fused-upsample concat can only feed the LDS-staged fp32 conv kernel")
                if cat.direct.C % 16 or any(u.C != cat.ups[0].C or u.C % 16 or (2 * u.H, 2 * u.W) != (cat.H, cat.W) for u in cat.ups) or not 1 <= len(cat.ups) <= 2:
                    raise _lib.IdhError("fused-upsample concat: channel counts must be multiples of 16 and the maps exactly half size")
                v = cat.direct
            elif v.C % 16 and (v.c0 != 0 or v.cs != ceil16(v.C)):
                raise _lib.IdhError("a conv input whose channel count is not a multiple of 16 must be a whole zero-padded buffer")
            if ch.w_layout == W_SPLIT:
                w = split_packed_weight(conv, self.math, conv2)
            else:
                w = pack[ch.w_layout if i == 0 else W_DIRECT](cv)
            self.keep.append(w)
            s = op.src[i]
            cin = cat.C if cat is not None else v.C
            s.in_, s.w, s.cs, s.H, s.W, s.Cin = v.ptr, w.data_ptr(), v.cs, v.H, v.W, cin
            s.ks, s.stride, s.pad_mode = ks, st, pad_mode
            if cat is not None:
                s.up_c0, s.up_C = cat.direct.C, cat.ups[0].C
                for ui, u in enumerate(cat.ups):
                    s.up_in[ui], s.up_cs[ui] = u.ptr, u.cs
            self.flops += 2 * out.N * out.H * out.W * cv.out_channels * cv.in_channels * ks * ks
        bias = conv.bias
        if conv2 is not None and conv2.bias is not None:
            bias = (conv.bias + conv2.bias).detach() if conv.bias is not None else conv2.bias
        if bias is not None:
            bias = bias.detach().contiguous()
            self.keep.append(bias)
            op.bias = bias.data_ptr()
        if res is not None:
            op.res, op.res_cs = res.ptr, res.cs
        op.out, op.out_cs = out.ptr, out.cs
        op.Ho, op.Wo, op.Cout = out.H, out.W, conv.out_channels
        op.act, op.slope = act, slope
        M = out.N * out.H * out.W
        op.tile_m, op.tile_n, op.split_k = tm, tn, split = ch.tile_m, ch.tile_n, ch.split_k
        if norm is not None:
            stats, n_act, n_slope = norm
            if tm not in (8, 9) or tn != 1 or x2 is not None or isinstance(x, CatView) or tuple(stats.shape) != (x.N, 2, x.C):
                raise _lib.IdhError("normalise-on-load needs the LDS-staged fp32 conv with 16-channel tiles and one source")
            op.src[0].norm, op.src[0].norm_act, op.src[0].norm_slope = stats.data_ptr(), n_act, n_slope
        if split > 1:
            ws = torch.empty(split * M * ceil16(conv.out_channels), device=self.device, dtype=torch.float32)
            self.keep.append(ws)
            op.ws = ws.data_ptr()
        self.ops.append(op)
        reads = ([_region(res)] if res is not None else []) + ([(norm[0].data_ptr(), 0, 1)] if norm is not None else [])
        for v, _ in srcs:
            if isinstance(v, CatView):
                reads += [_region(v.direct)] + [_region(u) for u in v.ups]
            else:
                reads.append(_region(v, pad16=True))
        self.meta.append({"reads": reads, "writes": [_region(out)]})
        self._arr = None
        return out

    def upsample2(self, x: View, out: View, nearest: bool = False):
        op = Op()
        op.kind, op.N = (OP_UPSAMPLE2_NEAREST if nearest else OP_UPSAMPLE2), x.N
        s = op.src[0]
        s.in_, s.cs, s.H, s.W, s.Cin = x.ptr, x.cs, x.H, x.W, x.C
        op.out, op.out_cs = out.ptr, out.cs
        self.ops.append(op)
        self.meta.append({"reads": [_region(x)], "writes": [_region(out)]})
        self._arr = None
        return out

    def pointwise_up(self, x: View, conv: nn.Conv2d, low: View, out: View):
        if conv.kernel_size[0] != 1 or conv.in_channels != x.C or conv.out_channels != out.C or low.C != out.C or (2 * low.H, 2 * low.W) != (x.H, x.W):
            raise _lib.IdhError("pointwise_up: a 1x1 conv of x plus the x2 upsampling of a half-resolution map with the output's channels")
        op = Op()
        op.kind, op.N = OP_POINTWISE_UP, x.N
        w = packed_weight(conv)
        self.keep.append(w)
        s = op.src[0]
        s.in_, s.w, s.cs, s.H, s.W, s.Cin, s.ks, s.stride = x.ptr, w.data_ptr(), x.cs, x.H, x.W, x.C, 1, 1
        l = op.src[1]
        l.in_, l.cs, l.H, l.W, l.Cin = low.ptr, low.cs, low.H, low.W, low.C
        if conv.bias is not None:
            b = conv.bias.detach().contiguous()
            self.keep.append(b)
            op.bias = b.data_ptr()
        op.out, op.out_cs, op.Ho, op.Wo, op.Cout = out.ptr, out.cs, out.H, out.W, out.C
        self.flops += 2 * x.N * x.H * x.W * conv.out_channels * conv.in_channels
        self.ops.append(op)
        self.meta.append({"reads": [_region(x), _region(low)], "writes": [_region(out)]})
        self._arr = None
        return out

    def instance_norm(self, x: View, out: Optional[View], act=ACT_NONE, slope=0.2):
        if x.C % 4 or 256 % (x.C // 4):
            raise _lib.IdhError(f"instance-norm kernel needs C/4 to divide 256 (C={x.C})")
        op = Op()
        op.kind, op.N = OP_INSTNORM, x.N
        s = op.src[0]
        s.in_, s.cs, s.H, s.W, s.Cin = x.ptr, x.cs, x.H, x.W, x.C
        op.act, op.slope = act, slope
        if out is not None:
            op.out, op.out_cs = out.ptr, out.cs
        nchunks = -(-(x.H * x.W) // 1024)
        ws = torch.empty(x.N * (nchunks + 1) * 2 * x.C, device=self.device, dtype=torch.float32)
        self.keep.append(ws)
        op.ws = ws.data_ptr()
        self.ops.append(op)
        stats = ws[x.N * nchunks * 2 * x.C:].view(x.N, 2, x.C)
        self.meta.append({"reads": [_region(x)], "writes": [_region(out)] if out is not None else [(stats.data_ptr(), 0, 1)]})
        self._arr = None
        return out if out is not None else stats

    def copy(self, x: View, out: View):
        if (x.N, x.H, x.W, x.C) != (out.N, out.H, out.W, out.C):
            raise _lib.IdhError("copy: shape mismatch")
        op = Op()
        op.kind, op.N = OP_COPY, x.N
        s = op.src[0]
        s.in_, s.cs, s.H, s.W, s.Cin = x.ptr, x.cs, x.H, x.W, x.C
        op.out, op.out_cs = out.ptr, out.cs
        self.ops.append(op)
        self.meta.append({"reads": [_region(x)], "writes": [_region(out)]})
        self._arr = None
        return out

    def import_nchw(self, shape_nchw, out: View) -> int:
        N, Cc, H, W = [int(v) for v in shape_nchw]
        if (N, H, W, Cc) != (out.N, out.H, out.W, out.C):
            raise _lib.IdhError(f"import of {tuple(shape_nchw)} into a view of {(out.N, out.C, out.H, out.W)}")
        op = Op()
        op.kind, op.N = OP_IMPORT, N
        s = op.src[0]
        s.H, s.W, s.Cin = H, W, Cc
        op.out, op.out_cs = out.ptr, out.cs
        self.ops.append(op)
        self.meta.append({"reads": [], "writes": [_region(out)]})
        self._arr = None
        return len(self.ops) - 1

    @staticmethod
    def pointwise_nchw_eligible(conv: nn.Conv2d) -> bool:
        return (conv.kernel_size == (1, 1) and conv.stride == (1, 1) and conv.in_channels == 64 and conv.out_channels == 128
                and conv.groups == 1)

    def pointwise_nchw(self, shape_nchw, conv: nn.Conv2d, out: View) -> int:
        N, Cc, H, W = [int(v) for v in shape_nchw]
        if (N, H, W) != (out.N, out.H, out.W) or Cc != conv.in_channels or out.C != conv.out_channels or not self.pointwise_nchw_eligible(conv):
            raise _lib.IdhError(f"pointwise_nchw: {tuple(shape_nchw)} with {conv} into a view of {(out.N, out.C, out.H, out.W)}")
        op = Op()
        op.kind, op.N = OP_POINTWISE_NCHW, N
        s = op.src[0]
        w = packed_weight(conv)
        self.keep.append(w)
        s.w, s.H, s.W, s.Cin, s.ks, s.stride = w.data_ptr(), H, W, Cc, 1, 1
        if conv.bias is not None:
            bias = conv.bias.detach().contiguous()
            self.keep.append(bias)
            op.bias = bias.data_ptr()
        op.out, op.out_cs, op.Ho, op.Wo, op.Cout = out.ptr, out.cs, H, W, conv.out_channels
        self.flops += 2 * N * H * W * conv.out_channels * conv.in_channels
        self.ops.append(op)
        self.meta.append({"reads": [], "writes": [_region(out)]})
        self._arr = None
        return len(self.ops) - 1

    def stem(self, shape, strides, blob: torch.Tensor, out: View) -> int:
        N, Cc, H, W = [int(v) for v in shape]
        Ho, Wo = ((H + 1) // 2) // 2, ((W + 1) // 2) // 2
        if Cc != 3 or H < 8 or W < 8 or (out.N, out.H, out.W, out.C) != (N, Ho, Wo, 64):
            raise _lib.IdhError(f"stem: images {tuple(shape)} (3 channels, H, W >= 8) into a view of {(out.N, out.C, out.H, out.W)}")
        group, img_stride, grp_stride = [int(v) for v in strides]
        if max(img_stride, grp_stride) >= 1 << 31 or N % group:
            raise _lib.IdhError("stem: image strides must fit in 32 bits and the groups divide the batch")
        op = Op()
        op.kind, op.N = OP_STEM, N
        s = op.src[0]
        s.w, s.H, s.W, s.Cin = blob.data_ptr(), H, W, 3
        s.up_C, s.up_cs[0], s.up_cs[1] = group, img_stride, grp_stride
        self.keep.append(blob)
        op.out, op.out_cs, op.Ho, op.Wo, op.Cout = out.ptr, out.cs, Ho, Wo, 64
        self.flops += 2 * N * ((H + 1) // 2) * ((W + 1) // 2) * 64 * 147
        self.ops.append(op)
        self.meta.append({"reads": [], "writes": [_region(out)]})
        self._arr = None
        return len(self.ops) - 1

    def export_nchw(self, x: View, out_nchw: Optional[torch.Tensor] = None) -> int:
        op = Op()
        op.kind, op.N = OP_EXPORT, x.N
        s = op.src[0]
        s.in_, s.cs, s.H, s.W, s.Cin = x.ptr, x.cs, x.H, x.W, x.C
        if out_nchw is not None:
            op.out = out_nchw.data_ptr()
        self.ops.append(op)
        self.meta.append({"reads": [_region(x)], "writes": []})
        self._arr = None
        return len(self.ops) - 1

    def head(self, x: View, conv: nn.Conv2d, out: torch.Tensor):
        if conv.out_channels != 1 or conv.kernel_size != (1, 1):
            raise _lib.IdhError("pointwise head kernel covers Conv2d(C,1,1) only")
        op = Op()
        op.kind, op.N = OP_HEAD, x.N
        w = conv.weight.detach().reshape(-1).contiguous()
        b = conv.bias.detach().contiguous()
        self.keep += [w, b]
        s = op.src[0]
        s.in_, s.w, s.cs, s.H, s.W, s.Cin = x.ptr, w.data_ptr(), x.cs, x.H, x.W, x.C
        op.bias, op.out = b.data_ptr(), out.data_ptr()
        self.ops.append(op)
        self.meta.append({"reads": [_region(x)], "writes": []})
        self._arr = None
        return len(self.ops) - 1

    def basic_block(self, x: View, blk, out: Optional[View] = None) -> View:
        st = blk.conv1.stride[0]
        Ho = (x.H + 2 - 3) // st + 1
        Wo = (x.W + 2 - 3) // st + 1
        planes = blk.conv1.out_channels
        h = self.buffer(x.N, Ho, Wo, planes)
        self.conv(x, blk.conv1, h, act=ACT_LRELU, slope=0.2)
        if out is None:
            out = self.buffer(x.N, Ho, Wo, planes)
        if blk.downsample is None:
            self.conv(h, blk.conv2, out, act=ACT_LRELU, slope=0.2, res=x)
        elif (self.math != "fp32" and blk.downsample[0].kernel_size[0] == 3
              and split_eligible([(h, blk.conv2)], planes, x.N, Ho, Wo, PAD_ZEROS)):
            proj = self.buffer(x.N, Ho, Wo, planes)
            self.conv(x, blk.downsample[0], proj)
            self.conv(h, blk.conv2, out, act=ACT_LRELU, slope=0.2, res=proj)
        else:
            self.conv(h, blk.conv2, out, act=ACT_LRELU, slope=0.2, x2=x, conv2=blk.downsample[0])
        self.release(h)
        return out

    def basic_block_upcat(self, cat: View, lows: List[View], blk) -> Optional[View]:
        ds = blk.downsample[0] if blk.downsample is not None else None
        planes = blk.conv1.out_channels
        c = planes
        if (not PROJ_LOWRES or self.math != "fp32" or ds is None or ds.kernel_size[0] != 1 or ds.stride[0] != 1 or planes not in (64, 128) or
                not 1 <= len(lows) <= 2 or cat.C != c * (1 + len(lows)) or any(l.C != c or (2 * l.H, 2 * l.W) != (cat.H, cat.W) for l in lows)):
            return None
        if cat.N * (-(-cat.H // 8)) * (-(-cat.W // 32)) * (planes // 64) < PROJ_LOWRES_MIN_TILES:
            return None
        key = (ds.weight.data_ptr(), _lib.param_version(ds.weight), None if ds.bias is None else _lib.param_version(ds.bias), str(ds.weight.device))
        parts = getattr(ds, "_idh_proj_parts", None)
        if parts is None or parts[0] != key:
            with torch.no_grad():
                mods = []
# ... 612 lines not shown
```

include/idh_ops.h:

```cpp
#ifndef IDH_OPS_H_
#define IDH_OPS_H_

#include <stddef.h>
#include <stdint.h>

#ifdef __cplusplus
extern "C" {
#endif
#if defined(__GNUC__) || defined(__clang__)
#pragma GCC visibility push(default)
#endif

enum {
    IDH_OP_CONV = 1,
    IDH_OP_UPSAMPLE2 = 2,
    IDH_OP_NCHW_TO_NHWC = 3,
    IDH_OP_NHWC_TO_NCHW = 4,
    IDH_OP_SPLITK_REDUCE = 5,
    IDH_OP_POINTWISE_HEAD = 6,
    IDH_OP_COPY = 9,
    IDH_OP_UPSAMPLE2_NEAREST = 8,
    IDH_OP_POINTWISE_NCHW = 10,
    IDH_OP_POINTWISE_UP = 11,
    IDH_OP_STEM = 12,
    IDH_OP_INSTNORM = 7
};

#define IDH_PAD_ZEROS 0
#define IDH_PAD_REPLICATE 1

typedef struct idh_conv_src {
    const float *in;
    const float *w;
    int32_t cs, H, W, Cin;
    int32_t ks, stride, pad_mode, _r;
    const float *up_in[2];
    int32_t up_cs[2];
    int32_t up_c0, up_C;
    const float *norm;
    float norm_slope;
    int32_t norm_act;
} idh_conv_src;

typedef struct idh_op {
    int32_t kind;
    int32_t N;
    idh_conv_src src[2];
    const float *bias;
    const float *res;
    float *out;
    float *ws;
    int32_t res_cs, out_cs;
    int32_t Ho, Wo, Cout;
    int32_t act;
    float slope;
    int32_t split_k;
    int32_t tile_m, tile_n;
    int32_t group;
} idh_op;

size_t idh_packed_weight_floats(int Cout, int Cin, int ks);
int idh_pack_conv_weight(const float *w_oihw, float *dst, int Cout, int Cin, int ks, void *stream);

#define IDH_SPLIT_F16X3 11
size_t idh_packed_split_weight_bytes(int Cout, int Cin, int Cin_1x1, int mode);
int idh_pack_conv_weight_split(const float *w_oihw, const float *w_1x1, void *dst, int Cout, int Cin, int Cin_1x1, int mode,
                               void *stream);

#define IDH_TILE_WINO 12
size_t idh_packed_wino_weight_floats(int Cout, int Cin);
int idh_pack_conv_weight_wino(const float *w_oihw, float *dst, int Cout, int Cin, void *stream);

#define IDH_TILE_WINO4 13
size_t idh_packed_wino4_weight_floats(int Cout, int Cin);
int idh_pack_conv_weight_wino4(const float *w_oihw, float *dst, int Cout, int Cin, void *stream);

size_t idh_stem_weight_floats(void);
int idh_pack_stem_weight(const float *w_oihw, const float *bn_weight, const float *bn_bias, const float *bn_mean, const float *bn_var, float eps,
                         float *dst, void *stream);
int idh_fold_conv_bn(const float *w, int cout, int per_out, const float *bn_weight, const float *bn_bias, const float *bn_mean,
                     const float *bn_var, float eps, float *w_out, float *b_out, void *stream);

size_t idh_sizeof_op(void);

int idh_run_ops(const idh_op *ops_host, int n, void *stream);

int idh_count_launches(const idh_op *ops_host, int n);

int idh_conv_variant(const idh_op *op, int32_t out[8]);

typedef struct idh_conv_desc_src {
    int32_t H, W, cs;
    int32_t Cin, ks, stride;
    int32_t is_cat, _r;
} idh_conv_desc_src;

typedef struct idh_conv_desc {
    int32_t N, Ho, Wo, Cout, pad_mode, act;
    float slope;
    int32_t out_cs, res_cs, has_res;
    int32_t has_norm;
    int32_t any_size;
    int32_t math;
    int32_t n_src;
    idh_conv_desc_src src[2];
} idh_conv_desc;

typedef struct idh_conv_tuning {
    int32_t winograd, winograd4, winograd4_proj, s2_first;
    int32_t wino_min_tiles, wino4_min_tiles, split_min_blocks, narrow_tile_below, narrowest_tile_below, split_min_chunks, split_max,
        s2_first_min_blocks, fused_up_rows, target_waves, min_waves, _r;
    double wino_min_fill, wino4_min_fill, proj_chunk_weight;
} idh_conv_tuning;
void idh_conv_tuning_defaults(idh_conv_tuning *t);

#define IDH_W_DIRECT 0
#define IDH_W_WINO 1
#define IDH_W_WINO4 2
#define IDH_W_SPLIT 3
#define IDH_FAMILY_WINO 1
#define IDH_FAMILY_WINO4 2
#define IDH_FAMILY_SPLIT 4
#define IDH_FAMILY_LDS 8
#define IDH_FAMILY_S2_FIRST 16

typedef struct idh_conv_choice {
    int32_t tile_m, tile_n, split_k;
    int32_t w_layout;
    int32_t families;
    int32_t lds_tile_m, lds_split_k, lds_subtiles, split_rows, direct_tile_m, direct_tile_n, direct_split_k;
} idh_conv_choice;

int idh_conv_select(const idh_conv_desc *desc, const idh_conv_tuning *tuning, idh_conv_choice *out);
void idh_sizeof_conv_select(size_t out[3]);

#define IDH_SCHED_MERGE_LEVELS 1
#define IDH_SCHED_WINO_GROUP 2
int idh_schedule_ops(idh_op *ops, int n, int n_first, const uint64_t *regions, const int32_t *offsets, int flags, int32_t *order, int32_t *levels);

#if defined(__GNUC__) || defined(__clang__)
#pragma GCC visibility pop
#endif
#ifdef __cplusplus
}
#endif
#endif
```

Measured before the change: 684.9.

## Add narrow 16x16 Winograd tile arrangement for convs with poor 32-wide fill

Adds a Winograd F(2,3) kernel variant that tiles outputs as 16 columns by 16 rows instead of 32 by 8. The halo layout, swizzle, patch addressing and output indexing are adjusted for the new shape. The selector picks it when the standard 32x8 grid fails the fill check but the narrow grid passes, so convs on narrow feature maps can use Winograd instead of a slower fallback. Narrow and wide convs are kept in separate launch groups, which may split existing groups and adds kernel instantiations.

Result: no change. 687.0, median of 6 (+0.3%).

```diff
diff --git a/implicit-depth_amd/_lib.py b/implicit-depth_amd/_lib.py
--- a/implicit-depth_amd/_lib.py
+++ b/implicit-depth_amd/_lib.py
@@ -105,7 +105,7 @@
 
 
 class ConvDescSrc(C.Structure):
-    _fields_ = [(n, C.c_int32) for n in ("H", "W", "cs", "Cin", "ks", "stride", "is_cat", "_r")]
+    _fields_ = [(n, C.c_int32) for n in ("H", "W", "cs", "Cin", "ks", "stride", "is_cat", "wino_narrow")]
 
 
 class ConvDesc(C.Structure):
diff --git a/implicit-depth_amd/csrc/conv.hip b/implicit-depth_amd/csrc/conv.hip
--- a/implicit-depth_amd/csrc/conv.hip
+++ b/implicit-depth_amd/csrc/conv.hip
@@ -1222,7 +1222,7 @@
         if (!wino_supported(a)) return IDH_EUNSUPPORTED;
         pc.lds_rows = 32;
         pc.tm = op.tile_m;
-        pc.tn = 0;
+        pc.tn = op.tile_n == IDH_WINO_NARROW ? IDH_WINO_NARROW : 0;
         pc.n_img = op.N;
         pc.blocks = 0;
     } else if (op.tile_m == IDH_TILE_WINO4) {
@@ -1291,7 +1291,7 @@
     }
     if (pc.lds_rows == 32) {
         if (t_dry_run) { ++t_launches; return IDH_OK; }
-        return launch_conv_wino(pc.a, pc.n_img, pc.tn, st);
+        return launch_conv_wino(pc.a, pc.n_img, pc.tn == IDH_WINO_NARROW, st);
     }
     if (pc.lds_rows == 36) {
         if (t_dry_run) { ++t_launches; return IDH_OK; }
@@ -1469,7 +1469,7 @@
                 if (op.kind == IDH_OP_CONV && pcs[0].lds_rows == 32) {
                     wg = 1;
                     while (wg < run && wg < wino_max_group() && ops[i + wg].kind == IDH_OP_CONV && pcs[wg].lds_rows == 32 &&
-                           (pcs[wg].a.s[1].in != nullptr) == (pcs[0].a.s[1].in != nullptr))
+                           (pcs[wg].a.s[1].in != nullptr) == (pcs[0].a.s[1].in != nullptr) && pcs[wg].tn == pcs[0].tn)
                         ++wg;
                 }
                 int rc, used;
@@ -1481,7 +1481,7 @@
                         const ConvArgs *as[kMaxGroup];
                         int ns[kMaxGroup];
                         for (int j = 0; j < wg; ++j) { as[j] = &pcs[j].a; ns[j] = pcs[j].n_img; }
-                        rc = launch_conv_wino_group(as, ns, wg, st);
+                        rc = launch_conv_wino_group(as, ns, wg, pcs[0].tn == IDH_WINO_NARROW, st);
                         if (rc == IDH_EUNSUPPORTED) {
                             rc = IDH_OK;
                             for (int j = 0; j < wg && rc == IDH_OK; ++j) rc = launch_conv(pcs[j], st);
diff --git a/implicit-depth_amd/csrc/conv_args.h b/implicit-depth_amd/csrc/conv_args.h
--- a/implicit-depth_amd/csrc/conv_args.h
+++ b/implicit-depth_amd/csrc/conv_args.h
@@ -57,9 +57,9 @@
 int launch_conv_split(const ConvArgs &a, int N, int mode, int rows, hipStream_t st);
 
 bool wino_supported(const ConvArgs &a);
-int launch_conv_wino(const ConvArgs &a, int N, int rows, hipStream_t st);
+int launch_conv_wino(const ConvArgs &a, int N, bool narrow, hipStream_t st);
 int wino_max_group();
-int launch_conv_wino_group(const ConvArgs *const *as, const int *Ns, int n, hipStream_t st);
+int launch_conv_wino_group(const ConvArgs *const *as, const int *Ns, int n, bool narrow, hipStream_t st);
 
 bool wino4_supported(const ConvArgs &a);
 int launch_conv_wino4(const ConvArgs &a, int N, hipStream_t st);
diff --git a/implicit-depth_amd/csrc/conv_wino.hip b/implicit-depth_amd/csrc/conv_wino.hip
--- a/implicit-depth_amd/csrc/conv_wino.hip
+++ b/implicit-depth_amd/csrc/conv_wino.hip
@@ -15,9 +15,8 @@
 constexpr int kWinoHalf = 17;
 constexpr int kOob = 0x7fffffff;
 
-constexpr int wino_plane(int WAVES) { return (2 * WAVES + 2) * 2 * kWinoHalf; }
-constexpr int wino_qs(int WAVES) { return (wino_plane(WAVES) + 63) / 64 * 64; }
-constexpr int wino_stage(int WAVES, int NCO) { return 4 * wino_qs(WAVES) + NCO * 1024; }
+constexpr int kWinoNarrowW = 16;
+constexpr int wino_plane(int WAVES, bool NARROW) { return NARROW ? (4 * WAVES + 2) * 2 * (kWinoNarrowW / 2 + 1) : (2 * WAVES + 2) * 2 * kWinoHalf; }
 
 __global__ __launch_bounds__(256) void pack_wino_weight_k(const float *__restrict__ w, float *__restrict__ dst, int Cout, int Cin, int nS, int nCB, int KS) {
     const long long total = (long long)nS * nCB * 16 * 64 * KS;
@@ -63,20 +62,22 @@
     int tiles;
 };
 
-template <int WAVES, int NCO, int CH, bool SRC2>
+template <int WAVES, int NCO, int CH, bool SRC2, bool NARROW>
 constexpr int wino_stage_slots() {
-    constexpr int halo = ((CH / 4) * wino_plane(WAVES) + 63) / 64 * 64;
+    constexpr int halo = ((CH / 4) * wino_plane(WAVES, NARROW) + 63) / 64 * 64;
     constexpr int s3 = halo + 64 * NCO * 4 * (CH / 4), sp = 8 * 32 * 2 * WAVES + 64 * 2 * NCO;
     return SRC2 && sp > s3 ? sp : s3;
 }
 
-template <int WAVES, int NCO, int CH, bool SRC2>
+template <int WAVES, int NCO, int CH, bool SRC2, bool NARROW>
 __device__ __forceinline__ void wino_tiles(const WinoArgs &wa, f32x4 *lds, const unsigned vblock, const unsigned vgrid) {
     constexpr int KS = CH / 4;
     constexpr int NP = CH / 4;
     typedef float vec __attribute__((ext_vector_type(KS)));
-    constexpr int kRows = 2 * WAVES;
-    constexpr int kPlane = wino_plane(WAVES);
+    constexpr int kRows = NARROW ? 4 * WAVES : 2 * WAVES;
+    constexpr int kTileW = NARROW ? kWinoNarrowW : kWinoTileW;
+    constexpr int kHalf = kTileW / 2 + 1;
+    constexpr int kPlane = wino_plane(WAVES, NARROW);
     static_assert(NP == 2, "halo swizzle written for 8-channel K steps");
     constexpr int kHaloPieces = (NP * kPlane + 63) / 64;
     constexpr int kHP = (kHaloPieces + WAVES - 1) / WAVES;
@@ -87,17 +88,19 @@
     static_assert(CH == 8, "K steps of 8 channels: every tile has >= 2 steps (the first stores the previous tile's outputs, the last loads the residual)");
     static_assert(kTPW <= 8 && 4 * NCO <= 8, "one DMA piece per even position group, one output store per odd group");
     constexpr int kHalo = 64 * kHaloPieces;
-    constexpr int kTight = 32 * kRows;
+    constexpr int kTight = kTileW * kRows;
     constexpr int kStage3 = kHalo + 64 * kPanelPieces;
     constexpr int kStageP = 8 * kTight + 64 * 2 * NCO;
     constexpr int kStage = SRC2 && kStageP > kStage3 ? kStageP : kStage3;
-    static_assert(kStage == wino_stage_slots<WAVES, NCO, CH, SRC2>(), "stage size used by the kernels' LDS declaration");
+    static_assert(kStage == wino_stage_slots<WAVES, NCO, CH, SRC2, NARROW>(), "stage size used by the kernels' LDS declaration");
 
     const ConvArgs &a = wa.c;
     const ConvSrc &s = a.s[0];
     const int lane = threadIdx.x & 63;
     const int wave = __builtin_amdgcn_readfirstlane(threadIdx.x >> 6);
     const int n = lane & 15, h = lane >> 4;
+    const int tcol = NARROW ? n & 7 : n, trow = NARROW ? n >> 3 : 0;
+    constexpr int kWaveRows = kRows / WAVES;
 #ifdef IDH_ABL_WINO_TRACE
     unsigned long long *trace = reinterpret_cast<unsigned long long *>(a.ws) + ((size_t)blockIdx.x * WAVES + wave) * 64;
     int tr_i = 1;
@@ -127,7 +130,7 @@
         const int tx = blk % wa.tiles_x; blk /= wa.tiles_x;
         const int ty = blk % wa.tiles_y;
         img = blk / wa.tiles_y;
-        y0 = ty * kRows; x0 = tx * kWinoTileW; cb0 = nt * NCO;
+        y0 = ty * kRows; x0 = tx * kTileW; cb0 = nt * NCO;
     };
     BufRef rsA;
     int voffH[kHP], panel_so;
@@ -135,8 +138,8 @@
     auto halo_piece = [&](int k) { return wave + WAVES * k < kHaloPieces ? wave + WAVES * k : wave; };
     auto halo_voff = [&](int j, int lane) {
         const int pt = 32 * j + (lane >> 1);
-        const int row = pt / kWinoHalf, hxh = pt - row * kWinoHalf;
-        const int q = (lane & 1) ^ ((hxh >> 3) & 1);
+        const int row = pt / kHalf, hxh = pt - row * kHalf;
+        const int q = (lane & 1) ^ (NARROW ? (row >> 2) & 1 : (hxh >> 3) & 1);
         const int iy = y0 - 1 + (row >> 1), ix = x0 - 1 + 2 * hxh + (row & 1);
         const bool ok = (pt < kPlane) & ((unsigned)iy < (unsigned)s.H) & ((unsigned)ix < (unsigned)s.W);
         return ok ? (iy * s.W + ix) * s.cs * 4 + 16 * q : kOob;
@@ -190,9 +193,9 @@
             bool halo1 = true;
             if (k < 8) {
                 const int t = 8 * wave + k;
-                const int plane = (lane & 7) ^ ((4 * (t & 1) + (lane >> 4)) & 7);
+                const int plane = (lane & 7) ^ ((4 * (NARROW ? (t >> 2) & 1 : t & 1) + (lane >> 4)) & 7);
                 vo1 = (plane >= 4 && 2 * c + 1 >= s1.cblocks) ? kOob : voffT + 16 * plane;
-                so1 = tile2_so + (((t >> 2) * s1.W + 16 * (t & 1) + ((t >> 1) & 1)) * s1.cs + 32 * c) * 4;
+                so1 = tile2_so + ((NARROW ? (t >> 1) * s1.W + (t & 1) : (t >> 2) * s1.W + 16 * (t & 1) + ((t >> 1) & 1)) * s1.cs + 32 * c) * 4;
                 lo1 = 64 * t;
             } else {
                 const int hh = wave / NCO, cbw = wave % NCO;
@@ -217,7 +220,7 @@
     bool pending = false;
 
     const int pq = (KS * h) >> 2, pb8 = ((KS * h) & 3) * 4;
-    const int patch0 = (NP * ((4 * wave) * kWinoHalf + n) + (pq ^ ((n >> 3) & 1))) * 16 + pb8;
+    const int patch0 = (NP * ((2 * kWaveRows * wave + 4 * trow) * kHalf + tcol) + (pq ^ (NARROW ? trow : (n >> 3) & 1))) * 16 + pb8;
     const int frag0 = kHalo * 16 + (h * 16 + n) * (4 * KS);
 
     constexpr int kAhead = CH == 16 ? 2 : 3;
@@ -226,7 +229,8 @@
         typedef const __attribute__((address_space(3))) volatile vec lds_cvec;
         int n_o = n;
         asm volatile("" : "+v"(n_o));
-        const int patch1 = patch0 + (NP + ((pq ^ (((n_o + 1) >> 3) & 1)) - (pq ^ ((n_o >> 3) & 1)))) * 16;
+        const int patch1 = NARROW ? patch0 + ((pq ^ ((n_o >> 3) ^ 1)) - (pq ^ (n_o >> 3))) * 16
+                                  : patch0 + (NP + ((pq ^ (((n_o + 1) >> 3) & 1)) - (pq ^ ((n_o >> 3) & 1)))) * 16;
         lds_cchar *sH0 = (lds_cchar *)(lds + stage * kStage) + patch0, *sH1 = (lds_cchar *)(lds + stage * kStage) + patch1;
         lds_cchar *sW = (lds_cchar *)(lds + stage * kStage) + frag0;
         vec d[4][4], A[kAhead + 1][NCO], r[4];
@@ -237,7 +241,9 @@
         };
         auto rd_row = [&](int y) {
 #pragma unroll
-            for (int x = 0; x < 4; ++x) d[y][x] = *(lds_cvec *)(((x >> 1) ? sH1 : sH0) + NP * (2 * y + (x & 1)) * kWinoHalf * 16);
+            for (int x = 0; x < 4; ++x)
+                d[y][x] = NARROW ? *(lds_cvec *)(((y >> 1) ? sH1 : sH0) + NP * ((2 * y + (x & 1)) * kHalf + (x >> 1)) * 16)
+                                 : *(lds_cvec *)(((x >> 1) ? sH1 : sH0) + NP * (2 * y + (x & 1)) * kHalf * 16);
         };
         rd_frag(0);
         rd_row(1);
@@ -296,7 +302,7 @@
         int ln_o = lane;
         asm volatile("" : "+v"(ln_o));
         const int n_o = ln_o & 15, h_o = ln_o >> 4;
-        const f32x4 *sH = lds + stage * kStage + 8 * ((4 * wave) * 16 + n_o);
+        const f32x4 *sH = lds + stage * kStage + 8 * ((4 * wave) * 16 + n_o + (NARROW ? 24 * (n_o >> 3) : 0));
         const int x0s = h_o ^ ((n_o >> 1) & 7);
         const f32x4 *sW = lds + stage * kStage + 8 * kTight + ln_o;
         f32x4 d2[2][2][2], A1[2][NCO];
@@ -309,7 +315,7 @@
 #pragma unroll
             for (int j = 0; j < 2; ++j)
 #pragma unroll
-                for (int hh = 0; hh < 2; ++hh) d2[i][j][hh] = sH[8 * 16 * (2 * i + j) + (x0s ^ (4 * hh))];
+                for (int hh = 0; hh < 2; ++hh) d2[i][j][hh] = sH[8 * (kTileW / 2) * (2 * i + j) + (x0s ^ (4 * hh))];
 #pragma unroll
         for (int g = 0; g < 8; ++g) {
             if (pnext) {
@@ -371,7 +377,7 @@
                 for (int i = 0; i < 2; ++i)
 #pragma unroll
                     for (int j = 0; j < 2; ++j) {
-                        const int oy = y0 + 2 * wave + i, ox = x0 + 2 * n + j;
+                        const int oy = y0 + kWaveRows * wave + 2 * trow + i, ox = x0 + 2 * tcol + j;
                         const bool ok = (oy < a.Ho) & (ox < a.Wo);
                         const int voffR = ok ? ((oy * a.Wo + ox) * a.res_cs + n0 + 4 * h) * 4 : kOob;
 #pragma unroll
@@ -430,7 +436,7 @@
         for (int i = 0; i < 2; ++i)
 #pragma unroll
             for (int j = 0; j < 2; ++j) {
-                const int oy = ey0 + 2 * wave + i, ox = ex0 + 2 * n + j;
+                const int oy = ey0 + kWaveRows * wave + 2 * trow + i, ox = ex0 + 2 * tcol + j;
                 voffS[i][j] = ((oy < a.Ho) & (ox < a.Wo)) ? ((oy * a.Wo + ox) * a.out_cs + n0 + 4 * h) * 4 : kOob;
             }
         rsS = rsO;
@@ -449,8 +455,13 @@
 
 template <int WAVES, int NCO, int CH, bool SRC2>
 __global__ __launch_bounds__(64 * WAVES, 2) void conv3x3_wino_k(const WinoArgs wa) {
-    __shared__ f32x4 lds[2 * wino_stage_slots<WAVES, NCO, CH, SRC2>()];
-    wino_tiles<WAVES, NCO, CH, SRC2>(wa, lds, blockIdx.x, gridDim.x);
+    __shared__ f32x4 lds[2 * wino_stage_slots<WAVES, NCO, CH, SRC2, false>()];
+    wino_tiles<WAVES, NCO, CH, SRC2, false>(wa, lds, blockIdx.x, gridDim.x);
+}
+template <int WAVES, int NCO, int CH, bool SRC2>
+__global__ __launch_bounds__(64 * WAVES, 2) void conv3x3_wino_narrow_k(const WinoArgs wa) {
+    __shared__ f32x4 lds[2 * wino_stage_slots<WAVES, NCO, CH, SRC2, true>()];
+    wino_tiles<WAVES, NCO, CH, SRC2, true>(wa, lds, blockIdx.x, gridDim.x);
 }
 
 constexpr int kWinoMaxGroup = 6;
@@ -459,21 +470,31 @@
     int rot[kWinoMaxGroup];
     int n;
 };
-template <int WAVES, int NCO, int CH, bool SRC2>
-__global__ __launch_bounds__(64 * WAVES, 2) void conv3x3_wino_group_k(const WinoGroupArgs g) {
-    __shared__ f32x4 lds[2 * wino_stage_slots<WAVES, NCO, CH, SRC2>()];
+template <int WAVES, int NCO, int CH, bool SRC2, bool NARROW>
+__device__ __forceinline__ void wino_group(const WinoGroupArgs &g, f32x4 *lds) {
     const unsigned per = gridDim.x >> 3;
     for (int i = 0; i < g.n; ++i) {
         const unsigned vblock = (((blockIdx.x >> 3) + per - (unsigned)g.rot[i] % per) % per) << 3 | (blockIdx.x & 7);
-        wino_tiles<WAVES, NCO, CH, SRC2>(g.op[i], lds, vblock, gridDim.x);
+        wino_tiles<WAVES, NCO, CH, SRC2, NARROW>(g.op[i], lds, vblock, gridDim.x);
         asm volatile("s_waitcnt vmcnt(0)" ::: "memory");
         __syncthreads();
     }
 }
-
-template <int WAVES, int NCO>
+template <int WAVES, int NCO, int CH, bool SRC2>
+__global__ __launch_bounds__(64 * WAVES, 2) void conv3x3_wino_group_k(const WinoGroupArgs g) {
+    __shared__ f32x4 lds[2 * wino_stage_slots<WAVES, NCO, CH, SRC2, false>()];
+    wino_group<WAVES, NCO, CH, SRC2, false>(g, lds);
+}
+template <int WAVES, int NCO, int CH, bool SRC2>
+__global__ __launch_bounds__(64 * WAVES, 2) void conv3x3_wino_narrow_group_k(const WinoGroupArgs g) {
+    __shared__ f32x4 lds[2 * wino_stage_slots<WAVES, NCO, CH, SRC2, true>()];
+    wino_group<WAVES, NCO, CH, SRC2, true>(g, lds);
+}
+
+template <int WAVES, int NCO, bool NARROW>
 int wino_args(const ConvArgs &a, int N, WinoArgs &wa) {
-    wa = WinoArgs{a, (a.Wo + kWinoTileW - 1) / kWinoTileW, (a.Ho + 2 * WAVES - 1) / (2 * WAVES), 0};
+    constexpr int tw = NARROW ? kWinoNarrowW : kWinoTileW, th = NARROW ? 4 * WAVES : 2 * WAVES;
+    wa = WinoArgs{a, (a.Wo + tw - 1) / tw, (a.Ho + th - 1) / th, 0};
     wa.c.NT = a.Cout / (16 * NCO);
     const long long tiles = (long long)N * wa.tiles_x * wa.tiles_y * wa.c.NT;
     if (tiles >= (1ll << 31)) return IDH_EUNSUPPORTED;
@@ -481,7 +502,7 @@
     return IDH_OK;
 }
 
-template <int WAVES, int NCO, int CH, bool SRC2>
+template <int WAVES, int NCO, int CH, bool SRC2, bool NARROW>
 long long wino_resident() {
     static int resident = 0;
     if (resident == 0) {
@@ -489,29 +510,30 @@
         if (hipGetDevice(&dev) == hipSuccess) (void)hipDeviceGetAttribute(&cus, hipDeviceAttributeMultiprocessorCount, dev);
         resident = cus > 0 ? cus : 256;
     }
-    constexpr int kLdsBytes = 2 * wino_stage_slots<WAVES, NCO, CH, SRC2>() * 16;
+    constexpr int kLdsBytes = 2 * wino_stage_slots<WAVES, NCO, CH, SRC2, NARROW>() * 16;
     return (long long)resident * (kLdsBytes * 2 <= 160 * 1024 ? 2 : 1);
 }
 
-template <int WAVES, int NCO, int CH, bool SRC2>
+template <int WAVES, int NCO, int CH, bool SRC2, bool NARROW>
 int launch_wino(const ConvArgs &a, int N, hipStream_t st) {
     WinoArgs wa;
-    if (int rc = wino_args<WAVES, NCO>(a, N, wa)) return rc;
-    long long grid = wino_resident<WAVES, NCO, CH, SRC2>();
+    if (int rc = wino_args<WAVES, NCO, NARROW>(a, N, wa)) return rc;
+    long long grid = wino_resident<WAVES, NCO, CH, SRC2, NARROW>();
     if (grid > wa.tiles) grid = wa.tiles >= 8 ? wa.tiles / 8 * 8 : wa.tiles;
-    hipLaunchKernelGGL((conv3x3_wino_k<WAVES, NCO, CH, SRC2>), dim3((unsigned)grid), dim3(64 * WAVES), 0, st, wa);
+    if constexpr (NARROW) hipLaunchKernelGGL((conv3x3_wino_narrow_k<WAVES, NCO, CH, SRC2>), dim3((unsigned)grid), dim3(64 * WAVES), 0, st, wa);
+    else hipLaunchKernelGGL((conv3x3_wino_k<WAVES, NCO, CH, SRC2>), dim3((unsigned)grid), dim3(64 * WAVES), 0, st, wa);
     IDH_CHECK_LAUNCH();
     return IDH_OK;
 }
 
-template <int WAVES, int NCO, int CH, bool SRC2>
+template <int WAVES, int NCO, int CH, bool SRC2, bool NARROW>
 int launch_wino_group(const ConvArgs *const *as, const int *Ns, int n, hipStream_t st) {
     WinoGroupArgs g{};
     long long total = 0;
     int rot = 0;
-    const long long res = wino_resident<WAVES, NCO, CH, SRC2>();
+    const long long res = wino_resident<WAVES, NCO, CH, SRC2, NARROW>();
     for (int i = 0; i < n; ++i) {
-        if (int rc = wino_args<WAVES, NCO>(*as[i], Ns[i], g.op[i])) return rc;
+        if (int rc = wino_args<WAVES, NCO, NARROW>(*as[i], Ns[i], g.op[i])) return rc;
         g.rot[i] = rot;
         rot = (int)((rot + (g.op[i].tiles + 7) / 8) % (res / 8));
         total += g.op[i].tiles;
@@ -520,7 +542,8 @@
     long long grid = res;
     if (grid > total) grid = total >= 8 ? total / 8 * 8 : 8;
     if ((grid & 7) || (res & 7)) return IDH_EUNSUPPORTED;
-    hipLaunchKernelGGL((conv3x3_wino_group_k<WAVES, NCO, CH, SRC2>), dim3((unsigned)grid), dim3(64 * WAVES), 0, st, g);
+    if constexpr (NARROW) hipLaunchKernelGGL((conv3x3_wino_narrow_group_k<WAVES, NCO, CH, SRC2>), dim3((unsigned)grid), dim3(64 * WAVES), 0, st, g);
+    else hipLaunchKernelGGL((conv3x3_wino_group_k<WAVES, NCO, CH, SRC2>), dim3((unsigned)grid), dim3(64 * WAVES), 0, st, g);
     IDH_CHECK_LAUNCH();
     return IDH_OK;
 }
@@ -541,18 +564,19 @@
 
 int wino_max_group() { return kWinoMaxGroup; }
 
-int launch_conv_wino_group(const ConvArgs *const *as, const int *Ns, int n, hipStream_t st) {
+int launch_conv_wino_group(const ConvArgs *const *as, const int *Ns, int n, bool narrow, hipStream_t st) {
     if (n < 1 || n > kWinoMaxGroup) return IDH_EINVAL;
     const bool src2 = as[0]->s[1].in != nullptr;
     for (int i = 0; i < n; ++i)
         if (!wino_supported(*as[i]) || (as[i]->s[1].in != nullptr) != src2) return IDH_EUNSUPPORTED;
-    return src2 ? launch_wino_group<4, 2, kWinoCH, true>(as, Ns, n, st) : launch_wino_group<4, 2, kWinoCH, false>(as, Ns, n, st);
-}
-
-int launch_conv_wino(const ConvArgs &a, int N, int rows, hipStream_t st) {
+    if (narrow) return src2 ? launch_wino_group<4, 2, kWinoCH, true, true>(as, Ns, n, st) : launch_wino_group<4, 2, kWinoCH, false, true>(as, Ns, n, st);
+    return src2 ? launch_wino_group<4, 2, kWinoCH, true, false>(as, Ns, n, st) : launch_wino_group<4, 2, kWinoCH, false, false>(as, Ns, n, st);
+}
+
+int launch_conv_wino(const ConvArgs &a, int N, bool narrow, hipStream_t st) {
     if (!wino_supported(a)) return IDH_EUNSUPPORTED;
-    (void)rows;
-    return a.s[1].in ? launch_wino<4, 2, kWinoCH, true>(a, N, st) : launch_wino<4, 2, kWinoCH, false>(a, N, st);
+    if (narrow) return a.s[1].in ? launch_wino<4, 2, kWinoCH, true, true>(a, N, st) : launch_wino<4, 2, kWinoCH, false, true>(a, N, st);
+    return a.s[1].in ? launch_wino<4, 2, kWinoCH, true, false>(a, N, st) : launch_wino<4, 2, kWinoCH, false, false>(a, N, st);
 }
 
 }
diff --git a/implicit-depth_amd/csrc/networks.hip b/implicit-depth_amd/csrc/networks.hip
--- a/implicit-depth_amd/csrc/networks.hip
+++ b/implicit-depth_amd/csrc/networks.hip
@@ -142,7 +142,7 @@
         d.n_src = (int)srcs.size();
         for (size_t i = 0; i < srcs.size(); ++i) {
             const View &v = srcs[i].v;
-            d.src[i] = idh_conv_desc_src{H(v), W(v), cs(v), srcs[i].cv->cin, srcs[i].cv->ks, srcs[i].cv->stride, 0, 0};
+            d.src[i] = idh_conv_desc_src{H(v), W(v), cs(v), srcs[i].cv->cin, srcs[i].cv->ks, srcs[i].cv->stride, 0, i == 0};
         }
         return idh_conv_select(&d, nullptr, c);
     }
diff --git a/implicit-depth_amd/csrc/plan_select.hip b/implicit-depth_amd/csrc/plan_select.hip
--- a/implicit-depth_amd/csrc/plan_select.hip
+++ b/implicit-depth_amd/csrc/plan_select.hip
@@ -22,12 +22,17 @@
         if (s0.ks != 3 || s0.stride != 1 || d.pad_mode != IDH_PAD_ZEROS || d.Cout % cout_mult || (!cat_ok && s0.is_cat)) return false;
         return !two || (s1.ks == 1 && s1.stride == 1 && (cat_ok || !s1.is_cat));
     }
-    bool wino_grid(int ch, double min_fill, int min_tiles) const {
-        const i64 ty = cdiv(d.Ho, 8), tx = cdiv(d.Wo, 32);
-        if ((double)((i64)d.Ho * d.Wo) < min_fill * (ty * 8) * (tx * 32)) return false;
+    bool wino_grid(int ch, double min_fill, int min_tiles, int tw = 32, int th = 8) const {
+        const i64 ty = cdiv(d.Ho, th), tx = cdiv(d.Wo, tw);
+        if ((double)((i64)d.Ho * d.Wo) < min_fill * (ty * th) * (tx * tw)) return false;
         return d.N * ty * tx * (d.Cout / ch) >= min_tiles;
     }
-    bool wino() const { return plain3(32, false) && wino_grid(32, t.wino_min_fill, t.wino_min_tiles); }
+    int wino_arrangement() const {
+        if (!plain3(32, false)) return -1;
+        if (wino_grid(32, t.wino_min_fill, 0)) return wino_grid(32, t.wino_min_fill, t.wino_min_tiles) ? 0 : -1;
+        return s0.wino_narrow && wino_grid(32, t.wino_min_fill, t.wino_min_tiles, IDH_WINO_NARROW, 16) ? IDH_WINO_NARROW : -1;
+    }
+    bool wino() const { return wino_arrangement() >= 0; }
     bool wino4() const {
         if (!plain3(64, false) || (two && !t.winograd4_proj)) return false;
         if ((d.act != IDH_ACT_NONE && d.act != IDH_ACT_LRELU && d.act != IDH_ACT_ELU) || (d.act == IDH_ACT_LRELU && !(d.slope >= 0.f && d.slope <= 1.f))) return false;
@@ -88,7 +93,9 @@
 void launch_rank(const idh_op &op, int flags, i64 r[3]) {
     const bool conv = op.kind == IDH_OP_CONV, merge = flags & IDH_SCHED_MERGE_LEVELS;
     r[0] = 3; r[1] = 0; r[2] = 0;
-    if ((flags & IDH_SCHED_WINO_GROUP) && conv && op.tile_m == IDH_TILE_WINO) { r[0] = -1; r[1] = op.src[1].in ? 1 : 0; r[2] = -(i64)op.N * op.Ho * op.Wo * op.Cout; }
+    if ((flags & IDH_SCHED_WINO_GROUP) && conv && op.tile_m == IDH_TILE_WINO) {
+        r[0] = -1; r[1] = (op.src[1].in ? 1 : 0) + (op.tile_n == IDH_WINO_NARROW ? 2 : 0); r[2] = -(i64)op.N * op.Ho * op.Wo * op.Cout;
+    }
     else if (conv && op.tile_m == 9) { r[0] = 0; r[1] = op.tile_n; }
     else if (merge && conv && op.tile_m == 1 && op.tile_n == 4) { r[0] = 1; }
     else if (merge && op.kind == IDH_OP_UPSAMPLE2) { r[0] = 2; }
@@ -132,7 +139,7 @@
     } else if (plain && t.winograd4 && (!s.two || !d.has_res) && (c.families & IDH_FAMILY_WINO4)) {
         c.w_layout = IDH_W_WINO4; c.tile_m = IDH_TILE_WINO4;
     } else if (plain && t.winograd && (c.families & IDH_FAMILY_WINO)) {
-        c.w_layout = IDH_W_WINO; c.tile_m = IDH_TILE_WINO;
+        c.w_layout = IDH_W_WINO; c.tile_m = IDH_TILE_WINO; c.tile_n = s.wino_arrangement();
     } else if (c.families & IDH_FAMILY_LDS) {
         c.tile_m = c.lds_tile_m == 8 && t.fused_up_rows == 4 && cat ? 9 : c.lds_tile_m;
         c.tile_n = c.lds_subtiles;
diff --git a/implicit-depth_amd/nhwc.py b/implicit-depth_amd/nhwc.py
--- a/implicit-depth_amd/nhwc.py
+++ b/implicit-depth_amd/nhwc.py
@@ -155,6 +155,7 @@
 
 TILE_WINO = 12
 TILE_WINO4 = 13
+WINO_NARROW = 16
 WINOGRAD = True
 WINO_MIN_TILES = 128
 WINO_MIN_FILL = 0.74
@@ -294,6 +295,7 @@
     for s, (v, cv) in zip(d.src, srcs):
         s.H, s.W, s.cs, s.is_cat = getattr(v, "H", 0), getattr(v, "W", 0), getattr(v, "cs", 0), isinstance(v, CatView)
         s.Cin, s.ks, s.stride = getattr(cv, "in_channels", 0), cv.kernel_size[0], cv.stride[0]
+    d.src[0].wino_narrow = 1
     ch = _lib.ConvChoice()
     _lib.check(_bind().idh_conv_select(C.byref(d), C.byref(conv_tuning()), C.byref(ch)), "idh_conv_select")
     return ch
diff --git a/include/idh_ops.h b/include/idh_ops.h
--- a/include/idh_ops.h
+++ b/include/idh_ops.h
@@ -68,6 +68,7 @@
                                void *stream);
 
 #define IDH_TILE_WINO 12
+#define IDH_WINO_NARROW 16
 size_t idh_packed_wino_weight_floats(int Cout, int Cin);
 int idh_pack_conv_weight_wino(const float *w_oihw, float *dst, int Cout, int Cin, void *stream);
 
@@ -92,7 +93,8 @@
 typedef struct idh_conv_desc_src {
     int32_t H, W, cs;
     int32_t Cin, ks, stride;
-    int32_t is_cat, _r;
+    int32_t is_cat;
+    int32_t wino_narrow;
 } idh_conv_desc_src;
 
 typedef struct idh_conv_desc {
```
